# ViTAE-Transformer/SAMRS

Measured on AMD Instinct MI355X. Metric: images/sec (1024^2, vit_h, 32 boxes/img) SAM box->mask, higher is better.
Workload: dtype f16

## Files before the change

### include/samrs_hip_internal.h

```cpp
#ifndef SAMRS_HIP_INTERNAL_H
#define SAMRS_HIP_INTERNAL_H

#include "samrs_hip.h"

#ifdef __cplusplus
extern "C" {
#endif

int samrs_debug_encoder_prefix(samrs_engine_t* e, const uint8_t* images, int n_images, int in_h,
                               int in_w, int n_blocks, float* x_out, void* stream);

int samrs_debug_outlier_columns(samrs_engine_t* e, int block, int gemm, int32_t* out32);

void samrs_debug_set_gemm_variant(int variant);
void samrs_debug_gemm_choice(int prec, int M, int N, int K, int out_f32, int gelu, int accumulate, int has_add2d, int ld, int variant,
                             int32_t* out);
void samrs_debug_set_gemm_skew(int xcd_units, int cu_units);
int samrs_debug_has_experiments(void);

int samrs_debug_copy_buffer(samrs_engine_t* e, const char* name, void* dst, size_t bytes, void* stream);

int samrs_debug_time_dominant_kernel(samrs_engine_t* e, int enable);
int samrs_debug_dominant_kernel_time(samrs_engine_t* e, float* avg_ms, int* launches, int* M, int* N, int* K);

// ... 43 lines not shown
int samrs_k_mask_embed(const float* w0, const float* b0, const float* ln1w, const float* ln1b, const float* w3, const float* b3,
                       const float* ln4w, const float* ln4b, const float* w6, const float* b6, const float* mask_in, float* dense,
                       int n, int grid, void* stream);
int samrs_k_fill_slot_table(const int32_t* start_host, const int32_t* slot_host, int n_runs, int32_t* out, void* stream);
int samrs_k_make_keys(int prec, const float* emb, const float* dense, const float* vec, float* out_f32, void* out_et, int n_batches,
                      int tokens, int C, const int32_t* slot_of, void* stream);
int samrs_k_token_self_attn(const float* q, const float* k, const float* v, float* o, int n, int T, int C, int heads, void* stream);
int64_t samrs_k_t2i_workspace_floats(int n, int T);
int samrs_k_t2i_attention(int prec, const float* qp, const void* kp_et, const void* vp_et, int ld, int64_t bstride, float* out,
                          float* workspace, int n, int T, int tokens, int Ci, int heads, const int32_t* slot_of, void* stream);
int samrs_k_i2t_attention(int prec, const void* qi_et, int ld, int64_t bstride, const float* kt, const float* vt, void* out_et, int n,
                          int T, int tokens, int Ci, int heads, void* stream);
int samrs_k_i2t_fused(int prec, const void* qi_et, int ld, int64_t q_bstride, const float* kt, const float* vt, const void* w_et,
                      const void* w_lo_et, const float* bias, const float* resid, int64_t r_bstride, const float* gamma,
                      const float* beta, float eps, float* outF, void* outE, void* outE_lo, int n, int T, int tokens, int Ci, int C,
                      const int32_t* slot_of, void* stream);
int samrs_k_group_ln_gelu(int prec, const float* in, const float* gamma, const float* beta, float eps, void* out_et, int64_t rows,
                          int groups, int gsize, void* stream);
int samrs_k_mask_product(int prec, const void* up2_et, const float* hyper, float* low, int n, int grid, int n_mask_tokens, int sel0,
                         int n_sel, void* stream);
int samrs_k_attention_mx(int prec, int global, const void* qkv_et, const float* qkv_bias, const float* rel_h, const float* rel_w,
                         void* out_et, void* out_lo_et, int n_images, int grid, int heads, int head_dim, void* q_hi, void* q_lo,
                         void* s_hi, void* s_lo, void* stream);
int64_t samrs_k_mx_scale_bytes(int rows, int Kp, int is_b);
int samrs_k_layernorm_mx(int prec, const float* X, const float* gamma, const float* beta, float eps, void* out_et, int rows, int D,
                         void* q_hi, void* q_lo, void* s_hi, void* s_lo, void* stream);
int samrs_k_mx4_pack(int prec, const float* x, const void* hi_in, const void* lo_in, void* out_hi, void* q_hi, void* q_lo, void* s_hi,
                     void* s_lo, int rows, int K, int G, int GP, int is_b, void* stream);
int samrs_k_gemm_mx(int prec, const void* A, const void* B, void* C, const float* bias, int M, int N, int K, int Kp, const void* a4_lo,
                    const void* a4_hi, const void* sa_lo, const void* sa_hi, const void* b4_hi, const void* b4_lo, const void* sb_hi,
                    const void* sb_lo, int out_f32, int accumulate, int split_from_n, void* stream);
int samrs_k_gemm_mx_gelu_mxout(int prec, const void* A, const void* B, void* C_et, const float* bias, int M, int N, int K, int Kp,
                               const void* a4_lo, const void* a4_hi, const void* sa_lo, const void* sa_hi, const void* b4_hi, const void* b4_lo,
                               const void* sb_hi, const void* sb_lo, int gelu, void* o4_hi, void* o4_lo, void* so_hi, void* so_lo, void* stream);
int samrs_k_convert_split(int prec, const float* in, void* out_hi_et, void* out_lo_et, int64_t n, void* stream);
int samrs_k_range_profile(int prec, const void* x_et, long n, int cols, int ld, int64_t* row48, void* stream);
int samrs_k_column_stats(int prec, const void* x_et, int M, int K, int ld, float* partials, double* sumsq, uint32_t* maxbits, void* stream);
int samrs_k_audit_rows_per_partial(void);
int samrs_k_gemm_ld(int prec, const void* A_et, const void* B_et, void* C_et, const float* bias, int M, int N, int K, int ld, int gelu,
                    int gelu_form, void* stream);
int samrs_k_gemm_ext(int prec, const void* A_et, const void* B_et, const void* Ax_et, const void* Bx_et, float* C, const float* bias, int M,
                     int N, int K, void* stream);
int samrs_k_layernorm_ext(int prec, const float* X, const float* gamma, const float* beta, float eps, void* out_et, int rows, int D,
                          int ld_out, const int32_t* oc_idx, int n_oc, int window_mode, void* stream);
int samrs_k_outlier_weight_ext(int prec, const float* W, int N, int K, const int32_t* idx, int n_oc, void* out_et, int ld, int col0,
                               void* stream);
int samrs_k_outlier_side_weight(int prec, const float* W1, const float* b1, int n_rows1, int D, const int32_t* idx2, int n2,
                                const int32_t* idx1, int n1, void* out_et, int Ks, float* bias_out, void* stream);
int samrs_k_outlier_gather(const void* hi_et, const void* lo_et, int D, const int32_t* idx, int n_oc, void* out_et, int rows, void* stream);
int samrs_k_outlier_side_gemm(int prec, const void* Y_et, int lda, const void* Ws_et, const float* bias, int M, int K, void* out_et,
                              void* stream);
int samrs_k_weight_norms(const float* W, int N, int K, float* col_sq, float* row_sq, void* stream);
int samrs_k_range_scan(int prec, const void* x_et, int64_t n, int cols, int ld, uint64_t* counter, void* stream);
int samrs_k_gemm_f32_batch(const float* const* A, const float* const* A2, const float* const* W, const float* const* bias, float* const* C,
                           int count, int lda, int ldc, int M, int N, int K, int relu, int accumulate, void* stream);
int samrs_k_patch_im2col(int prec, const uint8_t* img_u8, void* A_et, void* A_lo_et, int n_images, int in_h, int in_w, int grid, int patch,
                         void* stream);
int samrs_k_transpose_f32(const float* in, float* out, int rows, int cols, void* stream);
int samrs_k_gelu_split(int prec, const float* in, void* hi_et, void* lo_et, int64_t n, void* stream);
int samrs_k_region_labels(const uint8_t* masks, int n, int h, int w, int complement, int32_t* labels_out, void* stream);
int samrs_k_mask_row_extents(const uint8_t* masks, int n, int h, int w, int32_t* ext_out, void* stream);
int samrs_k_mask_hull(const uint8_t* masks, int n, int h, int w, int x0, int y0, int32_t* ext_scratch, int32_t* verts_out, int cap,
                      int32_t* counts_out, void* stream);
int64_t samrs_k_polygon_scratch_bytes(int n, int h, int w, int max_edges);
int64_t samrs_k_polygon_edge_stride(int h, int w, int max_edges);
int samrs_k_polygon_edges(const uint8_t* masks, int n, int h, int w, int max_edges, void* scratch, uint32_t* ids_out, int32_t* succ_out,
                          uint8_t* corner_out, int32_t* counts_out, void* stream);
int samrs_k_polygon_ranks(const uint8_t* masks, int n, int h, int w, int max_edges, void* scratch, int32_t* leader_out,
                          int32_t* rank_out, int32_t* counts_out, void* stream);
int64_t samrs_k_polygon_simplify_scratch_bytes(int n, int64_t vertex_capacity, int64_t ring_capacity);
int samrs_k_polygon_simplify_keep(const int32_t* vertices, const int32_t* rings, const int64_t* table, int n, int eps_q,
                                  int64_t vertex_capacity, int64_t ring_capacity, void* scratch, uint8_t* keep_out, int32_t* kept_out,
                                  void* stream);

#ifdef __cplusplus
}
#endif
#endif
```

### samrs_amd/csrc/encoder_kernels.hip

```cpp
#include "common.h"
#include "kernels.h"

namespace {

__constant__ float c_mean[3] = {123.675f, 116.28f, 103.53f};
__constant__ float c_std[3] = {58.395f, 57.12f, 57.375f};

template <int PREC>
__global__ void patch_im2col_kernel(const uint8_t* __restrict__ img, uint16_t* __restrict__ A, uint16_t* __restrict__ A_lo,
                                    int n_images, int in_h, int in_w, int grid, int patch) {
    const int P2 = patch * patch;
    const int halves = patch / 8;
    const long total = (long)n_images * grid * grid * patch * halves;
    const long t = (long)blockIdx.x * blockDim.x + threadIdx.x;
    if (t >= total) return;
    const int half = t % halves;
    long u = t / halves;
    const int ky = u % patch; u /= patch;
    const int px = u % grid; u /= grid;
    const int py = u % grid;
    const int im = u / grid;
    const int y = py * patch + ky, x0 = px * patch + half * 8;
    float v[3][8];
#pragma unroll
// ... 1459 lines not shown
    }();
    dim3 g(n_items < n_cu ? n_items : n_cu), b(C::THREADS);
    k<<<g, b, C::LDS_BYTES, s>>>((const uint16_t*)qkv, qb, rh, rw, (uint16_t*)out, grid, heads, n_items, (uint16_t*)out_lo, mx, lo_heads,
                                 dense);
    return hipGetLastError();
}

hipError_t launch_window_attention(int prec, const void* qkv, const float* qkv_bias, const float* rel_h, const float* rel_w, void* out,
                                   int n_images, int grid, int window, int heads, int head_dim, hipStream_t s, void* out_lo,
                                   void* mx_q_hi, void* mx_q_lo, void* mx_s_hi, void* mx_s_lo, uint32_t lo_heads) {
    if (window != 14) return hipErrorInvalidValue;
    if (heads > 32) lo_heads = 0xffffffffu;
    MxOut mx;
    if (mx_q_hi) {
        if (!mx_q_lo || !mx_s_hi || !mx_s_lo || (heads * ((head_dim + 31) / 32) * 32) % MXK) return hipErrorInvalidValue;
        mx.q_hi = (unsigned char*)mx_q_hi; mx.q_lo = (unsigned char*)mx_q_lo; mx.s_hi = (unsigned char*)mx_s_hi; mx.s_lo = (unsigned char*)mx_s_lo;
    }
#define WIN_CALL(P, H)                                                                                                          \
    return mx_q_hi ? launch_win<P, H, 2>(qkv, qkv_bias, rel_h, rel_w, out, n_images, grid, heads, s, nullptr, mx)               \
         : out_lo ? launch_win<P, H, 1>(qkv, qkv_bias, rel_h, rel_w, out, n_images, grid, heads, s, out_lo, MxOut(), lo_heads)  \
                  : launch_win<P, H, 0>(qkv, qkv_bias, rel_h, rel_w, out, n_images, grid, heads, s)
    if (prec == PREC_BF16) {
        if (head_dim == 64) WIN_CALL(PREC_BF16, 64);
        if (head_dim == 80) WIN_CALL(PREC_BF16, 80);
    } else if (prec == PREC_F16) {
        if (head_dim == 64) WIN_CALL(PREC_F16, 64);
        if (head_dim == 80) WIN_CALL(PREC_F16, 80);
    }
#undef WIN_CALL
    return hipErrorInvalidValue;
}

static int g_glb_waves = [] { const char* v = getenv("SAMRS_GLB_WAVES"); return (v && atoi(v) == 4) ? 4 : 8; }();

template <int PREC, int HD, int NW, int LO = 0>
static hipError_t launch_glb_nw(const void* qkv, const float* rh, const float* rw, void* out, int n_images,
                                int heads, void* vt_ws, hipStream_t s, void* out_lo = nullptr, MxOut mx = MxOut()) {
    using C = GlbCfg<HD, NW>;
    constexpr int NTOK = C::G * C::G;
#ifdef SAMRS_EXPERIMENTS
    static const bool pipe = [] { const char* v = getenv("SAMRS_GLB_PIPE"); return v ? atoi(v) != 0 : false; }();
    auto k = pipe ? global_attention_kernel<PREC, HD, NW, LO, 1> : global_attention_kernel<PREC, HD, NW, LO, 0>;
#else
    auto k = global_attention_kernel<PREC, HD, NW, LO, 0>;
#endif
    HIP_CHECK_RET(set_lds(k, C::LDS_BYTES));
    dim3 g((NTOK / (32 * NW)) * heads * n_images), b(64 * NW);
    k<<<g, b, C::LDS_BYTES, s>>>((const uint16_t*)qkv, (const uint16_t*)vt_ws, rh, rw, (uint16_t*)out, heads, (uint16_t*)out_lo, mx);
    return hipGetLastError();
}

template <int PREC, int HD>
static hipError_t launch_glb(const void* qkv, const float* rh, const float* rw, void* out, int n_images,
                             int heads, void* vt_ws, hipStream_t s, void* out_lo, MxOut mx) {
    constexpr int NTOK = GlbCfg<HD>::G * GlbCfg<HD>::G;
    vt_pack_kernel<HD><<<n_images * heads * (NTOK / 64), 256, 0, s>>>((const uint16_t*)qkv, (uint16_t*)vt_ws, heads, NTOK);
    HIP_CHECK_RET(hipGetLastError());
    if (mx.q_hi) return launch_glb_nw<PREC, HD, 8, 2>(qkv, rh, rw, out, n_images, heads, vt_ws, s, nullptr, mx);
    if (out_lo) return launch_glb_nw<PREC, HD, 8, 1>(qkv, rh, rw, out, n_images, heads, vt_ws, s, out_lo);
    if (g_glb_waves == 4) return launch_glb_nw<PREC, HD, 4>(qkv, rh, rw, out, n_images, heads, vt_ws, s);
    return launch_glb_nw<PREC, HD, 8>(qkv, rh, rw, out, n_images, heads, vt_ws, s);
}

hipError_t launch_global_attention(int prec, const void* qkv, const float* rel_h, const float* rel_w, void* out,
                                   int n_images, int grid, int heads, int head_dim, void* vt_ws, hipStream_t s, void* out_lo,
                                   void* mx_q_hi, void* mx_q_lo, void* mx_s_hi, void* mx_s_lo) {
    if (grid != 64 || !vt_ws) return hipErrorInvalidValue;
    MxOut mx;
    if (mx_q_hi) {
        if (!mx_q_lo || !mx_s_hi || !mx_s_lo || (heads * ((head_dim + 31) / 32) * 32) % MXK) return hipErrorInvalidValue;
        mx.q_hi = (unsigned char*)mx_q_hi; mx.q_lo = (unsigned char*)mx_q_lo; mx.s_hi = (unsigned char*)mx_s_hi; mx.s_lo = (unsigned char*)mx_s_lo;
    }
    if (prec == PREC_BF16) {
        if (head_dim == 64) return launch_glb<PREC_BF16, 64>(qkv, rel_h, rel_w, out, n_images, heads, vt_ws, s, out_lo, mx);
        if (head_dim == 80) return launch_glb<PREC_BF16, 80>(qkv, rel_h, rel_w, out, n_images, heads, vt_ws, s, out_lo, mx);
    } else if (prec == PREC_F16) {
        if (head_dim == 64) return launch_glb<PREC_F16, 64>(qkv, rel_h, rel_w, out, n_images, heads, vt_ws, s, out_lo, mx);
        if (head_dim == 80) return launch_glb<PREC_F16, 80>(qkv, rel_h, rel_w, out, n_images, heads, vt_ws, s, out_lo, mx);
    }
    return hipErrorInvalidValue;
}

template <int PREC>
__global__ void gelu_split_kernel(const float* __restrict__ in, uint16_t* __restrict__ hi, uint16_t* __restrict__ lo, long n4) {
    const long i = (long)blockIdx.x * blockDim.x + threadIdx.x;
    if (i >= n4) return;
    const float4 v = reinterpret_cast<const float4*>(in)[i];
    const float2_t a = gelu_erf2(float2_t{v.x, v.y}), b = gelu_erf2(float2_t{v.z, v.w});
    uint2 h, l;
    split2_pack<PREC>(a.x, a.y, h.x, l.x);
    split2_pack<PREC>(b.x, b.y, h.y, l.y);
    reinterpret_cast<uint2*>(hi)[i] = h;
    reinterpret_cast<uint2*>(lo)[i] = l;
}
hipError_t launch_gelu_split(int prec, const float* in, void* hi, void* lo, long n, hipStream_t s) {
    if (n % 4 || !hi || !lo) return hipErrorInvalidValue;
    const long n4 = n / 4;
    const int blocks = (int)((n4 + 255) / 256);
    if (prec == PREC_BF16) gelu_split_kernel<PREC_BF16><<<blocks, 256, 0, s>>>(in, (uint16_t*)hi, (uint16_t*)lo, n4);
    else gelu_split_kernel<PREC_F16><<<blocks, 256, 0, s>>>(in, (uint16_t*)hi, (uint16_t*)lo, n4);
    return hipGetLastError();
}

hipError_t launch_neck_im2col(const void* in, void* A, int n_images, int grid, int C, hipStream_t s) {
    if (C % 8) return hipErrorInvalidValue;
    const long total = (long)n_images * grid * grid * (9 * C / 8);
    neck_im2col_kernel<<<(int)((total + 255) / 256), 256, 0, s>>>((const uint16_t*)in, (uint16_t*)A, n_images, grid, C);
    return hipGetLastError();
}

hipError_t launch_transpose_f32(const float* in, float* out, int rows, int cols, hipStream_t s) {
    dim3 g((cols + 31) / 32, (rows + 31) / 32), b(32, 8);
    transpose_f32_kernel<<<g, b, 0, s>>>(in, out, rows, cols);
    return hipGetLastError();
}
```

### samrs_amd/csrc/engine.hip

```cpp
#include <algorithm>
#include <cmath>
#include <cstdlib>

#include "engine_state.h"

static int env_int(const char* name, int dflt) { const char* v = getenv(name); return v ? atoi(v) : dflt; }

namespace {

bool is_global(const samrs_config& c, int i) {
    for (int k = 0; k < c.n_global; ++k)
        if (c.global_attn_indexes[k] == i) return true;
    return false;
}

void required_tensors(const samrs_engine* e, std::vector<std::pair<std::string, std::vector<int64_t>>>& out) {
    const samrs_config& c = e->cfg;
    const int64_t D = c.embed_dim, g = e->grid, hd = e->hd, C = c.out_chans, P = c.patch_size;
    auto add = [&](const std::string& n, std::vector<int64_t> s) { out.emplace_back(n, std::move(s)); };
    add("image_encoder.pos_embed", {1, g, g, D});
    add("image_encoder.patch_embed.proj.weight", {D, 3, P, P});
    add("image_encoder.patch_embed.proj.bias", {D});
    for (int i = 0; i < c.depth; ++i) {
        const std::string p = "image_encoder.blocks." + std::to_string(i);
// ... 201 lines not shown
extern "C" {

int samrs_abi_version(void) { return SAMRS_ABI_VERSION; }

const char* samrs_last_error(const samrs_engine_t* e) { return e ? e->err.c_str() : "null engine"; }

samrs_engine_t* samrs_create(const samrs_config* cfg, int device, char* err, int err_len) {
    auto bad = [&](const char* m) -> samrs_engine_t* {
        if (err && err_len > 0) snprintf(err, err_len, "%s", m);
        return nullptr;
    };
    if (!cfg) return bad("null config");
    if (cfg->img_size != 1024 || cfg->patch_size != 16 || cfg->window_size != 14 || cfg->out_chans != 256)
        return bad("only img_size 1024 / patch 16 / window 14 / out_chans 256 are supported (build_sam.py:62-80)");
    if (cfg->embed_dim % 128 || cfg->embed_dim % cfg->num_heads) return bad("embed_dim must be a multiple of 128 and of num_heads");
    const int hd = cfg->embed_dim / cfg->num_heads;
    if (hd != 64 && hd != 80) return bad("head_dim must be 64 or 80");
    if (cfg->precision != SAMRS_PREC_BF16 && cfg->precision != SAMRS_PREC_F16) return bad("bad precision");
    if (cfg->max_images < 1 || cfg->max_prompts < 1 || cfg->max_points < 0 || cfg->n_global < 0 || cfg->n_global > 8)
        return bad("bad capacity / n_global");
    if (5 + cfg->max_points + 1 + 2 > 16) return bad("max_points too large (token count must stay <= 16)");
    {
        DeviceGuard dg(device);
        if (dg.status != hipSuccess) return bad("hipSetDevice failed (no HIP device? this library has no CPU fallback)");
    }
    samrs_engine* e = new samrs_engine();
    e->cfg = *cfg;
    e->device = device;
    e->prec = cfg->precision;
    e->grid = cfg->img_size / cfg->patch_size;
    e->tokens = e->grid * e->grid;
    e->D = cfg->embed_dim;
    e->C = cfg->out_chans;
    e->hd = hd;
    e->nwin = (e->grid + cfg->window_size - 1) / cfg->window_size;
    e->T_max = 5 + cfg->max_points + 1 + 2;
    e->decode_prompts = cfg->max_prompts;
    e->slot_set.assign(cfg->max_images, 0);
    e->slot_split.assign(cfg->max_images, 0);
    e->slot_depth.assign(cfg->max_images, 0);
    e->decoder_fusion = env_int("SAMRS_DECODER_FUSION", 1) != 0;
    e->ln_fold = env_int("SAMRS_LN_FOLD", 0) != 0 && gemm_has_experiments();
    const bool h_like = gemm_split3_ok(e->tokens, 3 * e->D, e->D) && gemm_split3_ok(e->tokens, e->D, e->D) && (2 * e->D) % 320 == 0;
    e->split = env_int("SAMRS_SPLIT", SPLIT_DEFAULT | (h_like ? SPLIT_ATTN_V : 0)) & SPLIT_ALL;
    e->grade_multimask = h_like ? SPLIT_ATTN_ANY : 0;
    e->allow_reduced = env_int("SAMRS_ALLOW_REDUCED", getenv("SAMRS_SPLIT") ? 1 : 0) != 0;
    e->upscaler_fused = env_int("SAMRS_UPSCALER_FUSED", 1) != 0;
    e->split_passes = env_int("SAMRS_SPLIT_PASSES", 0) != 0;
    e->split_depth = env_int("SAMRS_SPLIT_DEPTH", 0);
    e->lo_format = (h_like && env_int("SAMRS_LO_FORMAT", 4) == 4) ? 4 : 0;
    e->gelu_fast = env_int("SAMRS_GELU_FAST", -1);
    e->ln_tail = env_int("SAMRS_LN_TAIL", 0) != 0;
    e->operand_pad_on = env_int("SAMRS_OPERAND_PAD", 1) != 0;
    e->outlier_on = env_int("SAMRS_OUTLIER_COLS", 7) & 7;
    e->outlier_ratio_pct = env_int("SAMRS_OUTLIER_RATIO_PCT", 400);
    if (e->outlier_ratio_pct < 101) e->outlier_ratio_pct = 101;
    if (e->gelu_fast > 1) e->gelu_fast = 1;
    e->range_profile = env_int("SAMRS_RANGE_PROFILE", 0);
    if (e->range_profile < 0 || e->range_profile > 2) e->range_profile = 0;
    e->audit_passes = env_int("SAMRS_AUDIT_PASSES", 0);
    if (e->audit_passes > 0) e->range_profile = 2; else e->audit_passes = 0;
    if (const int rc0 = env_int("SAMRS_RANGE_CHECK", 0)) {
        if (samrs_set_option(e, "range_check", rc0) != SAMRS_OK) {
            if (err && err_len > 0) snprintf(err, err_len, "SAMRS_RANGE_CHECK=%d: %s", rc0, e->err.c_str());
            samrs_destroy(e);
            return nullptr;
        }
    }
    return e;
}

void samrs_destroy(samrs_engine_t* e) {
    if (!e) return;
    DeviceGuard dg(e->device);
    for (void* p : e->owned) (void)hipFree(p);
    for (DeviceScratch* sc : {&e->rle_scratch, &e->rle_decode_scratch, &e->region_scratch, &e->box_scratch, &e->poly_scratch, &e->png_scratch, &e->png_rgb_scratch, &e->overlap_scratch, &e->ap_scratch, &e->boundary_scratch}) scratch_release(*sc);
    delete e;
}

int samrs_load_weight(samrs_engine_t* e, const char* name, const float* host, const int64_t* shape, int ndim) {
    if (!e || !name || !host || !shape || ndim < 1 || ndim > 4) return fail(e, SAMRS_ERR_BAD_ARG, "samrs_load_weight: bad argument");
    if (e->finalized) return fail(e, SAMRS_ERR_BAD_WEIGHTS, "weights already finalized");
    ON_DEVICE(e);
    DevTensor t;
    t.shape.assign(shape, shape + ndim);
    t.numel = 1;
    for (int i = 0; i < ndim; ++i) t.numel *= (size_t)shape[i];
    const std::string n(name);
    std::vector<float> tmp;
    const float* src = host;
    if (n == "image_encoder.neck.2.weight" && ndim == 4) {
        const int64_t Co = shape[0], Ci = shape[1], KH = shape[2], KW = shape[3];
        tmp.resize(t.numel);
        for (int64_t co = 0; co < Co; ++co)
            for (int64_t ci = 0; ci < Ci; ++ci)
                for (int64_t ky = 0; ky < KH; ++ky)
                    for (int64_t kx = 0; kx < KW; ++kx)
                        tmp[(co * KH * KW + ky * KW + kx) * Ci + ci] = host[((co * Ci + ci) * KH + ky) * KW + kx];
        src = tmp.data();
    } else if ((n == "mask_decoder.output_upscaling.0.weight" || n == "mask_decoder.output_upscaling.3.weight") && ndim == 4) {
        const int64_t Ci = shape[0], Co = shape[1];
        tmp.resize(t.numel);
        for (int64_t ci = 0; ci < Ci; ++ci)
            for (int64_t co = 0; co < Co; ++co)
                for (int64_t s = 0; s < 4; ++s) tmp[(s * Co + co) * Ci + ci] = host[(ci * Co + co) * 4 + s];
        src = tmp.data();
// ... 324 lines not shown

int samrs_get_slot_info(const samrs_engine_t* e, int slot, int32_t* is_set, int32_t* split, int32_t* split_depth) {
    if (!e) return SAMRS_ERR_BAD_ARG;
    if (slot < 0 || slot >= e->cfg.max_images) return SAMRS_ERR_CAPACITY;
    if (is_set) *is_set = e->slot_set[slot];
    if (split) *split = e->slot_set[slot] ? e->slot_split[slot] : 0;
    if (split_depth) *split_depth = e->slot_set[slot] ? e->slot_depth[slot] : 0;
    return SAMRS_OK;
}

int samrs_reset_image(samrs_engine_t* e, int slot) {
    if (!e) return SAMRS_ERR_BAD_ARG;
    if (slot < 0 || slot >= e->cfg.max_images) return fail(e, SAMRS_ERR_CAPACITY, "slot out of range");
    e->slot_set[slot] = 0;
    return SAMRS_OK;
}

int samrs_set_option(samrs_engine_t* e, const char* name, int value) {
    if (!e || !name) return SAMRS_ERR_BAD_ARG;
    const std::string n(name);
    if (n == "decoder_fusion") e->decoder_fusion = value != 0;
    else if (n == "ln_fold") {
        if (value && !gemm_has_experiments())
            return fail(e, SAMRS_ERR_BAD_ARG, "ln_fold: the folded LayerNorm (measured slower: DESIGN.md 6) is built with make EXPERIMENTS=1 only");
        e->ln_fold = value != 0;
    }
    else if (n == "split") {
        if (e->finalized && (value & (SPLIT_ATTN_ANY | SPLIT_MLP | SPLIT_LIN2) & ~e->split_ready))
            return fail(e, SAMRS_ERR_BAD_ARG, "split bits 16 / 32 / 64 / 128 (block GEMMs) need their lo weights: set them before the weights are "
                                              "finalized (SAMRS_SPLIT or options={'split': ...})");
        e->split = value & SPLIT_ALL;
    }
    else if (n == "gemm_variant") e->gemm_variant = value;
    else if (n == "decode_prompts") {
        const long long prod = (long long)e->cfg.max_images * e->cfg.max_prompts;
        const int lo = e->cfg.max_prompts, lim = prod < DECODE_PROMPTS_LIMIT ? (int)prod : DECODE_PROMPTS_LIMIT, hi = lim > lo ? lim : lo;
        if (value < lo || value > hi)
            return fail(e, SAMRS_ERR_BAD_ARG, "decode_prompts=%d is outside [%d, %d]: from max_prompts to max_images x max_prompts = %lld, "
                                              "at most %d (the index range of the decoder kernels)", value, lo, hi, prod, DECODE_PROMPTS_LIMIT);
        if (e->finalized) {
            ON_DEVICE(e);
            const int rc = grow_decode_workspaces(e, value);
            if (rc != SAMRS_OK) return rc;
        }
        e->decode_prompts = value;
    }
    else if (n == "upscaler_fused") e->upscaler_fused = value != 0;
    else if (n == "split_passes") e->split_passes = value != 0;
    else if (n == "split_depth") e->split_depth = value > 0 ? value : 0;
    else if (n == "allow_reduced") e->allow_reduced = value != 0;
    else if (n == "gelu_fast") e->gelu_fast = value < 0 ? -1 : (value != 0);
    else if (n == "ln_tail") e->ln_tail = value > 0;
    else if (n == "operand_pad") e->operand_pad_on = value != 0;
    else if (n == "outlier_cols") e->outlier_on = value & 7;
    else if (n == "outlier_ratio_pct") {
        if (e->finalized) return fail(e, SAMRS_ERR_BAD_ARG, "outlier_ratio_pct: the columns are picked when the weights are finalized; set it before");
        if (value < 101) return fail(e, SAMRS_ERR_BAD_ARG, "outlier_ratio_pct must exceed 100 (a column's score as a percentage of the median score)");
        e->outlier_ratio_pct = value;
    }
    else if (n == "range_check") {
        if (value < 0 || value > 2) return fail(e, SAMRS_ERR_BAD_ARG, "range_check is 0 (off), 1 (count) or 2 (count, and samrs_set_images fails)");
        if (value && !e->range_counter) {
            ON_DEVICE(e);
            CK(e, dalloc(e, &e->range_counter, 1));
            CK(e, hipMemset(e->range_counter, 0, sizeof(unsigned long long)));
        }
        if (value == 2 && e->range_check != 2 && e->range_counter) {
            ON_DEVICE(e);
            CK(e, hipDeviceSynchronize());
            CK(e, hipMemcpy(&e->range_seen, e->range_counter, sizeof(unsigned long long), hipMemcpyDeviceToHost));
        }
        e->range_check = value;
    }
    else if (n == "saturated") {
        if (e->range_counter) {
            ON_DEVICE(e);
            CK(e, hipDeviceSynchronize());
            CK(e, hipMemset(e->range_counter, 0, sizeof(unsigned long long)));
        }
        e->range_seen = 0;
    }
    else if (n == "range_profile") {
        if (value < 0 || value > 2) return fail(e, SAMRS_ERR_BAD_ARG, "range_profile is 0 (off), 1 (range profile per site) or 2 (and column statistics)");
        e->range_profile = value;
        if (!value) e->audit_passes = 0;
    }
    else if (n == "audit_passes") {
        if (value < 0) return fail(e, SAMRS_ERR_BAD_ARG, "audit_passes is the number of encoder passes to profile (0 stops a running audit)");
        if (value > 0) {
            ON_DEVICE(e);
            const int rc = audit_reset(e);
            if (rc != SAMRS_OK) return rc;
            e->range_profile = 2;
        } else if (e->audit_passes > 0) e->range_profile = 0;
        e->audit_passes = value;
    }
    else if (n == "lo_format") {
        if (value != 0 && value != 4) return fail(e, SAMRS_ERR_BAD_ARG, "lo_format is 0 (f16 lo terms) or 4 (MXFP4 lo terms)");
        if (value == 4 && e->finalized && !e->mx_ready && !e->mx_mlp_ready)
            return fail(e, SAMRS_ERR_BAD_ARG, "lo_format 4 needs the fp4 weight copies: set it (and a block-GEMM split bit) before the weights are "
                                              "finalized; it covers the attention-side split of models whose block GEMMs fit the 256 x 320 tile (ViT-H)");
        e->lo_format = value;
    }
    else return fail(e, SAMRS_ERR_BAD_ARG, "unknown option %s", name);
    return SAMRS_OK;
}
int samrs_get_option(const samrs_engine_t* e, const char* name, int* value) {
    if (!e || !name || !value) return SAMRS_ERR_BAD_ARG;
    const std::string n(name);
    if (n == "decoder_fusion") *value = e->decoder_fusion;
    else if (n == "ln_fold") *value = e->ln_fold;
    else if (n == "split") *value = e->split;
    else if (n == "gemm_variant") *value = e->gemm_variant;
    else if (n == "decode_prompts") *value = e->decode_prompts;
    else if (n == "decode_kbytes") *value = (int)((e->decode_bytes + 1023) / 1024);
    else if (n == "upscaler_fused") *value = e->upscaler_fused;
    else if (n == "split_passes") *value = e->split_passes;
    else if (n == "split_depth") *value = e->split_depth;
    else if (n == "allow_reduced") *value = e->allow_reduced;
    else if (n == "gelu_fast") *value = e->gelu_fast;
    else if (n == "ln_tail") *value = e->ln_tail;
    else if (n == "operand_pad") *value = e->operand_pad_on;
    else if (n == "outlier_cols") *value = e->outlier_on;
    else if (n == "outlier_ratio_pct") *value = e->outlier_ratio_pct;
    else if (n == "outlier_blocks") *value = e->outlier_blocks;
    else if (n == "outlier_columns") *value = e->outlier_columns;
    else if (n == "outlier_dominant_blocks") *value = e->outlier_dominant_blocks;
    else if (n == "range_check") *value = e->range_check;
    else if (n == "saturated") {
        unsigned long long c = 0;
        if (e->range_counter) {
            DeviceGuard dg(e->device);
            if (dg.status != hipSuccess || hipDeviceSynchronize() != hipSuccess ||
                hipMemcpy(&c, e->range_counter, sizeof(c), hipMemcpyDeviceToHost) != hipSuccess) return SAMRS_ERR_HIP;
        }
        *value = c > 0x7fffffffull ? 0x7fffffff : (int)c;
    }
    else if (n == "range_profile") *value = e->range_profile;
    else if (n == "audit_passes") *value = e->audit_passes;
    else if (n == "lo_format") *value = (e->finalized && !e->mx_ready && !e->mx_mlp_ready) ? 0 : e->lo_format;
    else if (n == "grade_multimask") *value = e->grade_multimask;
    else return SAMRS_ERR_BAD_ARG;
    return SAMRS_OK;
}

}
```

### samrs_amd/csrc/engine_decode.hip

```cpp
#include "engine_state.h"

namespace {

struct PredictImage {
    int slot, p0, p1, in_h, in_w, orig_h, orig_w;
    void* masks;
};


enum class I2T { FUSED, PER_SEGMENT, SHARED_RESIDUAL, ACCUMULATE };
enum class Upscaler { ONE_KERNEL, GLN_SPLIT, GLN, UNFUSED };

struct DecodeLayerRoute {
    bool shared = false;
    long bstride = 0;
    bool tab = false;
    I2T i2t = I2T::FUSED;
    bool write_kf = false;
    bool write_ke_lo = false;
    bool ow_lo = false;
};

struct DecodeRoute {
    int T = 0, BT = 0, Mi = 0;
// ... 149 lines not shown
    const size_t hs = (size_t)e->decode_alloc * C;
    F32Batch l0{}, l1{}, l2{};
    for (int i = 0; i < 5; ++i) {
        l0.A[i] = i < 4 ? e->Q + (size_t)(1 + i) * C : e->Q;
        l0.W[i] = w.head_w[i][0]; l0.bias[i] = w.head_b[i][0]; l0.C[i] = e->HY1 + i * hs;
        l1.A[i] = e->HY1 + i * hs;
        l1.W[i] = w.head_w[i][1]; l1.bias[i] = w.head_b[i][1]; l1.C[i] = e->HY2 + i * hs;
        if (i < 4) {
            l2.A[i] = e->HY2 + i * hs;
            l2.W[i] = w.head_w[i][2]; l2.bias[i] = w.head_b[i][2]; l2.C[i] = e->HYPER + i * (C / 8);
        }
    }
    CK(e, launch_gemm_f32_batch(l0, 5, r.T * C, C, n, C, C, true, false, s));
    CK(e, launch_gemm_f32_batch(l1, 5, C, C, n, C, C, true, false, s));
    CK(e, launch_gemm_f32_batch(l2, 4, C, 4 * (C / 8), n, C / 8, C, false, false, s));
    if (r.iou)
        CK(e, launch_gemm_f32(e->HY2 + 4 * hs, C, w.head_w[4][2] + (size_t)r.sel0 * C, w.head_b[4][2] + r.sel0, iou_out, r.nsel, n, r.nsel, C,
                              false, false, s));
    return SAMRS_OK;
}

static int run_upscaler(samrs_engine_t* e, const DecodeRoute& r, int n, float* low, hipStream_t s) {
    const int C = e->C, prec = e->prec, g = e->grid, Mi = r.Mi;
    for (const char* name : {"U1raw", "U1", "U2"}) {
        const bool used = !strcmp(name, "U1raw") ? (r.up == Upscaler::GLN_SPLIT || r.up == Upscaler::UNFUSED)
                        : !strcmp(name, "U1")    ? (r.up == Upscaler::GLN || r.up == Upscaler::UNFUSED) : r.up == Upscaler::UNFUSED;
        if (used) { const int rc = need_decode_buffer(e, name); if (rc != SAMRS_OK) return rc; }
    }
    switch (r.up) {
    case Upscaler::ONE_KERNEL:
        CK(e, launch_upscaler_fused(prec, e->KE, r.sp_up ? e->KE_lo : nullptr, e->up1_w, r.sp_up ? e->up1_w_lo : nullptr, e->up1_b, e->up_ln,
                                    e->up2_w, r.sp_up ? e->up2_w_lo : nullptr, e->up2_b, e->HYPER, low, n, g, 4, r.sel0, r.nsel, s));
        break;
    case Upscaler::GLN_SPLIT:
        CK(e, launch_gemm_et_gln(prec, e->KE, e->up1_w, e->U1raw, e->up1_b, e->up_ln, Mi, C, C, s, e->KE_lo, e->up1_w_lo));
        CK(e, launch_upscale2_masks(prec, e->U1raw, e->up2_w, e->up2_w_lo, e->up2_b, e->HYPER, low, n, g, 4, r.sel0, r.nsel, s));
        break;
    case Upscaler::GLN:
        CK(e, launch_gemm_et_gln(prec, e->KE, e->up1_w, e->U1, e->up1_b, e->up_ln, Mi, C, C, s));
        CK(e, launch_upscale2_masks(prec, e->U1, e->up2_w, nullptr, e->up2_b, e->HYPER, low, n, g, 4, r.sel0, r.nsel, s));
        break;
    case Upscaler::UNFUSED:
        CK(e, launch_gemm_et(prec, e->KE, e->up1_w, e->U1raw, e->up1_b, nullptr, 0, Mi, C, C, true, false, false, s));
        CK(e, launch_group_ln_gelu(prec, e->U1raw, e->dec.up_ln_w, e->dec.up_ln_b, 1e-6f, e->U1, (long)Mi, 4, C / 4, s));
        CK(e, launch_gemm_et(prec, e->U1, e->up2_w, e->U2, e->up2_b, nullptr, 0, Mi * 4, C / 2, C / 4, false, true, false, s));
        CK(e, launch_mask_product(prec, e->U2, e->HYPER, low, n, g, 4, r.sel0, r.nsel, s));
        break;
    }
    return SAMRS_OK;
}

static int run_postprocess(samrs_engine_t* e, const DecodeRoute& r, const PredictImage* seg, int n_seg, const float* low, int return_logits,
                           hipStream_t s) {
    for (int k = 0; k < n_seg; ++k)
        if (seg[k].masks)
            CK(e, launch_postprocess(low + (size_t)seg[k].p0 * r.nsel * 256 * 256, (seg[k].p1 - seg[k].p0) * r.nsel, seg[k].in_h, seg[k].in_w,
                                     seg[k].orig_h, seg[k].orig_w, e->cfg.img_size, return_logits, seg[k].masks, s));
    return SAMRS_OK;
}

static int predict_chunk(samrs_engine_t* e, const PredictImage* seg, int n_seg, int n, const float* boxes, const float* point_coords,
                         const int32_t* point_labels, int n_points, const float* mask_input, int multimask,
                         int return_logits, float* iou_out, float* lowres_out, void* stream) {
    if (n < 1 || n > e->decode_prompts || n > e->decode_alloc)
        return fail(e, SAMRS_ERR_CAPACITY, "a decoder chain of %d prompts exceeds decode_prompts=%d", n, e->decode_prompts);
    hipStream_t s = (hipStream_t)stream;
    ON_DEVICE(e);
    const DecodeRoute r = decode_route(e, n, n_seg, seg[0].slot, boxes != nullptr, point_coords ? n_points : 0, mask_input != nullptr,
                                       multimask != 0, iou_out != nullptr, lowres_out != nullptr);
    float* low = r.low_own ? e->LOW : lowres_out;
    int rc;
    if ((rc = run_prompt_side(e, r, seg, n_seg, n, boxes, point_coords, point_labels, n_points, mask_input, s))) return rc;
    for (int li = 0; li < 2; ++li)
        if ((rc = run_dec_layer(e, r, li, seg, n_seg, n, s))) return rc;
    if ((rc = run_final_attn(e, r, n, s))) return rc;
    if ((rc = run_heads(e, r, n, iou_out, s))) return rc;
    if ((rc = run_upscaler(e, r, n, low, s))) return rc;
    return run_postprocess(e, r, seg, n_seg, low, return_logits, s);
}

static std::string slot_note(int slot) { return " (slot " + std::to_string(slot) + ")"; }

static int check_multimask_grade(samrs_engine_t* e, int slot, bool multi) {
    if (e->allow_reduced || !e->grade_multimask || slot < 0 || slot >= e->cfg.max_images || !e->slot_set[slot]) return SAMRS_OK;
    const int sm = e->slot_split[slot];
    const int need_depth = sm < 0 ? 0 : (sm & (SPLIT_ATTN | SPLIT_MLP | SPLIT_LIN2)) ? e->cfg.depth : (3 * e->cfg.depth + 3) / 4;
    if (sm >= 0 && (!(sm & e->grade_multimask) || e->slot_depth[slot] < need_depth ||
                    (e->split & (SPLIT_OI | SPLIT_UP)) != (SPLIT_OI | SPLIT_UP)))
        return fail(e, SAMRS_ERR_PRECISION, "multimask_output=True on an embedding encoded with split=%d over %d of %d blocks (decoder split=%d): "
                    "this model's multimask outputs need a block-GEMM split bit (64 or 16) at its automatic depth and the decoder "
                    "bits 4 | 8 to hold IoU >= 0.999; re-encode the image in the engine's default mode, or set option "
                    "\"allow_reduced\" = 1%s", sm, e->slot_depth[slot], need_depth, e->split, multi ? slot_note(slot).c_str() : "");
    return SAMRS_OK;
}

static int check_predict(samrs_engine_t* e, const PredictImage* im, int n_img, bool multi, const float* boxes, const float* point_coords,
                         const int32_t* point_labels, int n_points, const float* mask_input) {
    if (!e->finalized) return fail(e, SAMRS_ERR_BAD_WEIGHTS, "weights not finalized");
    const samrs_config& c = e->cfg;
    for (int i = 0; i < n_img; ++i) {
        const int slot = im[i].slot;
        if (slot < 0 || slot >= c.max_images)
            return multi ? fail(e, SAMRS_ERR_CAPACITY, "image %d: slot %d out of range (max_images=%d)", i, slot, c.max_images)
                         : fail(e, SAMRS_ERR_CAPACITY, "slot out of range");
        if (!e->slot_set[slot])
            return multi ? fail(e, SAMRS_ERR_NOT_SET, "An image must be set with .set_image(...) before mask prediction "
                                "(image %d: slot %d is not set).", i, slot)
                         : fail(e, SAMRS_ERR_NOT_SET, "An image must be set with .set_image(...) before mask prediction.");
    }
    if (!boxes && !point_coords && !mask_input) return fail(e, SAMRS_ERR_BAD_ARG, "at least one prompt (points, boxes or mask_input) is required");
// ... 77 lines not shown
```

### samrs_amd/csrc/engine_encode.hip

```cpp
#include "engine_state.h"

enum { AUDIT_QKV_IN = 0, AUDIT_Q, AUDIT_K, AUDIT_V, AUDIT_PROJ_IN, AUDIT_LIN1_IN, AUDIT_LIN2_IN, AUDIT_PER_BLOCK };
enum { AUDIT_NECK1_IN = 0, AUDIT_NECK2_IN, AUDIT_KEYS0, AUDIT_TAIL };

namespace samrs_detail {
void audit_build_sites(samrs_engine_t* e) {
    static const char* const per_block[AUDIT_PER_BLOCK] = {"qkv_in", "q", "k", "v", "proj_in", "lin1_in", "lin2_in"};
    e->audit_sites.clear();
    e->audit_columns = 0;
    auto add = [&](const std::string& name, int columns) {
        e->audit_sites.push_back({name, columns, e->audit_columns});
        e->audit_columns += (size_t)columns;
    };
    for (int i = 0; i < e->cfg.depth; ++i)
        for (int k = 0; k < AUDIT_PER_BLOCK; ++k)
            add("blocks." + std::to_string(i) + "." + per_block[k],
                (k == AUDIT_QKV_IN || k == AUDIT_PROJ_IN || k == AUDIT_LIN1_IN) ? e->D : k == AUDIT_LIN2_IN ? 4 * e->D : 0);
    add("neck.conv1_in", 0); add("neck.conv2_in", 0); add("decoder.keys0", 0);
    e->audit_col_rows.assign(e->audit_sites.size(), 0);
}

int audit_reset(samrs_engine_t* e) {
    if (e->audit_rows || e->audit_sumsq) CK(e, hipDeviceSynchronize());
    if (e->audit_rows) CK(e, hipMemset(e->audit_rows, 0, e->audit_sites.size() * AUDIT_PROFILE_WORDS * sizeof(long long)));
// ... 62 lines not shown
    if (r == hipSuccess && order == MainPass::LAST) r = launch_gemm_et(prec, A, B, C, bias, add2d, add2d_period, M, N, K, true, false, true, s);
    return r;
}

namespace {
struct PassRoute {
    int M = 0;
    int n_blocks = 0;
    bool sp_patch = false, sp_neck = false;
    bool one3 = false;
    bool fold = false;
    int depth_full = 0, depth_v = 0;
    bool fast_gelu = false;
    bool ln_tail = false;
    bool pad_ok = false;
    bool oc_any = false, oc_ok = false;
};

static PassRoute pass_route(const samrs_engine_t* e, int M, int n_blocks) {
    const samrs_config& c = e->cfg;
    const int D = e->D;
    PassRoute p;
    p.M = M;
    p.n_blocks = n_blocks;
    p.sp_patch = (e->split & SPLIT_PATCH) != 0;
    p.sp_neck = (e->split & SPLIT_NECK) != 0;
    p.fold = e->can_fold && e->ln_fold && !(e->split & SPLIT_ATTN_ANY) && !(e->split & SPLIT_MLP);
    p.depth_full = e->split_depth > 0 ? e->split_depth : c.depth;
    p.depth_v = e->split_depth > 0 ? e->split_depth : (3 * c.depth + 3) / 4;
    p.one3 = !e->split_passes;
    p.fast_gelu = e->gelu_fast >= 0 ? e->gelu_fast != 0 : !(e->split & (SPLIT_ATTN_ANY | SPLIT_MLP | SPLIT_LIN2));
    p.ln_tail = !p.fold && !(e->split & (SPLIT_ATTN_ANY | SPLIT_MLP | SPLIT_LIN2)) && e->ln_tail > 0 &&
                e->ln_counters && gemm_lntail_ok(M, D, D) && gemm_lntail_ok(M, D, 4 * D);
    p.pad_ok = e->ldk && e->operand_pad_on && !p.fold && !p.ln_tail;
    p.oc_any = e->outlier_on && e->outlier_columns > 0 && !p.fold && !p.ln_tail;
    p.oc_ok = p.oc_any && (e->outlier_on & 1);
    return p;
}

enum class Norm { NONE, TAIL, PLAIN, LO, MX };
enum class Gemm { FOLD, MX, SPLIT3, PLAIN, LNTAIL, EXT };
enum class Wcopy { W, WP, WX };

struct BlockRoute {
    Norm norm1 = Norm::PLAIN, norm2 = Norm::PLAIN;
    Gemm qkv = Gemm::PLAIN, proj = Gemm::PLAIN, lin1 = Gemm::PLAIN, lin2 = Gemm::PLAIN;
    bool qkv_one = false, proj_one = false, lin1_one = false, lin2_one = false;
    int v_from = 0;
    int noc = 0;
    Wcopy qkv_wc = Wcopy::W;
    int qkv_K = 0, qkv_ld = 0;
    int norm1_ld = 0;
    int y1_ld = 0, y1_live = 0;
    bool mx_ao = false;
    bool ao_lo = false;
    int nop = 0;
    uint32_t lo_heads = 0xffffffffu;
    int nol = 0;
    Wcopy lin1_wc = Wcopy::W;
    int lin1_K = 0, lin1_ld = 0;
    int norm2_ld = 0;
    int y2_ld = 0, y2_live = 0;
    int lin1_mx_from = 0;
    int nol2 = 0;
    int side_ld = 0;
    bool next_rowstat = false;
};

static BlockRoute block_route(const samrs_engine_t* e, const PassRoute& p, const EncBlock& b, int i) {
    const int D = e->D, M = p.M, depth = e->cfg.depth;
    BlockRoute r;
    const bool attn_full = (e->split & SPLIT_ATTN) && i < p.depth_full;
    const bool oc_dominant = p.oc_any && (e->outlier_on & 5) == 5 && !attn_full && (b.oc_share[0] > 0.5f || b.oc_share[3] > 0.5f);
    const bool sp_attn = attn_full || ((e->split & SPLIT_ATTN_V) && i < p.depth_v && !oc_dominant);
    const bool sp_mlp = (e->split & SPLIT_MLP) && i < p.depth_full;
    const bool mx_mlp = e->lo_format == 4 && e->mx_mlp_ready && !e->split_passes && gemm_mx_ok(M, 4 * D, D, D) && gemm_mx_ok(M, D, 4 * D, e->mx_kp_lin2);
    const bool sp_lin2 = (e->split & SPLIT_LIN2) && !sp_mlp && mx_mlp && i < p.depth_full;
    const bool mx_attn = e->lo_format == 4 && e->mx_ready && !e->split_passes && gemm_mx_ok(M, 3 * D, D, D) && (2 * D) % 320 == 0;

    r.qkv_K = D; r.y1_ld = D; r.y1_live = D;
    if (p.fold) {
        r.norm1 = Norm::NONE; r.qkv = Gemm::FOLD;
    } else if (sp_attn && mx_attn) {
        r.norm1 = Norm::MX; r.qkv = Gemm::MX;
        r.v_from = attn_full ? 0 : 2 * D;
        r.noc = (p.oc_ok && !attn_full && b.oc_n[0] && e->ldk && b.qkv_wp) ? b.oc_n[0] : 0;
        if (r.noc) { r.qkv_wc = Wcopy::WP; r.qkv_ld = r.norm1_ld = r.y1_ld = e->ldk; r.y1_live = D + 64; }
    } else if (sp_attn) {
        r.norm1 = Norm::LO; r.qkv = Gemm::SPLIT3;
        r.qkv_one = p.one3 && gemm_split3_ok(M, 3 * D, D);
        r.v_from = (!attn_full && r.qkv_one && (2 * D) % 320 == 0) ? 2 * D : 0;
    } else {
        r.noc = (p.oc_ok && b.oc_n[0] && b.qkv_wx) ? b.oc_n[0] : 0;
        r.qkv_K = r.noc ? D + 64 : D;
        r.qkv_ld = (p.pad_ok && b.qkv_wp && gemm_ld_ok(M, 3 * D, r.qkv_K, false)) ? e->ldk : 0;
        r.qkv_wc = r.qkv_ld ? Wcopy::WP : (r.noc ? Wcopy::WX : Wcopy::W);
        r.y1_ld = r.qkv_ld ? r.qkv_ld : r.qkv_K;
        r.y1_live = r.qkv_K;
        r.norm1_ld = r.y1_ld == D ? 0 : r.y1_ld;
    }

    r.mx_ao = sp_attn && mx_attn;
    r.nop = (p.oc_any && (e->outlier_on & 4) && !sp_attn && b.oc_n[3] && b.oc_bx[3] && e->AOlo && e->OCX) ? b.oc_n[3] : 0;
    r.ao_lo = (sp_attn && !r.mx_ao) || r.nop;
    r.lo_heads = r.nop ? b.oc_heads : 0xffffffffu;

    if (p.fold) r.proj = Gemm::FOLD;
    else if (sp_attn && mx_attn) r.proj = Gemm::MX;
    else if (sp_attn) { r.proj = Gemm::SPLIT3; r.proj_one = p.one3 && gemm_split3_ok(M, D, D); }
    else if (p.ln_tail) r.proj = Gemm::LNTAIL;
    else if (r.nop) r.proj = Gemm::EXT;

    const bool lin1_plain = !p.fold && !sp_lin2 && !sp_mlp;
    r.nol = (p.oc_ok && lin1_plain && b.oc_n[1] && b.lin1_wx) ? b.oc_n[1] : 0;
    r.lin1_K = r.nol ? D + 64 : D;
    r.lin1_ld = (p.pad_ok && b.lin1_wp && lin1_plain && gemm_ld_ok(M, 4 * D, r.lin1_K, true)) ? e->ldk : 0;
    r.lin1_wc = r.lin1_ld ? Wcopy::WP : (r.nol ? Wcopy::WX : Wcopy::W);
    r.side_ld = r.lin1_ld ? r.lin1_ld : r.lin1_K;
    r.y2_ld = D; r.y2_live = D;
    if (p.fold) r.norm2 = Norm::NONE;
    else if (r.proj == Gemm::LNTAIL) r.norm2 = Norm::TAIL;
    else if (sp_mlp && mx_mlp) r.norm2 = Norm::MX;
    else {
        r.norm2 = sp_mlp ? Norm::LO : Norm::PLAIN;
        r.norm2_ld = (sp_mlp || r.side_ld == D) ? 0 : r.side_ld;
        if (r.norm2_ld) { r.y2_ld = r.norm2_ld; r.y2_live = r.lin1_K; }
    }
    if (p.fold) r.lin1 = Gemm::FOLD;
    else if (sp_lin2) { r.lin1 = Gemm::MX; r.lin1_mx_from = 4 * D; }
    else if (sp_mlp && mx_mlp) r.lin1 = Gemm::MX;
    else if (sp_mlp) { r.lin1 = Gemm::SPLIT3; r.lin1_one = p.one3 && gemm_split3_ok(M, 4 * D, D); }

    r.nol2 = (p.oc_any && (e->outlier_on & 2) && lin1_plain && b.oc_n[2] && b.oc_bx[2] && e->OCX && b.lin2_ws &&
              (b.oc_n[1] == 0 || r.nol > 0)) ? b.oc_n[2] : 0;
    if (p.fold) { r.lin2 = Gemm::FOLD; r.next_rowstat = i + 1 < depth; }
    else if ((sp_mlp && mx_mlp) || sp_lin2) r.lin2 = Gemm::MX;
    else if (sp_mlp) { r.lin2 = Gemm::SPLIT3; r.lin2_one = p.one3 && gemm_split3_ok(M, D, 4 * D); }
    else if (p.ln_tail && i + 1 < depth && i + 1 < p.n_blocks) r.lin2 = Gemm::LNTAIL;
    else if (r.nol2) r.lin2 = Gemm::EXT;
    return r;
}

static const uint16_t* weight_copy(Wcopy c, const uint16_t* w, const uint16_t* wp, const uint16_t* wx) {
    return c == Wcopy::WP ? wp : c == Wcopy::WX ? wx : w;
}

static hipError_t run_norm(samrs_engine_t* e, Norm form, const float* gamma, const float* beta, int M, int ld, const int* oc_idx, int n_oc,
                           hipStream_t s) {
    if (form == Norm::NONE || form == Norm::TAIL) return hipSuccess;
    const bool mx = form == Norm::MX;
    return launch_layernorm(e->prec, e->X, gamma, beta, 1e-6f, e->Y, nullptr, M, e->D, 0, e->grid, 0, s, form == Norm::LO ? e->Ylo : nullptr,
                            mx ? e->Y4[0] : nullptr, mx ? e->Y4[1] : nullptr, mx ? e->SY4[0] : nullptr, mx ? e->SY4[1] : nullptr, ld,
                            n_oc ? oc_idx : nullptr, n_oc);
}
}

static int run_patch_embed(samrs_engine_t* e, const PassRoute& p, const uint8_t* const* images, const int* in_h, const int* in_w, int n,
                           hipStream_t s) {
    const samrs_config& c = e->cfg;
    const int D = e->D, tokens = e->tokens, prec = e->prec, M = p.M;
    const size_t KP = (size_t)3 * c.patch_size * c.patch_size;
    uint16_t* Hlo = e->H + (size_t)M * KP;
    for (int i = 0; i < n;) {
        int j = i + 1;
        while (j < n && in_h[j] == in_h[i] && in_w[j] == in_w[i] &&
               images[j] == images[i] + (size_t)(j - i) * in_h[i] * in_w[i] * 3) ++j;
        CK(e, launch_patch_im2col(prec, images[i], e->H + (size_t)i * tokens * KP, j - i, in_h[i], in_w[i], e->grid, c.patch_size, s,
                                  p.sp_patch ? Hlo + (size_t)i * tokens * KP : nullptr));
        i = j;
    }
    const float *bias = W(e, "image_encoder.patch_embed.proj.bias"), *pos = W(e, "image_encoder.pos_embed");
    if (p.sp_patch)
        CK(e, gemm_hilo(prec, p.one3 && gemm_split3_ok(M, D, (int)KP, true), MainPass::FIRST, e->H, Hlo, e->patch_w, e->patch_w_lo, e->X,
                        bias, pos, tokens, M, D, (int)KP, false, s));
    else
        CK(e, launch_gemm_et(prec, e->H, e->patch_w, e->X, bias, pos, tokens, M, D, (int)KP, true, false, false, s));
    if (p.fold && p.n_blocks > 0) {
        CK(e, launch_rowstats_convert(prec, e->X, e->Y, e->STATS, M, D, s));
        CK(e, launch_ln_rowstat(e->STATS, e->ROWSTAT, M, 1e-6f, s));
    }
    return SAMRS_OK;
}

static int run_block_attn(samrs_engine_t* e, const PassRoute& p, const BlockRoute& r, const EncBlock& b, int i, int n, bool y_ready,
                          hipStream_t s) {
    const samrs_config& c = e->cfg;
    const int D = e->D, g = e->grid, prec = e->prec, M = p.M;
    int rc;
    if (!y_ready) CK(e, run_norm(e, r.norm1, b.ln1w, b.ln1b, M, r.norm1_ld, b.oc_idx[0], r.noc, s));
    const uint16_t* qkv_w = weight_copy(r.qkv_wc, b.qkv_w, b.qkv_wp, b.qkv_wx);
    if (r.qkv == Gemm::FOLD) {
        CK(e, launch_gemm_et_fold(prec, e->Y, b.qkv_wf, e->QKV, b.qkv_bf, b.qkv_c, e->ROWSTAT, M, 3 * D, D, false, s));
    } else if (r.qkv == Gemm::MX) {
        CK(e, launch_gemm_et_mx(prec, e->Y, qkv_w, e->QKV, b.qkv_b, M, 3 * D, D, D, e->Y4[1], e->Y4[0], e->SY4[1], e->SY4[0],
                                b.qkv_w4[0], b.qkv_w4[1], b.qkv_s4[0], b.qkv_s4[1], false, false, r.v_from, s,
                                false, nullptr, nullptr, nullptr, nullptr, r.qkv_ld, r.noc != 0));
    } else if (r.qkv == Gemm::SPLIT3 && r.qkv_one) {
        CK(e, launch_gemm_et_split3(prec, e->Y, e->Ylo, b.qkv_w, b.qkv_w_lo, e->QKV, b.qkv_b, M, 3 * D, D, false, false, s, r.v_from));
    } else if (r.qkv == Gemm::SPLIT3) {
        if (!e->F32T) CK(e, dalloc(e, &e->F32T, (size_t)c.max_images * e->tokens * 4 * D));
        CK(e, gemm_hilo(prec, false, MainPass::LAST, e->Y, e->Ylo, b.qkv_w, b.qkv_w_lo, e->F32T, b.qkv_b, nullptr, 0, M, 3 * D, D, false, s));
        CK(e, launch_convert(prec, e->F32T, e->QKV, (long)M * 3 * D, s));
    } else {
        CK(e, launch_gemm_et(prec, e->Y, qkv_w, e->QKV, b.qkv_b, nullptr, 0, M, 3 * D, r.qkv_K, false, false, false, s, GemmOpts{r.qkv_ld, 1}));
    }
    if (!b.global)
        CK(e, launch_window_attention(prec, e->QKV, b.qkv_b, b.rel_h, b.rel_w, e->AO, n, g, c.window_size, c.num_heads, e->hd, s,
                                      r.ao_lo ? e->AOlo : nullptr, r.mx_ao ? e->AO4[0] : nullptr, r.mx_ao ? e->AO4[1] : nullptr,
                                      r.mx_ao ? e->SAO4[0] : nullptr, r.mx_ao ? e->SAO4[1] : nullptr, r.lo_heads));
    else
        CK(e, launch_global_attention(prec, e->QKV, b.rel_h, b.rel_w, e->AO, n, g, c.num_heads, e->hd, e->VTG, s,
                                      r.ao_lo ? e->AOlo : nullptr, r.mx_ao ? e->AO4[0] : nullptr, r.mx_ao ? e->AO4[1] : nullptr,
                                      r.mx_ao ? e->SAO4[0] : nullptr, r.mx_ao ? e->SAO4[1] : nullptr));
    if ((rc = range_scan(e, e->Y, (size_t)M * r.y1_live, s, r.y1_live, r.y1_ld))) return rc;
    if ((rc = range_scan(e, e->QKV, (size_t)M * 3 * D, s))) return rc;
    if ((rc = range_scan(e, e->AO, (size_t)M * D, s))) return rc;
    if ((rc = audit_site(e, AUDIT_PER_BLOCK * i + AUDIT_QKV_IN, e->Y, M, D, r.y1_ld, s))) return rc;
    for (int t = 0; t < 3; ++t)
        if ((rc = audit_site(e, AUDIT_PER_BLOCK * i + AUDIT_Q + t, e->QKV + (size_t)t * D, M, D, 3 * D, s))) return rc;
    if ((rc = audit_site(e, AUDIT_PER_BLOCK * i + AUDIT_PROJ_IN, e->AO, M, D, D, s))) return rc;

    if (r.proj == Gemm::FOLD) {
        CK(e, launch_gemm_et_stats(prec, e->AO, b.proj_w, e->X, b.proj_b, e->Y, e->STATS, M, D, D, s));
        CK(e, launch_ln_rowstat(e->STATS, e->ROWSTAT, M, 1e-6f, s));
    } else if (r.proj == Gemm::MX) {
        CK(e, launch_gemm_et_mx(prec, e->AO, b.proj_w, e->X, b.proj_b, M, D, D, e->mx_kp_proj, e->AO4[1], e->AO4[0], e->SAO4[1],
                                e->SAO4[0], b.proj_w4[0], b.proj_w4[1], b.proj_s4[0], b.proj_s4[1], true, true, 0, s));
    } else if (r.proj == Gemm::SPLIT3) {
        CK(e, gemm_hilo(prec, r.proj_one, MainPass::LAST, e->AO, e->AOlo, b.proj_w, b.proj_w_lo, e->X, b.proj_b, nullptr, 0, M, D, D, true, s));
    } else if (r.proj == Gemm::LNTAIL) {
        CK(e, launch_gemm_et_lntail(prec, e->AO, b.proj_w, e->X, b.proj_b, M, D, D, b.ln2w, b.ln2b, 1e-6f, e->Y, e->ln_counters, s));
    } else if (r.proj == Gemm::EXT) {
        CK(e, launch_outlier_gather(e->AO, e->AOlo, D, b.oc_idx[3], r.nop, e->OCX, M, s));
        CK(e, resid_gemm_ext(e, prec, e->AO, b.proj_w, e->OCX, b.oc_bx[3], b.proj_b, M, D, D, s));
    } else {
        CK(e, launch_gemm_et(prec, e->AO, b.proj_w, e->X, b.proj_b, nullptr, 0, M, D, D, true, false, true, s));
    }
    CK(e, run_norm(e, r.norm2, b.ln2w, b.ln2b, M, r.norm2_ld, b.oc_idx[1], r.nol, s));
    return SAMRS_OK;
}

static int run_block_mlp(samrs_engine_t* e, const PassRoute& p, const BlockRoute& r, const EncBlock& b, int i, bool* y_ready, hipStream_t s) {
    const int D = e->D, prec = e->prec, M = p.M;
    int rc;
    hipEvent_t t0 = nullptr, t1 = nullptr;
    if (e->timing) {
        auto get = [&](hipEvent_t* ev) -> hipError_t {
            if (!e->tpool.empty()) { *ev = e->tpool.back(); e->tpool.pop_back(); return hipSuccess; }
            return hipEventCreate(ev);
        };
        CK(e, get(&t0)); CK(e, get(&t1));
        CK(e, hipEventRecord(t0, s));
    }
    if (r.lin1 == Gemm::FOLD) {
        CK(e, launch_gemm_et_fold(prec, e->Y, b.lin1_wf, e->H, b.lin1_bf, b.lin1_c, e->ROWSTAT, M, 4 * D, D, true, s));
    } else if (r.lin1 == Gemm::MX) {
        CK(e, launch_gemm_et_mx(prec, e->Y, b.lin1_w, e->H, b.lin1_b, M, 4 * D, D, D, e->Y4[1], e->Y4[0], e->SY4[1], e->SY4[0], b.lin1_w4[0],
                                b.lin1_w4[1], b.lin1_s4[0], b.lin1_s4[1], false, false, r.lin1_mx_from, s, true, e->H4[0], e->H4[1], e->SH4[0], e->SH4[1]));
    } else if (r.lin1 == Gemm::SPLIT3) {
        CK(e, gemm_hilo(prec, r.lin1_one, MainPass::LAST, e->Y, e->Ylo, b.lin1_w, b.lin1_w_lo, e->F32T, b.lin1_b, nullptr, 0, M, 4 * D, D, false, s));
        CK(e, launch_gelu_split(prec, e->F32T, e->H, e->Hlo, (long)M * 4 * D, s));
    } else {
        CK(e, launch_gemm_et(prec, e->Y, weight_copy(r.lin1_wc, b.lin1_w, b.lin1_wp, b.lin1_wx), e->H, b.lin1_b, nullptr, 0, M, 4 * D, r.lin1_K,
                             false, true, false, s, GemmOpts{r.lin1_ld, p.fast_gelu ? 2 : 1}));
    }
    if (e->timing) {
        CK(e, hipEventRecord(t1, s));
        e->tev.emplace_back(t0, t1);
    }
    if ((rc = range_scan(e, e->Y, (size_t)M * r.y2_live, s, r.y2_live, r.y2_ld))) return rc;
    if ((rc = range_scan(e, e->H, (size_t)M * 4 * D, s))) return rc;
    if ((rc = audit_site(e, AUDIT_PER_BLOCK * i + AUDIT_LIN1_IN, e->Y, M, D, r.y2_ld, s))) return rc;
    if ((rc = audit_site(e, AUDIT_PER_BLOCK * i + AUDIT_LIN2_IN, e->H, M, 4 * D, 4 * D, s))) return rc;

    *y_ready = false;
    if (r.lin2 == Gemm::FOLD) {
        CK(e, launch_gemm_et_stats(prec, e->H, b.lin2_w, e->X, b.lin2_b, e->Y, e->STATS, M, D, 4 * D, s));
        if (r.next_rowstat) CK(e, launch_ln_rowstat(e->STATS, e->ROWSTAT, M, 1e-6f, s));
    } else if (r.lin2 == Gemm::MX) {
        CK(e, launch_gemm_et_mx(prec, e->H, b.lin2_w, e->X, b.lin2_b, M, D, 4 * D, e->mx_kp_lin2, e->H4[1], e->H4[0], e->SH4[1], e->SH4[0],
                                b.lin2_w4[0], b.lin2_w4[1], b.lin2_s4[0], b.lin2_s4[1], true, true, 0, s));
    } else if (r.lin2 == Gemm::SPLIT3) {
        CK(e, gemm_hilo(prec, r.lin2_one, MainPass::LAST, e->H, e->Hlo, b.lin2_w, b.lin2_w_lo, e->X, b.lin2_b, nullptr, 0, M, D, 4 * D, true, s));
    } else if (r.lin2 == Gemm::LNTAIL) {
        const EncBlock& nb = e->blocks[i + 1];
        CK(e, launch_gemm_et_lntail(prec, e->H, b.lin2_w, e->X, b.lin2_b, M, D, 4 * D, nb.ln1w, nb.ln1b, 1e-6f, e->Y, e->ln_counters, s));
        *y_ready = true;
    } else if (r.lin2 == Gemm::EXT) {
        CK(e, launch_outlier_side_gemm(prec, e->Y, r.side_ld, b.lin2_ws, b.lin2_sb, M, r.lin1_K, e->OCX, s));
        CK(e, resid_gemm_ext(e, prec, e->H, b.lin2_w, e->OCX, b.oc_bx[2], b.lin2_b, M, D, 4 * D, s));
    } else {
        CK(e, launch_gemm_et(prec, e->H, b.lin2_w, e->X, b.lin2_b, nullptr, 0, M, D, 4 * D, true, false, true, s));
    }
    return SAMRS_OK;
}

static int prepare_slot_keys(samrs_engine_t* e, int slot0, int n, hipStream_t s) {
    const int C = e->C, Ci = C / 2, tokens = e->tokens, prec = e->prec;
    const DecLayer& L = e->layers[0];
    for (int i = 0; i < n; ++i) {
        const size_t o = (size_t)(slot0 + i) * tokens * C;
        CK(e, launch_make_keys(prec, e->EMB + o, nullptr, e->dec.no_mask_embed, e->K0F + o, e->K0E + o, 1, tokens, C, s));
    }
    CK(e, launch_gemm_et(prec, e->K0E + (size_t)slot0 * tokens * C, L.kvq_w, e->KVQ0 + (size_t)slot0 * tokens * 3 * Ci, L.kvq_b, L.kvq_pe,
                         tokens, n * tokens, 3 * Ci, C, false, false, false, s));
    return SAMRS_OK;
}

static int run_neck(samrs_engine_t* e, const PassRoute& p, int n, int slot0, hipStream_t s) {
    const samrs_config& c = e->cfg;
    const int D = e->D, C = e->C, g = e->grid, tokens = e->tokens, prec = e->prec, M = p.M;
    const int audit_tail = AUDIT_PER_BLOCK * c.depth;
    int rc;
    uint16_t* lo_buf = e->QKV;
    if (p.sp_neck) CK(e, launch_convert(prec, e->X, e->Y, (long)M * D, s, lo_buf));
    else if (!(p.fold && c.depth > 0 && p.n_blocks >= c.depth)) CK(e, launch_convert(prec, e->X, e->Y, (long)M * D, s));
    if ((rc = range_scan(e, e->Y, (size_t)M * D, s))) return rc;
    if ((rc = audit_site(e, audit_tail + AUDIT_NECK1_IN, e->Y, M, D, D, s))) return rc;
    if (p.sp_neck)
        CK(e, gemm_hilo(prec, p.one3 && gemm_split3_ok(M, C, D, true), MainPass::FIRST, e->Y, lo_buf, e->neck0_w, e->neck0_w_lo, e->N1,
                        nullptr, nullptr, 0, M, C, D, false, s));
    else
        CK(e, launch_gemm_et(prec, e->Y, e->neck0_w, e->N1, nullptr, nullptr, 0, M, C, D, true, false, false, s));
    CK(e, launch_layernorm(prec, e->N1, W(e, "image_encoder.neck.1.weight"), W(e, "image_encoder.neck.1.bias"), 1e-6f,
                           e->N1e, nullptr, M, C, 0, g, 0, s, p.sp_neck ? lo_buf : nullptr));
    if ((rc = range_scan(e, e->N1e, (size_t)M * C, s))) return rc;
    if ((rc = audit_site(e, audit_tail + AUDIT_NECK2_IN, e->N1e, M, C, C, s))) return rc;
    CK(e, launch_neck_im2col(e->N1e, e->H, n, g, C, s));
    uint16_t* H2lo = e->H + (size_t)M * 9 * C;
    if (p.sp_neck) {
        CK(e, launch_neck_im2col(lo_buf, H2lo, n, g, C, s));
        CK(e, gemm_hilo(prec, p.one3 && gemm_split3_ok(M, C, 9 * C, true), MainPass::FIRST, e->H, H2lo, e->neck2_w, e->neck2_w_lo, e->N1,
                        nullptr, nullptr, 0, M, C, 9 * C, false, s));
    } else
        CK(e, launch_gemm_et(prec, e->H, e->neck2_w, e->N1, nullptr, nullptr, 0, M, C, 9 * C, true, false, false, s));
    CK(e, launch_layernorm(prec, e->N1, W(e, "image_encoder.neck.3.weight"), W(e, "image_encoder.neck.3.bias"), 1e-6f,
                           nullptr, e->EMB + (size_t)slot0 * tokens * C, M, C, 0, g, 0, s));
    return prepare_slot_keys(e, slot0, n, s);
}

static int finish_pass(samrs_engine_t* e, const PassRoute& p, int n, int slot0, hipStream_t s) {
    const int C = e->C, tokens = e->tokens;
    int rc;
    if ((rc = range_scan(e, e->K0E + (size_t)slot0 * tokens * C, (size_t)n * tokens * C, s))) return rc;
    if (e->range_check == 2) {
        unsigned long long now = 0;
        CK(e, hipStreamSynchronize(s));
        CK(e, hipMemcpy(&now, e->range_counter, sizeof(now), hipMemcpyDeviceToHost));
        const unsigned long long before = e->range_seen;
        e->range_seen = now;
        if (now > before)
            return fail(e, SAMRS_ERR_RANGE, "%llu operand values of this encoder pass saturated the %s range (|x| >= %s): the masks of these "
                        "images are not the reference's.  Use precision bf16 (fp32 exponent range, 8 mantissa bits) for this "
                        "checkpoint, or option \"range_check\" = 1 to count without failing", now - before,
                        e->prec == PREC_F16 ? "f16" : "bf16", e->prec == PREC_F16 ? "65504" : "inf");
    }
// ... 16 lines not shown
    for (int i = 0; i < n; ++i) {
        if (!images[i]) return fail(e, SAMRS_ERR_BAD_ARG, "samrs_set_images: null image pointer (tile %d)", i);
        if (in_h[i] < 1 || in_w[i] < 1 || in_h[i] > c.img_size || in_w[i] > c.img_size || (in_h[i] != c.img_size && in_w[i] != c.img_size))
            return fail(e, SAMRS_ERR_BAD_SHAPE, "set_torch_image input must be BCHW with long side %d.", c.img_size);
    }
    hipStream_t s = (hipStream_t)stream;
    ON_DEVICE(e);
    int rc;
    for (int i = 0; i < n; ++i) e->slot_set[slot0 + i] = 0;
    if (e->range_profile && (rc = audit_prepare(e, e->range_profile == 2))) return rc;
    const PassRoute p = pass_route(e, n * e->tokens, n_blocks);
    if ((rc = run_patch_embed(e, p, images, in_h, in_w, n, s))) return rc;
    bool y_ready = false;
    for (int i = 0; i < c.depth && i < n_blocks; ++i) {
        const EncBlock& b = e->blocks[i];
        const BlockRoute r = block_route(e, p, b, i);
        if ((rc = run_block_attn(e, p, r, b, i, n, y_ready, s))) return rc;
        if ((rc = run_block_mlp(e, p, r, b, i, &y_ready, s))) return rc;
    }
    if (!do_neck) return SAMRS_OK;
    if ((rc = run_neck(e, p, n, slot0, s))) return rc;
    return finish_pass(e, p, n, slot0, s);
}

static int encode_stack(samrs_engine_t* e, const uint8_t* images, int n, int in_h, int in_w, int slot0, void* stream,
                        int n_blocks, bool do_neck) {
    if (!e || !images) return fail(e, SAMRS_ERR_BAD_ARG, "samrs_set_images: null argument");
    if (n < 1 || n > e->cfg.max_images) return fail(e, SAMRS_ERR_CAPACITY, "n_images/slot out of range (max_images=%d)", e->cfg.max_images);
    std::vector<const uint8_t*> ptr(n);
    std::vector<int> hs(n, in_h), ws(n, in_w);
    for (int i = 0; i < n; ++i) ptr[i] = images + (size_t)i * (in_h > 0 ? in_h : 0) * (in_w > 0 ? in_w : 0) * 3;
    return encode(e, ptr.data(), hs.data(), ws.data(), n, slot0, stream, n_blocks, do_neck);
}

extern "C" {
int samrs_set_images(samrs_engine_t* e, const uint8_t* images, int n, int in_h, int in_w, int slot0, void* stream) {
    return encode_stack(e, images, n, in_h, in_w, slot0, stream, 1 << 30, true);
}

int samrs_set_images_ragged(samrs_engine_t* e, const uint8_t* const* images, const int* in_h, const int* in_w, int n,
                            int slot0, void* stream) {
    return encode(e, images, in_h, in_w, n, slot0, stream, 1 << 30, true);
}

int samrs_debug_encoder_prefix(samrs_engine_t* e, const uint8_t* images, int n, int in_h, int in_w, int n_blocks,
                               float* x_out, void* stream) {
    if (!x_out) return fail(e, SAMRS_ERR_BAD_ARG, "samrs_debug_encoder_prefix: null output");
    const int rc = encode_stack(e, images, n, in_h, in_w, 0, stream, n_blocks, false);
    if (rc) return rc;
    CK(e, hipMemcpyAsync(x_out, e->X, sizeof(float) * (size_t)n * e->tokens * e->D, hipMemcpyDeviceToDevice, (hipStream_t)stream));
    return SAMRS_OK;
}

int samrs_get_embedding(samrs_engine_t* e, int slot, float* out_chw, void* stream) {
    if (!e || !out_chw) return fail(e, SAMRS_ERR_BAD_ARG, "samrs_get_embedding: null argument");
    if (slot < 0 || slot >= e->cfg.max_images) return fail(e, SAMRS_ERR_CAPACITY, "slot out of range");
    if (!e->slot_set[slot]) return fail(e, SAMRS_ERR_NOT_SET, "An image must be set with .set_image(...) to generate an embedding.");
    ON_DEVICE(e);
    CK(e, launch_transpose_f32(e->EMB + (size_t)slot * e->tokens * e->C, out_chw, e->tokens, e->C, (hipStream_t)stream));
    return SAMRS_OK;
}

int samrs_set_embedding(samrs_engine_t* e, int slot, const float* emb_chw, void* stream) {
    if (!e || !emb_chw) return fail(e, SAMRS_ERR_BAD_ARG, "samrs_set_embedding: null argument");
    if (!e->finalized) return fail(e, SAMRS_ERR_BAD_WEIGHTS, "weights not finalized");
    if (slot < 0 || slot >= e->cfg.max_images) return fail(e, SAMRS_ERR_CAPACITY, "slot out of range");
    ON_DEVICE(e);
    CK(e, launch_transpose_f32(emb_chw, e->EMB + (size_t)slot * e->tokens * e->C, e->C, e->tokens, (hipStream_t)stream));
    { const int rc = prepare_slot_keys(e, slot, 1, (hipStream_t)stream); if (rc != SAMRS_OK) return rc; }
    e->slot_set[slot] = 1;
    e->slot_split[slot] = -1;
    e->slot_depth[slot] = 0;
    return SAMRS_OK;
}

int samrs_audit_site_count(const samrs_engine_t* e, int* n_sites) {
    if (!e || !n_sites) return SAMRS_ERR_BAD_ARG;
    *n_sites = (int)e->audit_sites.size();
    return SAMRS_OK;
}
int samrs_audit_site_name(const samrs_engine_t* e, int site, char* name, int name_len, int* columns) {
    if (!e || !name || name_len < 1 || site < 0 || site >= (int)e->audit_sites.size()) return SAMRS_ERR_BAD_ARG;
    snprintf(name, (size_t)name_len, "%s", e->audit_sites[site].name.c_str());
    if (columns) *columns = e->audit_sites[site].columns;
    return SAMRS_OK;
}
int samrs_audit_read_profile(samrs_engine_t* e, int64_t* rows, int reset) {
    if (!e || !rows) return fail(e, SAMRS_ERR_BAD_ARG, "samrs_audit_read_profile: null argument");
    const size_t n = e->audit_sites.size() * AUDIT_PROFILE_WORDS;
    if (!e->audit_rows) {
        for (size_t i = 0; i < n; ++i) rows[i] = 0;
        return SAMRS_OK;
    }
    ON_DEVICE(e);
    CK(e, hipDeviceSynchronize());
    CK(e, hipMemcpy(rows, e->audit_rows, n * sizeof(int64_t), hipMemcpyDeviceToHost));
    return reset ? audit_reset(e) : SAMRS_OK;
}
int samrs_audit_read_columns(samrs_engine_t* e, int site, double* sumsq, float* max_abs, int64_t* n_rows) {
    if (!e || !sumsq || !max_abs || !n_rows) return fail(e, SAMRS_ERR_BAD_ARG, "samrs_audit_read_columns: null argument");
    if (site < 0 || site >= (int)e->audit_sites.size()) return fail(e, SAMRS_ERR_BAD_ARG, "samrs_audit_read_columns: site %d of %d", site, (int)e->audit_sites.size());
    const samrs_engine::AuditSite& a = e->audit_sites[site];
    if (a.columns == 0)
        return fail(e, SAMRS_ERR_BAD_ARG, "samrs_audit_read_columns: site %s has no column statistics (the block GEMMs' A operands have: qkv_in, proj_in, lin1_in, lin2_in)", a.name.c_str());
    if (!e->audit_sumsq || e->audit_col_rows[site] == 0)
        return fail(e, SAMRS_ERR_BAD_ARG, "samrs_audit_read_columns: no encoder pass has been profiled with option \"range_profile\" = 2 (or \"audit_passes\") since the last reset");
// ... 21 lines not shown
```

### samrs_amd/csrc/engine_hooks.hip

```cpp
#include <mutex>

#include "engine_state.h"

extern "C" {
void samrs_debug_set_gemm_variant(int v) { set_gemm_variant(v); }
void samrs_debug_gemm_choice(int prec, int M, int N, int K, int out_f32, int gelu, int accumulate, int has_add2d, int ld, int variant,
                             int32_t* out) {
    gemm_debug_choice(prec, M, N, K, out_f32 != 0, gelu != 0, accumulate != 0, has_add2d != 0, ld, variant, out);
}
void samrs_debug_set_gemm_skew(int xcd_units, int cu_units) { set_gemm_skew(xcd_units, cu_units); }
int samrs_debug_has_experiments(void) { return gemm_has_experiments() ? 1 : 0; }

int samrs_debug_copy_buffer(samrs_engine_t* e, const char* name, void* dst, size_t bytes, void* stream) {
    if (!e || !name || !dst) return SAMRS_ERR_BAD_ARG;
    const std::string n(name);
    const void* src = nullptr;
    if (n == "Q") src = e->Q; else if (n == "TOK0") src = e->TOK0; else if (n == "KF") src = e->KF; else if (n == "KE") src = e->KE;
    else if (n == "KVQ") src = e->KVQ; else if (n == "OI") src = e->OI; else if (n == "U1raw") src = e->U1raw;
    else if (n == "U1") src = e->U1; else if (n == "U2") src = e->U2; else if (n == "HYPER") src = e->HYPER;
    else if (n == "K0F") src = e->K0F; else if (n == "K0E") src = e->K0E; else if (n == "O128") src = e->O128;
    else if (n == "MH") src = e->MH; else if (n == "KT") src = e->KT; else if (n == "VT") src = e->VT; else if (n == "QP") src = e->QP;
    else if (n == "DENSE") src = e->DENSE;
    else return fail(e, SAMRS_ERR_BAD_ARG, "unknown buffer %s", name);
    if (!src) return fail(e, SAMRS_ERR_BAD_ARG, "buffer %s is not allocated yet", name);
    CK(e, hipMemcpyAsync(dst, src, bytes, hipMemcpyDeviceToDevice, (hipStream_t)stream));
    return SAMRS_OK;
}

int samrs_debug_time_dominant_kernel(samrs_engine_t* e, int enable) {
    if (!e) return SAMRS_ERR_BAD_ARG;
    e->timing = enable != 0;
    return SAMRS_OK;
}

int samrs_debug_dominant_kernel_time(samrs_engine_t* e, float* avg_ms, int* launches, int* M, int* N, int* K) {
    if (!e || !avg_ms || !launches) return SAMRS_ERR_BAD_ARG;
    double tot = 0.0;
    int n = 0;
    for (auto& pr : e->tev) {
        CK(e, hipEventSynchronize(pr.second));
        float ms = 0.f;
        CK(e, hipEventElapsedTime(&ms, pr.first, pr.second));
        tot += ms;
        ++n;
        e->tpool.push_back(pr.first);
        e->tpool.push_back(pr.second);
    }
    e->tev.clear();
    *avg_ms = n ? (float)(tot / n) : 0.f;
    *launches = n;
    if (M) *M = 0;
    if (N) *N = 4 * e->D;
    if (K) *K = e->D;
    return SAMRS_OK;
}

int samrs_k_gemm(int prec, const void* A, const void* B, void* C, const float* bias, const float* add2d, int period,
                 int M, int N, int K, int out_f32, int gelu, int accumulate, void* stream) {
    KRET(launch_gemm_et(prec, A, B, C, bias, add2d, period, M, N, K, out_f32 != 0, gelu != 0, accumulate != 0, (hipStream_t)stream));
}
int samrs_k_gemm_stats(int prec, const void* A, const void* B, float* C, const float* bias, void* xh, float* stats, int M, int N,
                       int K, void* stream) {
    KRET(launch_gemm_et_stats(prec, A, B, C, bias, xh, stats, M, N, K, (hipStream_t)stream));
}
int samrs_k_gemm_fold(int prec, const void* xh, const void* Wf, void* C, const float* bias_f, const float* cvec, const float* rowstat,
                      int M, int N, int K, int gelu, void* stream) {
    KRET(launch_gemm_et_fold(prec, xh, Wf, C, bias_f, cvec, rowstat, M, N, K, gelu != 0, (hipStream_t)stream));
}
int samrs_k_ln_rowstat(const float* stats, float* rowstat, int rows, float eps, void* stream) {
    KRET(launch_ln_rowstat(stats, rowstat, rows, eps, (hipStream_t)stream));
}
int samrs_k_ln_fold_weight(int prec, const float* W, const float* gamma, const float* beta, const float* bias, void* Wf, float* cvec,
                           float* bias_f, int N, int K, void* stream) {
    KRET(launch_ln_fold_weight(prec, W, gamma, beta, bias, Wf, cvec, bias_f, N, K, (hipStream_t)stream));
}
// ... 54 lines not shown
                         void* stream) {
    if (!global)
        KRET(launch_window_attention(prec, qkv, qkv_bias, rel_h, rel_w, out, n_images, grid, 14, heads, head_dim, (hipStream_t)stream, out_lo,
                                     q_hi, q_lo, s_hi, s_lo));
    const size_t need = (size_t)n_images * heads * head_dim * grid * grid * 2;
    void* ws = kernel_hook_workspace(need);
    if (!ws) return SAMRS_ERR_HIP;
    KRET(launch_global_attention(prec, qkv, rel_h, rel_w, out, n_images, grid, heads, head_dim, ws, (hipStream_t)stream, out_lo, q_hi, q_lo, s_hi, s_lo));
}
int samrs_debug_outlier_columns(samrs_engine_t* e, int block, int gemm, int32_t* out32) {
    if (!e || !out32 || gemm < 0 || gemm > 3 || block < 0 || block >= (int)e->blocks.size()) return SAMRS_ERR_BAD_ARG;
    const EncBlock& b = e->blocks[block];
    if (b.oc_n[gemm] > 0) {
        ON_DEVICE(e);
        CK(e, hipMemcpy(out32, b.oc_idx[gemm], sizeof(int32_t) * b.oc_n[gemm], hipMemcpyDeviceToHost));
    }
    return b.oc_n[gemm];
}
int samrs_k_range_profile(int prec, const void* x, long n, int cols, int ld, int64_t* row48, void* stream) {
    if (!x || !row48 || n < 0) return SAMRS_ERR_BAD_ARG;
    KRET(launch_range_profile(prec, x, n, cols, ld, reinterpret_cast<long long*>(row48), (hipStream_t)stream));
}
int samrs_k_column_stats(int prec, const void* x, int M, int K, int ld, float* partials, double* sumsq, uint32_t* maxbits, void* stream) {
    if (!x || !partials || !sumsq || !maxbits) return SAMRS_ERR_BAD_ARG;
    KRET(launch_column_stats(prec, x, M, K, ld, partials, sumsq, maxbits, (hipStream_t)stream));
}
int samrs_k_audit_rows_per_partial(void) { return AUDIT_ROWS_PER_PARTIAL; }
static bool idx_ok(const int32_t* idx, int n, int bound, void* stream) {
    if (n == 0) return true;
    int32_t h[32];
    if (!idx || n < 0 || n > 32 || bound < 1) return false;
    if (hipMemcpyAsync(h, idx, sizeof(int32_t) * n, hipMemcpyDeviceToHost, (hipStream_t)stream) != hipSuccess) return false;
    if (hipStreamSynchronize((hipStream_t)stream) != hipSuccess) return false;
    for (int j = 0; j < n; ++j)
        if (h[j] < 0 || h[j] >= bound || (j && h[j] <= h[j - 1])) return false;
    return true;
}
static bool aligned16(const void* p) { return (reinterpret_cast<uintptr_t>(p) & 15) == 0; }
int samrs_k_gemm_ld(int prec, const void* A, const void* B, void* C, const float* bias, int M, int N, int K, int ld, int gelu, int gelu_form,
                    void* stream) {
    if (!A || !B || !C || !aligned16(A) || !aligned16(B) || !aligned16(C)) return SAMRS_ERR_BAD_ARG;
    if (ld < 0 || (gelu_form != 1 && gelu_form != 2)) return SAMRS_ERR_BAD_ARG;
    GemmOpts opts;
    opts.ld = ld;
    opts.gelu_form = gelu_form;
    KRET(launch_gemm_et(prec, A, B, C, bias, nullptr, 0, M, N, K, false, gelu != 0, false, (hipStream_t)stream, opts));
}
int samrs_k_gemm_ext(int prec, const void* A, const void* B, const void* Ax, const void* Bx, float* C, const float* bias, int M, int N, int K,
                     void* stream) {
    if (!A || !B || !Ax || !Bx || !C || !aligned16(A) || !aligned16(B) || !aligned16(Ax) || !aligned16(Bx) || !aligned16(C)) return SAMRS_ERR_BAD_ARG;
    if (M < 1 || N < 1 || K < 1 || !gemm_ext_ok(M, N, K)) return SAMRS_ERR_BAD_SHAPE;
    KRET(launch_gemm_et_ext(prec, A, B, Ax, Bx, C, bias, M, N, K, (hipStream_t)stream));
}
int samrs_k_layernorm_ext(int prec, const float* X, const float* gamma, const float* beta, float eps, void* out_et, int rows, int D, int ld_out,
                          const int32_t* oc_idx, int n_oc, int window_mode, void* stream) {
    if (!X || !gamma || !beta || !out_et || !aligned16(X) || !aligned16(gamma) || !aligned16(beta) || !aligned16(out_et)) return SAMRS_ERR_BAD_ARG;
    if (rows < 1 || D < 4 || ld_out < 0 || n_oc < 0 || n_oc > 32 || (n_oc && ld_out < D + 64)) return SAMRS_ERR_BAD_SHAPE;
    if (window_mode) return SAMRS_ERR_BAD_SHAPE;
    if (!idx_ok(oc_idx, n_oc, D, stream)) return SAMRS_ERR_BAD_ARG;
    KRET(launch_layernorm(prec, X, gamma, beta, eps, out_et, nullptr, rows, D, 0, 0, 0, (hipStream_t)stream, nullptr, nullptr, nullptr, nullptr,
                          nullptr, ld_out, n_oc ? oc_idx : nullptr, n_oc));
}
int samrs_k_outlier_weight_ext(int prec, const float* W, int N, int K, const int32_t* idx, int n_oc, void* out, int ld, int col0, void* stream) {
    if (!W || !out || N < 1 || K < 1 || n_oc < 0 || n_oc > 32 || col0 < 0 || ld < col0 + 64) return SAMRS_ERR_BAD_SHAPE;
    if (!idx_ok(idx, n_oc, K, stream)) return SAMRS_ERR_BAD_ARG;
    KRET(launch_outlier_weight_ext(prec, W, N, K, idx, n_oc, out, ld, col0, (hipStream_t)stream));
}
int samrs_k_outlier_side_weight(int prec, const float* W1, const float* b1, int n_rows1, int D, const int32_t* idx2, int n2, const int32_t* idx1,
                                int n1, void* out, int Ks, float* bias_out, void* stream) {
    if (!W1 || !b1 || !out || n_rows1 < 1 || D < 1 || n2 < 1 || n2 > 32 || n1 < 0 || n1 > 32 || Ks < D + (n1 ? 64 : 0)) return SAMRS_ERR_BAD_SHAPE;
    if (!idx_ok(idx2, n2, n_rows1, stream) || !idx_ok(idx1, n1, D, stream)) return SAMRS_ERR_BAD_ARG;
    KRET(launch_outlier_side_weight(prec, W1, b1, D, idx2, n2, idx1, n1, out, Ks, bias_out, (hipStream_t)stream));
}
int samrs_k_outlier_gather(const void* hi, const void* lo, int D, const int32_t* idx, int n_oc, void* out, int rows, void* stream) {
    if (!hi || !lo || !out || D < 1 || n_oc < 1 || n_oc > 32 || rows < 1) return SAMRS_ERR_BAD_SHAPE;
    if (!idx_ok(idx, n_oc, D, stream)) return SAMRS_ERR_BAD_ARG;
    KRET(launch_outlier_gather(hi, lo, D, idx, n_oc, out, rows, (hipStream_t)stream));
}
int samrs_k_outlier_side_gemm(int prec, const void* Y, int lda, const void* Ws, const float* bias, int M, int K, void* out, void* stream) {
    if (!Y || !Ws || !bias || !out || !aligned16(Y) || !aligned16(Ws)) return SAMRS_ERR_BAD_ARG;
    if (M < 64 || M % 64 || K < 32 || K % 32 || lda < K || lda % 8) return SAMRS_ERR_BAD_SHAPE;
    KRET(launch_outlier_side_gemm(prec, Y, lda, Ws, bias, M, K, out, (hipStream_t)stream));
}
int samrs_k_weight_norms(const float* W, int N, int K, float* col_sq, float* row_sq, void* stream) {
    if (!W || (!col_sq && !row_sq)) return SAMRS_ERR_BAD_ARG;
    if (N < 1 || K < 1) return SAMRS_ERR_BAD_SHAPE;
    KRET(launch_weight_norms(W, N, K, col_sq, row_sq, (hipStream_t)stream));
}
int samrs_k_range_scan(int prec, const void* x, int64_t n, int cols, int ld, uint64_t* counter, void* stream) {
    if (!x || !counter || !aligned16(x)) return SAMRS_ERR_BAD_ARG;
    if (n < 0 || n % 8 || (cols > 0 && (cols % 8 || ld % 8 || ld < cols || n % cols))) return SAMRS_ERR_BAD_SHAPE;
    KRET(launch_range_scan(prec, x, (long)n, reinterpret_cast<unsigned long long*>(counter), (hipStream_t)stream, cols, ld));
}
int samrs_k_neck_im2col(const void* in, void* A, int n_images, int grid, int C, void* stream) {
    if (!in || !A || n_images < 1 || grid < 1 || C < 8 || C % 8) return SAMRS_ERR_BAD_ARG;
    KRET(launch_neck_im2col(in, A, n_images, grid, C, (hipStream_t)stream));
}
int samrs_k_gemm_f32_batch(const float* const* A, const float* const* A2, const float* const* W, const float* const* bias, float* const* C,
                           int count, int lda, int ldc, int M, int N, int K, int relu, int accumulate, void* stream) {
    if (!A || !W || !bias || !C || count < 1 || count > F32_BATCH_MAX) return SAMRS_ERR_BAD_ARG;
    if (M < 1 || N < 1 || K < 16 || K % 16 || lda % 4 || lda < K || ldc < N) return SAMRS_ERR_BAD_ARG;
    F32Batch bt{};
    for (int z = 0; z < count; ++z) {
        const float* a2 = A2 ? A2[z] : nullptr;
        if (!A[z] || !W[z] || !C[z] || !aligned16(A[z]) || !aligned16(a2) || !aligned16(W[z])) return SAMRS_ERR_BAD_ARG;
        bt.A[z] = A[z]; bt.A2[z] = a2; bt.W[z] = W[z]; bt.bias[z] = bias[z]; bt.C[z] = C[z];
// ... 191 lines not shown
```

### samrs_amd/csrc/engine_state.h

```cpp
#pragma once
#include <cstdarg>
#include <cstdio>
#include <cstring>
#include <map>
#include <string>
#include <utility>
#include <vector>

#include "../../include/samrs_hip.h"
#include "../../include/samrs_hip_internal.h"
#include "common.h"
#include "kernels.h"

namespace samrs_detail {
struct DevTensor {
    float* p = nullptr;
    std::vector<int64_t> shape;
    size_t numel = 0;
};

enum { SPLIT_PATCH = 1, SPLIT_NECK = 2, SPLIT_OI = 4, SPLIT_UP = 8, SPLIT_DEFAULT = 15, SPLIT_ATTN = 16, SPLIT_MLP = 32, SPLIT_ATTN_V = 64,
       SPLIT_LIN2 = 128, SPLIT_ATTN_ANY = SPLIT_ATTN | SPLIT_ATTN_V, SPLIT_ALL = 255 };

struct DecAttn {
// ... 48 lines not shown

struct samrs_engine {
    samrs_config cfg{};
    int device = 0;
    int prec = 0;
    bool finalized = false;
    std::string err;
    std::map<std::string, DevTensor> w;
    std::vector<void*> owned;

    int grid = 64, tokens = 4096, D = 0, C = 256, hd = 0, nwin = 5;
    int T_max = 0;
    bool decoder_fusion = true, ln_fold = false;
    int split = SPLIT_DEFAULT;
    int split_ready = SPLIT_DEFAULT;
    int gemm_variant = -1;
    int split_depth = 0;
    bool split_passes = false;
    int lo_format = 0;
    bool mx_ready = false;
    int mx_gp = 0, mx_kp_proj = 0;
    bool mx_mlp_ready = false;
    int mx_kp_lin2 = 0;
    unsigned char *H4[2] = {nullptr, nullptr}, *SH4[2] = {nullptr, nullptr};
    unsigned char *Y4[2] = {nullptr, nullptr}, *SY4[2] = {nullptr, nullptr};
    unsigned char *AO4[2] = {nullptr, nullptr}, *SAO4[2] = {nullptr, nullptr};
    bool upscaler_fused = true;

    std::vector<EncBlock> blocks;
    uint16_t *patch_w = nullptr, *neck0_w = nullptr, *neck2_w = nullptr;
    uint16_t *patch_w_lo = nullptr, *neck0_w_lo = nullptr, *neck2_w_lo = nullptr;
    float* X = nullptr;
    uint16_t* Y = nullptr;
    float* STATS = nullptr;
    float* ROWSTAT = nullptr;
    bool can_fold = false;
    uint16_t* QKV = nullptr;
    uint16_t* AO = nullptr;
    uint16_t *Ylo = nullptr, *AOlo = nullptr, *Hlo = nullptr;
    float* F32T = nullptr;
    uint16_t* VTG = nullptr;
    uint16_t* H = nullptr;
    float* N1 = nullptr;
    uint16_t* N1e = nullptr;
    float* EMB = nullptr;
    std::vector<char> slot_set;
    std::vector<int> slot_split, slot_depth;
    int grade_multimask = 0;
    bool allow_reduced = false;
    int ln_tail = 0;
    unsigned int* ln_counters = nullptr;
    int operand_pad_on = 1;
    int ldk = 0;
    int outlier_on = 7 , outlier_ratio_pct = 400, outlier_blocks = 0, outlier_columns = 0;
    int outlier_dominant_blocks = 0;
    float* oc_scratch = nullptr;
    uint16_t* OCX = nullptr;
    bool oc_resid = false;
    int gelu_fast = -1;
    int range_check = 0;
    unsigned long long* range_counter = nullptr;
    unsigned long long range_seen = 0;
    struct AuditSite { std::string name; int columns; size_t col_off; };
    std::vector<AuditSite> audit_sites;
    size_t audit_columns = 0;
    int range_profile = 0, audit_passes = 0;
    long long* audit_rows = nullptr;
    double* audit_sumsq = nullptr;
    uint32_t* audit_maxbits = nullptr;
    float* audit_partials = nullptr;
    std::vector<long long> audit_col_rows;

    std::vector<DecLayer> layers;
    DecAttn fin{};
    DecWeights dec{};
    uint16_t* fin_kv_w = nullptr;
    float *fin_kv_b = nullptr, *fin_pe = nullptr;
    uint16_t *up1_w = nullptr, *up2_w = nullptr, *up1_w_lo = nullptr, *up2_w_lo = nullptr;
    float *up1_b = nullptr, *up2_b = nullptr, *up_ln = nullptr;
    float* PE = nullptr;

    float *TOK0 = nullptr, *Q = nullptr, *TA = nullptr, *TQ = nullptr, *TK = nullptr, *TV = nullptr, *TO = nullptr;
    float *MH = nullptr, *QP = nullptr, *KT = nullptr, *VT = nullptr, *O128 = nullptr, *T2IW = nullptr;
    float *K0F = nullptr;
    uint16_t* K0E = nullptr;
    uint16_t* KVQ0 = nullptr;
    int decode_prompts = 0;
    int decode_alloc = 0;
    size_t decode_bytes = 0;
    float* KF = nullptr;
    uint16_t* KE = nullptr;
    uint16_t* KE_lo = nullptr;
    float* DENSE = nullptr;
    int* SLOT_OF = nullptr;
    uint16_t* KVQ = nullptr;
    uint16_t* OI = nullptr;
    float* U1raw = nullptr;
    uint16_t* U1 = nullptr;
    uint16_t* U2 = nullptr;
    float *HY1 = nullptr, *HY2 = nullptr, *HYPER = nullptr, *IOU = nullptr, *LOW = nullptr;

    DeviceScratch rle_scratch;
    DeviceScratch rle_decode_scratch;
    DeviceScratch region_scratch;
    DeviceScratch box_scratch;
    DeviceScratch poly_scratch;
// ... 89 lines not shown
```

### samrs_amd/csrc/gemm.hip

```cpp
#include "gemm_device.h"
#include "gemm_families.h"


int gemm_fam::cu_count_now() {
    int dev = 0, n = 256;
    if (hipGetDevice(&dev) == hipSuccess) (void)hipDeviceGetAttribute(&n, hipDeviceAttributeMultiprocessorCount, dev);
    return n > 0 ? n : 256;
}
int gemm_fam::cu_count() {
    static const int n = cu_count_now();
    return n;
}

namespace {


template <int PREC, int GELU, int JC = 4, bool DRAIN = false, bool FOLD = false, bool MXO = false, bool STREAM = false >
__device__ __forceinline__ void epilogue_pair_et(f32x4_t (&acc)[5][8], unsigned char* lds, void* __restrict__ Cv,
                                                 const float* __restrict__ bias, const float* __restrict__ pre2d, int period, int N,
                                                 int m_base , int n_pair ,
                                                 int wm, int wn, int lane, const float2* __restrict__ rowstat = nullptr ,
                                                 const float* __restrict__ cvec = nullptr , MxOut mxo = MxOut()) {
    constexpr int RS = 400;
    constexpr int TS = 16 * RS;
    const int fr = lane & 15, fq = lane >> 4, half = wn & 1;
    unsigned char* scr = lds + (wm * 2 + (wn >> 1)) * (JC * TS);
    float4 bv[5];
#pragma unroll
    for (int i = 0; i < 5; ++i)
        bv[i] = bias ? *reinterpret_cast<const float4*>(bias + n_pair + half * 80 + i * 16 + 4 * fq) : make_float4(0.f, 0.f, 0.f, 0.f);
    float2 rs_cur[JC], rs_nxt[JC];
    if constexpr (FOLD) {
#pragma unroll
        for (int jj = 0; jj < JC; ++jj) rs_cur[jj] = rowstat[m_base + jj * 16 + fr];
    }
#pragma unroll
    for (int j0 = 0; j0 < 8; j0 += JC) {
        if (j0) __syncthreads();
        if constexpr (FOLD) {
            if (j0 + JC < 8) {
#pragma unroll
                for (int jj = 0; jj < JC; ++jj) rs_nxt[jj] = rowstat[m_base + (j0 + JC + jj) * 16 + fr];
            }
        }
#pragma unroll
        for (int jj = 0; jj < JC; ++jj) {
            const int j = j0 + jj;
            float2 rs = make_float2(1.f, 0.f);
            if constexpr (FOLD) rs = rs_cur[jj];
            float mxh[MXO ? 24 : 1], mxl[MXO ? 24 : 1];
#pragma unroll
            for (int i = 0; i < 5; ++i) {
                float v0 = acc[i][j][0] + bv[i].x, v1 = acc[i][j][1] + bv[i].y;
                float v2 = acc[i][j][2] + bv[i].z, v3 = acc[i][j][3] + bv[i].w;
                if constexpr (FOLD) {
                    const float4 cv = *reinterpret_cast<const float4*>(cvec + n_pair + half * 80 + i * 16 + 4 * fq);
                    v0 = fmaf(rs.x, acc[i][j][0], fmaf(rs.y, cv.x, bv[i].x)); v1 = fmaf(rs.x, acc[i][j][1], fmaf(rs.y, cv.y, bv[i].y));
                    v2 = fmaf(rs.x, acc[i][j][2], fmaf(rs.y, cv.z, bv[i].z)); v3 = fmaf(rs.x, acc[i][j][3], fmaf(rs.y, cv.w, bv[i].w));
                }
                if (pre2d) {
                    const float4 e = *reinterpret_cast<const float4*>(pre2d + (size_t)((m_base + j * 16 + fr) % period) * N + n_pair +
                                                                      half * 80 + i * 16 + 4 * fq);
                    v0 += e.x; v1 += e.y; v2 += e.z; v3 += e.w;
                }
                if constexpr (GELU == 2) { const float2_t g01 = gelu_erf2_et(float2_t{v0, v1}), g23 = gelu_erf2_et(float2_t{v2, v3}); v0 = g01.x; v1 = g01.y; v2 = g23.x; v3 = g23.y; }
                else if constexpr (GELU != 0) { const float2_t g01 = gelu_erf2(float2_t{v0, v1}), g23 = gelu_erf2(float2_t{v2, v3}); v0 = g01.x; v1 = g01.y; v2 = g23.x; v3 = g23.y; }
                uint2 o;
                o.x = pack2<PREC>(v0, v1);
                o.y = pack2<PREC>(v2, v3);
                *reinterpret_cast<uint2*>(scr + jj * TS + fr * RS + half * 160 + (i * 16 + 4 * fq) * 2) = o;
                if constexpr (MXO) {
                    const float vv[4] = {v0, v1, v2, v3};
#pragma unroll
                    for (int e = 0; e < 4; ++e) {
                        const float hv = ET<PREC>::to_float((uint16_t)(((e & 2) ? o.y : o.x) >> (16 * (e & 1))));
                        mxh[4 * i + e] = hv;
                        mxl[4 * i + e] = vv[e] - hv;
                    }
                }
            }
            if constexpr (MXO) {
#pragma unroll
                for (int e = 20; e < 24; ++e) { mxh[e] = 0.f; mxl[e] = 0.f; }
                const int row = m_base + j * 16 + fr;
                const int wt = (n_pair + half * 80) / 80, nblk = (N / 80) * 3;
                const size_t rowb = (size_t)row * (size_t)(nblk * 16);
#pragma unroll
                for (int b3 = 0; b3 < 3; ++b3) {
                    float ah = 0.f, al = 0.f;
#pragma unroll
                    for (int e = 0; e < 8; ++e) { ah = fmaxf(ah, fabsf(mxh[8 * b3 + e])); al = fmaxf(al, fabsf(mxl[8 * b3 + e])); }
                    ah = fmaxf(ah, lane_xor16(ah)); al = fmaxf(al, lane_xor16(al));
                    ah = fmaxf(ah, lane_xor32(ah)); al = fmaxf(al, lane_xor32(al));
                    const int bh = mx_scale_byte(ah), bl = mx_scale_byte(al);
                    const size_t at = rowb + (size_t)(wt * 3 + b3) * 16 + 4 * fq;
                    *reinterpret_cast<uint32_t*>(mxo.q_hi + at) = fp4_pack8(mxh + 8 * b3, bh);
                    *reinterpret_cast<uint32_t*>(mxo.q_lo + at) = fp4_pack8(mxl + 8 * b3, bl);
                    if (fq == 0) {
                        const size_t si = mx_scale_index(false, row, wt * 3 + b3, nblk * 32 / MXK);
                        mxo.s_hi[si] = (unsigned char)bh;
                        mxo.s_lo[si] = (unsigned char)bl;
                    }
                }
            }
        }
        if (DRAIN && j0 == 0) asm volatile("s_waitcnt vmcnt(0)" ::: "memory");
        __syncthreads();
#pragma unroll
        for (int h = 0; h < JC * 160 / 64; ++h) {
            const int idx = lane + 64 * h;
            const int jj = idx / 160, rem = idx % 160;
            const int row = 8 * half + rem / 20, ch = rem % 20;
            const uint4 v = *reinterpret_cast<const uint4*>(scr + jj * TS + row * RS + ch * 16);
            uint16_t* C = reinterpret_cast<uint16_t*>(Cv) + (size_t)(m_base + (j0 + jj) * 16 + row) * N + n_pair + ch * 8;
            store16_stream<STREAM>(C, v);
        }
        if constexpr (FOLD) {
#pragma unroll
            for (int jj = 0; jj < JC; ++jj) rs_cur[jj] = rs_nxt[jj];
        }
    }
}



template <int PREC, bool OUT_F32, bool GELU, int ABL = 0, int NI = 4>
__global__ __launch_bounds__(QTHREADS) void gemm_et_big_kernel(
    const uint16_t* __restrict__ A, const uint16_t* __restrict__ B, void* __restrict__ Cv,
    const float* __restrict__ bias, const float* __restrict__ add2d, int add2d_period,
    int M, int N, int K, int accumulate) {
    constexpr int QBN = 64 * NI;
    constexpr int QSTAGE_ELEMS = (QBM + QBN) * QBK;
    __shared__ __attribute__((aligned(16))) uint16_t lds[QSTAGES * QSTAGE_ELEMS];

    const int tid = threadIdx.x;
    const int lane = tid & 63;
    const int wave = __builtin_amdgcn_readfirstlane(tid >> 6);
    const int grp = wave >> 2;
    const int wm = wave >> 2, wn = wave & 3;

    constexpr int GROUP = 8;
    const int tiles_n = N / QBN, tiles_m = M / QBM;
    const int bid = xcd_remap(blockIdx.x, gridDim.x);
    const int per_group = GROUP * tiles_n;
    const int group = bid / per_group, first_m = group * GROUP;
    const int gsz = (tiles_m - first_m) < GROUP ? (tiles_m - first_m) : GROUP;
    const int in_g = bid - group * per_group;
    const int tile_m = first_m + in_g % gsz, tile_n = in_g / gsz;
    const int m0 = tile_m * QBM, n0 = tile_n * QBN;

    const int g_row = 16 * wave + (lane >> 2);
    const int g_chunk = qswz(g_row, lane & 3);
    const uint16_t* gAg = A + (size_t)(m0 + g_row) * K + g_chunk * 8;
    const uint16_t* gBg = B + (size_t)(n0 + g_row) * K + g_chunk * 8;
    const uint32_t wave_lds_base = __builtin_amdgcn_readfirstlane(
        (uint32_t)(uintptr_t)(__attribute__((address_space(3))) void*)lds + (uint32_t)wave * (16 * QBK * 2));
    const size_t rs128 = (size_t)128 * K;
#define BIG_ISSUE(kt_, stage_)                                                                  \
    do {                                                                                         \
        const size_t koff_ = (size_t)(kt_) * QBK;                                                \
// ... 368 lines not shown
        for (int sl = 0; sl < LNP; ++sl) LNT_LOAD(sl, row0 + sl)
        for (int g = 0; g < 32 / LNP; ++g) {
#pragma unroll
            for (int sl = 0; sl < LNP; ++sl) {
                const int row = row0 + g * LNP + sl;
                float sm = 0.f;
#pragma unroll
                for (int i = 0; i < LNV; ++i) {
                    const int idx = lane_t + 64 * i;
                    if (idx < nv) sm += (ring[sl][i].x + ring[sl][i].y) + (ring[sl][i].z + ring[sl][i].w);
                }
                const float mean = wave_sum(sm) / (float)N;
                float q = 0.f;
#pragma unroll
                for (int i = 0; i < LNV; ++i) {
                    const int idx = lane_t + 64 * i;
                    if (idx < nv) {
                        const float a = ring[sl][i].x - mean, b = ring[sl][i].y - mean, c = ring[sl][i].z - mean, d = ring[sl][i].w - mean;
                        q += (a * a + b * b) + (c * c + d * d);
                    }
                }
                const float rstd = 1.0f / sqrtf(wave_sum(q) / (float)N + ln.eps);
#pragma unroll
                for (int i = 0; i < LNV; ++i) {
                    const int idx = lane_t + 64 * i;
                    if (idx < nv) {
                        const float4 g4 = reinterpret_cast<const float4*>(ln.gamma)[idx];
                        const float4 bt = reinterpret_cast<const float4*>(ln.beta)[idx];
                        const float o0 = (ring[sl][i].x - mean) * rstd * g4.x + bt.x;
                        const float o1 = (ring[sl][i].y - mean) * rstd * g4.y + bt.y;
                        const float o2 = (ring[sl][i].z - mean) * rstd * g4.z + bt.z;
                        const float o3 = (ring[sl][i].w - mean) * rstd * g4.w + bt.w;
                        uint2 o;
                        o.x = pack2<PREC>(o0, o1);
                        o.y = pack2<PREC>(o2, o3);
                        reinterpret_cast<uint2*>(ln.out + (size_t)row * N)[idx] = o;
                    }
                }
                if (g + 1 < 32 / LNP) LNT_LOAD(sl, row + LNP)
            }
        }
#undef LNT_LOAD
    }
#undef X64_PIECE
#undef X64_SEL
#undef X64_ISSUE
#undef X64_READ
#undef X64_MFMA
#undef X64_MIDBAR
}


template <int PREC, bool OUT_F32, int GELU , bool FOLD = false,
          bool SPLIT3 = false, bool MXO = false, bool STREAM = false >
__global__ __launch_bounds__(QTHREADS) void gemm_et_x64p_kernel(
    const uint16_t* __restrict__ A, const uint16_t* __restrict__ B, void* __restrict__ Cv,
    const float* __restrict__ bias, int M, int N, int K, int accumulate,
    const float2* __restrict__ rowstat = nullptr, const float* __restrict__ cvec = nullptr,
    const uint16_t* __restrict__ A_lo = nullptr, const uint16_t* __restrict__ B_lo = nullptr, int split_from_n = 0,
    MxOut mxo = MxOut(), int ld = 0 ) {
    static_assert(!(FOLD && OUT_F32), "the folded LayerNorm feeds ET outputs only (qkv, lin1)");
    static_assert(!(FOLD && SPLIT3), "the split operands come from an explicit LayerNorm");
    static_assert(!(MXO && (FOLD || SPLIT3 || OUT_F32)), "MX rows go with the plain ET-output flavour");
    constexpr int NI = 5;
    constexpr int XBN = 64 * NI;
    constexpr int XROWS = QBM + XBN;
    constexpr int XSTAGE_ELEMS = XROWS * XBK;
    constexpr uint32_t XSB = XSTAGE_ELEMS * 2;
    constexpr int NPIECE = 4 + NI;
    __shared__ __attribute__((aligned(16))) uint16_t lds[2 * XSTAGE_ELEMS];

    const int tid = threadIdx.x;
    const int lane = tid & 63;
    const int wave = __builtin_amdgcn_readfirstlane(tid >> 6);
    const int grp = wave >> 2;
    const int wm = wave >> 2, wn = wave & 3;

    constexpr int GROUP = 8;
    const int tiles_n = N / XBN, tiles_m = M / QBM, ntiles = tiles_n * tiles_m;
    const int per_group = GROUP * tiles_n;
#define X64P_TILE(L_, m_, n_)                                                                    \
    do {                                                                                         \
        const int bid_ = xcd_remap((L_), ntiles);                                                \
        const int group_ = bid_ / per_group, first_m_ = group_ * GROUP;                           \
        const int gsz_ = (tiles_m - first_m_) < GROUP ? (tiles_m - first_m_) : GROUP;            \
        const int in_g_ = bid_ - group_ * per_group;                                             \
        (m_) = (first_m_ + in_g_ % gsz_) * QBM;                                                  \
        (n_) = (in_g_ / gsz_) * XBN;                                                             \
    } while (0)

    const int LD = ld > 0 ? ld : K;
    const int prow = 8 * wave + ((lane >> 2) & 7);
    const uint32_t voff = ((uint32_t)prow * (uint32_t)LD + (uint32_t)(lane >> 5) * 32u + (uint32_t)qswz(prow, lane & 3) * 8u) * 2u;
    const size_t rs64 = (size_t)64 * LD;
    const uint32_t lds0 = __builtin_amdgcn_readfirstlane(
        (uint32_t)(uintptr_t)(__attribute__((address_space(3))) void*)lds + (uint32_t)wave * 1024u);
    const uint16_t* sA;
    const uint16_t* sB;
    const uint16_t* sAl = nullptr;
    const uint16_t* sBl = nullptr;
    const int nst1 = K / XBK;
    int sb = 0;
#define X64P_PIECE(st_, wr_, q_)                                                                           \
    glds16_s(voff, ((q_) < 4 ? seg_src_a<SPLIT3>(sA, sAl, (st_) + sb, nst1) + (size_t)(q_) * rs64          \
                             : seg_src_b<SPLIT3>(sB, sBl, (st_) + sb, nst1) + (size_t)((q_) - 4) * rs64),  \
             lds0 + (wr_) + ((q_) < 4 ? (q_) * 8192u : (uint32_t)(QBM * XBK * 2) + ((q_) - 4) * 8192u))
#define X64P_ISSUE(st_, wr_)                                                                               \
    do {                                                                                                   \
        X64P_PIECE(st_, wr_, 0); X64P_PIECE(st_, wr_, 1); X64P_PIECE(st_, wr_, 2); X64P_PIECE(st_, wr_, 3); \
        X64P_PIECE(st_, wr_, 4); X64P_PIECE(st_, wr_, 5); X64P_PIECE(st_, wr_, 6); X64P_PIECE(st_, wr_, 7); \
        X64P_PIECE(st_, wr_, 8);                                                                           \
    } while (0)

    const int fr = lane & 15, fq = lane >> 4;
// ... 37 lines not shown
        const int nst = SPLIT3 ? 3 * nst1 - sb : nst1;
#pragma unroll
        for (int i = 0; i < NI; ++i)
#pragma unroll
            for (int j = 0; j < 8; ++j) acc[i][j] = f32x4_t{0.f, 0.f, 0.f, 0.f};
        if (grp == 1) {
            if (nst > 1) X64P_ISSUE(1, XSB);
            __builtin_amdgcn_s_barrier();
        }
        uint32_t rd = 0;
        for (int t = 0; t < nst; ++t) {
            uint4 fa[8], fb[NI];
            const uint32_t wr = XSB - rd;
            const bool dma0 = (grp == 0) && (t + 1 < nst);
            const bool dma1 = (grp == 1) && (t + 2 < nst);
            if (grp == 0) __builtin_amdgcn_s_barrier();
            X64P_READ(rd, 0)
            asm volatile("s_waitcnt lgkmcnt(0)" ::: "memory");
            __builtin_amdgcn_sched_barrier(0);
            __builtin_amdgcn_s_setprio(1);
            X64P_MFMA(dma0, t + 1, wr)
            __builtin_amdgcn_s_setprio(0);
            __builtin_amdgcn_sched_barrier(0);
            X64P_READ(rd, 1)
            asm volatile("s_waitcnt lgkmcnt(0)" ::: "memory");
            if (grp == 1) asm volatile("s_waitcnt vmcnt(0)" ::: "memory");
            __builtin_amdgcn_sched_barrier(0);
            if (grp == 1) __builtin_amdgcn_s_barrier();
            __builtin_amdgcn_s_setprio(1);
            X64P_MFMA(dma1, t + 2, rd)
            __builtin_amdgcn_s_setprio(0);
            if (grp == 0) asm volatile("s_waitcnt vmcnt(0)" ::: "memory");
            __builtin_amdgcn_sched_barrier(0);
            rd = wr;
        }
        if (grp == 0) __builtin_amdgcn_s_barrier();

        const int Ln = L + (int)gridDim.x;
        const bool more = Ln < ntiles;
        int m1 = m0, n1 = n0;
        if (more) {
            X64P_TILE(Ln, m1, n1);
            sA = A + (size_t)m1 * LD;
            sB = B + (size_t)n1 * LD;
            if constexpr (SPLIT3) { sAl = A_lo + (size_t)m1 * LD; sBl = B_lo + (size_t)n1 * LD; sb = n1 >= split_from_n ? 0 : 2 * nst1; }
            X64P_ISSUE(0, 0u);
        }
        {
            unsigned char* upper = reinterpret_cast<unsigned char*>(lds) + XSB;
            if constexpr (MXO) {
                epilogue_pair_et<PREC, GELU, 2, true, false, true>(acc, upper, Cv, bias, nullptr, 1, N, m0 + wm * 128, n0 + (wn >> 1) * 160, wm, wn,
                                                                   lane, nullptr, nullptr, mxo);
            } else if constexpr (!OUT_F32) {
                epilogue_pair_et<PREC, GELU, 2, true, FOLD, false, STREAM>(acc, upper, Cv, bias, nullptr, 1, N, m0 + wm * 128, n0 + (wn >> 1) * 160, wm, wn,
                                                                           lane, rowstat, cvec);
            } else {
                epilogue_coalesced<PREC, true, GELU != 0, 8, 1, NI, false, true>(acc, upper + wave * (XSB / 8), Cv, bias, nullptr, 1, N,
                                                                           m0 + wm * 128, n0 + wn * (16 * NI), accumulate, lane);
            }
        }
        if (!more) break;
        __builtin_amdgcn_s_barrier();
        L = Ln; m0 = m1; n0 = n1;
    }
#undef X64P_TILE
#undef X64P_PIECE
#undef X64P_ISSUE
#undef X64P_READ
#undef X64P_MFMA
}

static bool stream_hidden(long M, long N) {
    static const int mode = [] { const char* v = getenv("SAMRS_NT_HIDDEN"); return v ? atoi(v) : -1; }();
    if (mode >= 0) return mode != 0;
    return M * N * 2 >= (256L << 20);
}
template <int PREC>
hipError_t launch_gemm_x64p(const void* A, const void* B, void* C, const float* bias, int M, int N, int K, bool out_f32, bool gelu,
                            bool accumulate, int ld, int gelu_form, hipStream_t s) {
    const int ntiles = (M / QBM) * (N / WBN);
    const int n_cu = cu_count();
    dim3 grid(ntiles < n_cu ? ntiles : n_cu), block(QTHREADS);
    const uint16_t* a = reinterpret_cast<const uint16_t*>(A);
    const uint16_t* b = reinterpret_cast<const uint16_t*>(B);
    const int acc = accumulate ? 1 : 0;
    if (out_f32) {
        if (gelu) gemm_et_x64p_kernel<PREC, true, true><<<grid, block, 0, s>>>(a, b, C, bias, M, N, K, acc);
        else gemm_et_x64p_kernel<PREC, true, false><<<grid, block, 0, s>>>(a, b, C, bias, M, N, K, acc);
    } else {
        const bool so = gelu && stream_hidden(M, N);
#define X64P_ARGS a, b, C, bias, M, N, K, acc, nullptr, nullptr, nullptr, nullptr, 0, MxOut(), ld
        if (gelu && gelu_form == 2 && so) gemm_et_x64p_kernel<PREC, false, 2, false, false, false, true><<<grid, block, 0, s>>>(X64P_ARGS);
        else if (gelu && gelu_form == 2) gemm_et_x64p_kernel<PREC, false, 2><<<grid, block, 0, s>>>(X64P_ARGS);
        else if (gelu && so) gemm_et_x64p_kernel<PREC, false, true, false, false, false, true><<<grid, block, 0, s>>>(X64P_ARGS);
        else if (gelu) gemm_et_x64p_kernel<PREC, false, true><<<grid, block, 0, s>>>(X64P_ARGS);
        else gemm_et_x64p_kernel<PREC, false, false><<<grid, block, 0, s>>>(X64P_ARGS);
#undef X64P_ARGS
    }
    return hipGetLastError();
}

template <int PREC>
hipError_t launch_gemm_x64p_mxo(const void* A, const void* B, void* C, const float* bias, int M, int N, int K, bool gelu,
                                void* o4_hi, void* o4_lo, void* so_hi, void* so_lo, hipStream_t s) {
    const int ntiles = (M / QBM) * (N / WBN);
    const int n_cu = cu_count();
    dim3 grid(ntiles < n_cu ? ntiles : n_cu), block(QTHREADS);
    const uint16_t* a = reinterpret_cast<const uint16_t*>(A);
    const uint16_t* b = reinterpret_cast<const uint16_t*>(B);
    MxOut mxo;
    mxo.q_hi = reinterpret_cast<unsigned char*>(o4_hi);
    mxo.q_lo = reinterpret_cast<unsigned char*>(o4_lo);
    mxo.s_hi = reinterpret_cast<unsigned char*>(so_hi);
    mxo.s_lo = reinterpret_cast<unsigned char*>(so_lo);
    if (gelu) gemm_et_x64p_kernel<PREC, false, true, false, false, true><<<grid, block, 0, s>>>(a, b, C, bias, M, N, K, 0, nullptr, nullptr, nullptr, nullptr, 0, mxo);
    else gemm_et_x64p_kernel<PREC, false, false, false, false, true><<<grid, block, 0, s>>>(a, b, C, bias, M, N, K, 0, nullptr, nullptr, nullptr, nullptr, 0, mxo);
    return hipGetLastError();
}

template <int PREC, bool ZERO>
__device__ __forceinline__ void mfma16_asm(f32x4_t& c, const uint4& a, const uint4& b) {
    const u32x4_t av = __builtin_bit_cast(u32x4_t, a), bv = __builtin_bit_cast(u32x4_t, b);
    if constexpr (PREC == PREC_F16) {
        if constexpr (ZERO) asm volatile("v_mfma_f32_16x16x32_f16 %0, %1, %2, 0" : "=a"(c) : "v"(av), "v"(bv));
        else asm volatile("v_mfma_f32_16x16x32_f16 %0, %1, %2, %0" : "+a"(c) : "v"(av), "v"(bv));
    } else {
        if constexpr (ZERO) asm volatile("v_mfma_f32_16x16x32_bf16 %0, %1, %2, 0" : "=a"(c) : "v"(av), "v"(bv));
        else asm volatile("v_mfma_f32_16x16x32_bf16 %0, %1, %2, %0" : "+a"(c) : "v"(av), "v"(bv));
    }
}

constexpr int W4X_ROWS = QBM + W4X_BN;
constexpr int W4X_STAGE_ELEMS = W4X_ROWS * XBK;
constexpr int W4X_SCR_BYTES = 4 * 16 * 272;

template <int PREC, bool OUT_F32, int GELU, bool STREAM = false >
__global__ __attribute__((amdgpu_flat_work_group_size(W4THREADS, W4THREADS), amdgpu_waves_per_eu(1, 1))) void gemm_et_w4x_kernel(
    const uint16_t* __restrict__ A, const uint16_t* __restrict__ B, void* __restrict__ Cv,
    const float* __restrict__ bias, int M, int N, int K, int accumulate, int ld = 0 ) {
    static_assert(!OUT_F32, "ET outputs only (epilogue scratch: 16 rows x 272 B per wave)");
    constexpr int NI = 8, NJ = 8;
    constexpr uint32_t XSB = W4X_STAGE_ELEMS * 2;
    __shared__ __attribute__((aligned(16))) uint16_t lds[2 * W4X_STAGE_ELEMS + W4X_SCR_BYTES / 2];

    const int tid = threadIdx.x;
    const int lane = tid & 63;
    const int wave = __builtin_amdgcn_readfirstlane(tid >> 6);
    const int wm = wave >> 1, wn = wave & 1;

    constexpr int GROUP = 8;
    const int tiles_n = N / W4X_BN, tiles_m = M / QBM, ntiles = tiles_n * tiles_m;
// ... 587 lines not shown
#undef ABL_CASE
#undef XABL_CASE
    return hipGetLastError();
}
#endif

hipError_t launch_gemm_et(int prec, const void* A, const void* B, void* C, const float* bias,
                          const float* add2d, int add2d_period, int M, int N, int K, bool out_f32,
                          bool gelu, bool accumulate, hipStream_t s, GemmOpts opts) {
    if (add2d && add2d_period <= 0) return hipErrorInvalidValue;
    const GemmChoice ch = gemm_select(GemmCall{M, N, K, out_f32, gelu, accumulate, add2d != nullptr, opts.ld, prec == PREC_F16}, gemm_env());
    if (ch.reject) return hipErrorInvalidValue;
    return with_prec(prec, [&](auto P) -> hipError_t {
        constexpr int PR = P.value;
        auto x64 = [&](auto NI, auto MODE) {
            return launch_gemm_x64<PR, NI.value, MODE.value>(A, B, C, bias, add2d, add2d_period, M, N, K, out_f32, gelu, accumulate, s);
        };
        switch (ch.kernel) {
            case GemmKernel::BASE: return gemm_fam::base(prec, ch.glds, ch.group_m, A, B, C, bias, add2d, add2d_period, M, N, K, out_f32, gelu, accumulate, s);
            case GemmKernel::STAG: return gemm_fam::stag(prec, A, B, C, bias, add2d, add2d_period, M, N, K, out_f32, gelu, accumulate, s);
            case GemmKernel::DUAL: return gemm_fam::dual(prec, true, A, B, C, bias, add2d, add2d_period, M, N, K, out_f32, gelu, accumulate, s);
            case GemmKernel::DUAL_LOCKSTEP: return gemm_fam::dual(prec, false, A, B, C, bias, add2d, add2d_period, M, N, K, out_f32, gelu, accumulate, s);
            case GemmKernel::STAG_256x256: return launch_gemm_big<PR>(A, B, C, bias, add2d, add2d_period, M, N, K, out_f32, gelu, accumulate, s);
            case GemmKernel::STAG_256x320: return launch_gemm_big<PR, 5>(A, B, C, bias, add2d, add2d_period, M, N, K, out_f32, gelu, accumulate, s);
            case GemmKernel::X64:
                switch (ch.ni * 8 + ch.mode) {
                    case 4 * 8 + 0: return x64(Int<4>{}, Int<0>{});
                    case 5 * 8 + 0: return x64(Int<5>{}, Int<0>{});
                    case 4 * 8 + 1: return x64(Int<4>{}, Int<1>{});
                    case 5 * 8 + 1: return x64(Int<5>{}, Int<1>{});
                    case 4 * 8 + 2: return x64(Int<4>{}, Int<2>{});
                    case 5 * 8 + 2: return x64(Int<5>{}, Int<2>{});
                    case 4 * 8 + 3: return x64(Int<4>{}, Int<3>{});
                    case 5 * 8 + 7: return x64(Int<5>{}, Int<7>{});
                    case 5 * 8 + 3: return x64(Int<5>{}, Int<3>{});
                }
                return hipErrorInvalidValue;
            case GemmKernel::X64P: return launch_gemm_x64p<PR>(A, B, C, bias, M, N, K, out_f32, gelu, accumulate, opts.ld, opts.gelu_form, s);
            case GemmKernel::W4X: return launch_gemm_w4x<PR>(A, B, C, bias, M, N, K, out_f32, gelu, accumulate, opts.ld, opts.gelu_form, s);
            case GemmKernel::K256: return gemm_fam::k256(prec, A, B, C, bias, add2d, add2d_period, M, N, s);
#ifdef SAMRS_EXPERIMENTS
            case GemmKernel::M32: return gemm_fam::m32(prec, ch.mode ? 1 : 0, A, B, C, bias, M, N, K, out_f32, gelu, accumulate, ch.persistent, s);
            case GemmKernel::W4: return gemm_fam::w4(prec, A, B, C, bias, M, N, K, out_f32, gelu, accumulate, ch.persistent, s);
            case GemmKernel::ABL_BIG:
            case GemmKernel::ABL_X64: return launch_gemm_abl(ch, A, B, C, bias, add2d, add2d_period, M, N, K, s);
#else
            default: break;
#endif
        }
        return hipErrorInvalidValue;
    });
}

bool gemm_has_experiments() {
#ifdef SAMRS_EXPERIMENTS
    return true;
#else
    return false;
#endif
}
#ifdef SAMRS_EXPERIMENTS
hipError_t gemm_fam::x64p_fold(int prec, const void* A, const void* B, void* C, const float* bias, const float* cvec, const float* rowstat,
                               int M, int N, int K, bool gelu, hipStream_t s) {
    return with_prec(prec, [&](auto P) { return launch_gemm_x64p_fold<P.value>(A, B, C, bias, cvec, rowstat, M, N, K, gelu, s); });
}
#endif

template <int PREC>
static hipError_t launch_gemm_split3_prec(const uint16_t* a, const uint16_t* al, const uint16_t* b, const uint16_t* bl, void* C,
                                          const float* bias, int M, int N, int K, bool out_f32, bool accumulate, int split_from_n,
                                          const float* add2d, int add2d_period, hipStream_t s) {
    if (out_f32) {
        if (N % WBN == 0)
            gemm_et_x64_kernel<PREC, true, false, 5, 3, 0, true><<<dim3((M / QBM) * (N / WBN)), dim3(QTHREADS), 0, s>>>(
                a, b, C, bias, add2d, add2d_period, M, N, K, accumulate ? 1 : 0, 0, al, bl);
        else
            gemm_et_x64_kernel<PREC, true, false, 4, 3, 0, true><<<dim3((M / QBM) * (N / QBN)), dim3(QTHREADS), 0, s>>>(
                a, b, C, bias, add2d, add2d_period, M, N, K, accumulate ? 1 : 0, 0, al, bl);
    } else {
        const int ntiles = (M / QBM) * (N / WBN);
        const int n_cu = cu_count_now();
        gemm_et_x64p_kernel<PREC, false, false, false, true><<<dim3(ntiles < n_cu ? ntiles : n_cu), dim3(QTHREADS), 0, s>>>(
            a, b, C, bias, M, N, K, 0, nullptr, nullptr, al, bl, split_from_n);
    }
    return hipGetLastError();
}

bool gemm_split3_ok(int M, int N, int K, bool out_f32) {
    return M > 0 && N > 0 && K > 0 && M % QBM == 0 && K % XBK == 0 && (N % WBN == 0 || (out_f32 && N % QBN == 0));
}

hipError_t launch_gemm_et_split3(int prec, const void* A, const void* A_lo, const void* B, const void* B_lo, void* C, const float* bias,
                                 int M, int N, int K, bool out_f32, bool accumulate, hipStream_t s, int split_from_n,
                                 const float* add2d, int add2d_period) {
    if (!gemm_split3_ok(M, N, K, out_f32) || !A || !A_lo || !B || !B_lo || (accumulate && !out_f32)) return hipErrorInvalidValue;
    if (split_from_n < 0 || split_from_n % WBN || (split_from_n && out_f32)) return hipErrorInvalidValue;
    if (add2d && (!out_f32 || add2d_period <= 0)) return hipErrorInvalidValue;
    const uint16_t* a = reinterpret_cast<const uint16_t*>(A);
    const uint16_t* al = reinterpret_cast<const uint16_t*>(A_lo);
    const uint16_t* b = reinterpret_cast<const uint16_t*>(B);
    const uint16_t* bl = reinterpret_cast<const uint16_t*>(B_lo);
    return with_prec(prec, [&](auto P) {
        return launch_gemm_split3_prec<P.value>(a, al, b, bl, C, bias, M, N, K, out_f32, accumulate, split_from_n, add2d, add2d_period, s);
    });
}

// ... 84 lines not shown
```

### samrs_amd/csrc/gemm_select.h

```cpp
#pragma once

namespace gemm_sel {

constexpr int BM = 128, BN = 128, BK = 64;
constexpr int PBM = 256;
constexpr int DBM = 256, DBN = 128, DBK = 32;
constexpr int QBM = 256, QBN = 256, QBK = 32;
constexpr int WBN = 320;
constexpr int XBK = 64;
constexpr int W4X_BN = 256;
constexpr int K2_ROWS = 128, K2_K = 256;

enum class GemmKernel {
    BASE,
    STAG,
    DUAL,
    DUAL_LOCKSTEP,
    STAG_256x256,
    STAG_256x320,
    X64,
    X64P,
    W4X,
    K256,
    M32,
// ... 98 lines not shown
        ch.persistent = v == 34;
        return ch;
    }
    if (v == 38 && !w4x_ok(M, N, K, c.has_add2d, c.out_f32)) v = pair;
    if (v == 38) return pick(GK::W4X);
    if (v == 28 && x64p_fits) return pick(GK::X64P);
    if ((v == 28 || v == 27) && x64_ok(M, N, K, 5)) {
        GemmChoice ch = pick(GK::X64);
        ch.ni = 5;
        ch.mode = 3;
        return ch;
    }
    const bool dual_fits = M % DBM == 0 && K % DBK == 0;
    if (v == 9 && dual_fits) return pick(GK::DUAL_LOCKSTEP);
    if (v == 7 && dual_fits) return pick(GK::DUAL);
    if ((v == 10 || v == 11) && M % QBM == 0 && N % WBN == 0 && K % QBK == 0) return pick(GK::STAG_256x320);
    if (v == 10 || v == 11) v = 5;
    if (v == 6 && M % QBM == 0 && N % QBN == 0 && K % QBK == 0) return pick(GK::STAG_256x256);
    if ((v == 5 || v == 6 || v == 7 || v == 9) && M % PBM == 0) return pick(GK::STAG);
    GemmChoice ch = pick(GK::BASE);
    ch.glds = !(gv == 0 || gv == 3);
    ch.group_m = (gv == 0 || gv == 1) ? 1 : 8;
    return ch;
}

inline bool gemm_takes_ld(GemmKernel k) { return k == GemmKernel::X64P || k == GemmKernel::W4X; }

inline GemmChoice gemm_select(const GemmCall& c, const GemmEnv& e) {
    GemmChoice no;
    no.reject = true;
    if (c.M <= 0 || c.N <= 0 || c.K <= 0 || c.M % BM || c.N % BN || c.K % BK) return no;
    if (c.has_add2d && c.gelu) return no;
    const GemmChoice ch = gemm_rule(c, e);
    if (c.ld != 0 && (c.ld < c.K || c.ld % 8 || e.variant != 8 || c.out_f32 || c.has_add2d || !gemm_takes_ld(ch.kernel))) return no;
    return ch;
}

inline bool gemm_is_x64_wide(const GemmChoice& ch) { return !ch.reject && ch.kernel == GemmKernel::X64 && ch.ni == 5 && ch.mode == 3; }
inline GemmChoice gemm_plan_choice(int M, int N, int K, bool out_f32, bool gelu, bool accumulate, GemmEnv e) {
    e.m32_mask = 0;
    return gemm_rule(GemmCall{M, N, K, out_f32, gelu, accumulate, false, 0, true}, e);
}
inline bool gemm_plan_ld_ok(int M, int N, int K, bool gelu, const GemmEnv& e) {
    const GemmChoice ch = gemm_plan_choice(M, N, K, false, gelu, false, e);
    return e.variant == 8 && !ch.reject && gemm_takes_ld(ch.kernel);
}
inline bool gemm_plan_ext_ok(int M, int N, int K, const GemmEnv& e) {
    return e.variant == 8 && K >= 2 * XBK && gemm_is_x64_wide(gemm_plan_choice(M, N, K, true, false, true, e));
}
inline bool gemm_plan_lntail_ok(int M, int N, int K, GemmEnv e) {
    e.variant = 8;
    return N <= 1280 && K >= 2 * XBK && gemm_is_x64_wide(gemm_plan_choice(M, N, K, true, false, true, e));
}

}
```

### samrs_amd/csrc/kernels.h

```cpp
#pragma once
#include <hip/hip_runtime.h>
#include <stdint.h>

struct GemmOpts {
    int ld = 0;
    int gelu_form = 1;
};
hipError_t launch_gemm_et(int prec, const void* A, const void* B, void* C, const float* bias,
                          const float* add2d, int add2d_period, int M, int N, int K, bool out_f32,
                          bool gelu, bool accumulate, hipStream_t s, GemmOpts opts = {});
void gemm_debug_choice(int prec, int M, int N, int K, bool out_f32, bool gelu, bool accumulate, bool has_add2d, int ld, int variant,
                       int32_t* out8);
hipError_t launch_gemm_et_gln(int prec, const void* A, const void* B, void* C, const float* bias, const float* gamma_beta,
                              int M, int N, int K, hipStream_t s, const void* A_lo = nullptr, const void* B_lo = nullptr);
hipError_t launch_gemm_et_stats(int prec, const void* A, const void* B, float* C, const float* bias, void* Xh, float* stats,
                                int M, int N, int K, hipStream_t s);
hipError_t launch_gemm_et_fold(int prec, const void* Xh, const void* Wf, void* C, const float* bias_f, const float* cvec,
                               const float* rowstat, int M, int N, int K, bool gelu, hipStream_t s);
bool gemm_split3_ok(int M, int N, int K, bool out_f32 = false);
hipError_t launch_gemm_et_split3(int prec, const void* A, const void* A_lo, const void* B, const void* B_lo, void* C, const float* bias,
                                 int M, int N, int K, bool out_f32, bool accumulate, hipStream_t s, int split_from_n = 0,
                                 const float* add2d = nullptr, int add2d_period = 0);
void set_gemm_variant(int v);
bool gemm_has_experiments();
bool gemm_lntail_ok(int M, int N, int K);
hipError_t launch_gemm_et_lntail(int prec, const void* A, const void* B, float* C, const float* bias, int M, int N, int K,
                                 const float* gamma, const float* beta, float eps, void* out_et, unsigned int* counters, hipStream_t s);
bool gemm_ld_ok(int M, int N, int K, bool gelu);
bool gemm_ext_ok(int M, int N, int K);
hipError_t launch_gemm_et_ext(int prec, const void* A, const void* B, const void* Ax, const void* Bx, float* C, const float* bias,
                              int M, int N, int K, hipStream_t s);
int swap_gemm_variant_override(int v);
void set_gemm_skew(int xcd_units, int cu_units);
hipError_t launch_gemm_f32(const float* A, int lda, const float* W, const float* bias, float* C,
                           int ldc, int M, int N, int K, bool relu, bool accumulate, hipStream_t s);
constexpr int F32_BATCH_MAX = 5;
struct F32Batch {
    const float* A[F32_BATCH_MAX];
    const float* A2[F32_BATCH_MAX];
    const float* W[F32_BATCH_MAX];
    const float* bias[F32_BATCH_MAX];
    float* C[F32_BATCH_MAX];
};
hipError_t launch_gemm_f32_batch(const F32Batch& bt, int count, int lda, int ldc, int M, int N, int K, bool relu,
                                 bool accumulate, hipStream_t s);

hipError_t launch_patch_im2col(int prec, const uint8_t* img, void* A, int n_images, int in_h, int in_w,
                               int grid, int patch, hipStream_t s, void* A_lo = nullptr);
hipError_t launch_convert(int prec, const float* in, void* out, long n, hipStream_t s, void* out_lo = nullptr);
hipError_t launch_ln_fold_weight(int prec, const float* W, const float* gamma, const float* beta, const float* bias, void* Wf,
                                 float* cvec, float* bias_f, int N, int K, hipStream_t s);
hipError_t launch_rowstats_convert(int prec, const float* X, void* Xh, float* stats, int rows, int D, hipStream_t s);
hipError_t launch_ln_rowstat(const float* stats, float* rowstat, int rows, float eps, hipStream_t s);
hipError_t launch_layernorm(int prec, const float* X, const float* gamma, const float* beta, float eps,
                            void* out_et, float* out_f32, int rows_out, int D, int window_mode, int grid,
                            int window, hipStream_t s, void* out_lo = nullptr,
                            void* mx_q_hi = nullptr, void* mx_q_lo = nullptr, void* mx_s_hi = nullptr, void* mx_s_lo = nullptr,
                            int ld_out = 0 ,
                            const int* oc_idx = nullptr, int n_oc = 0);
hipError_t launch_outlier_weight_ext(int prec, const float* W, int N, int K, const int* idx, int n_oc, void* out, int ld, int col0, hipStream_t s);
hipError_t launch_outlier_side_weight(int prec, const float* W1, const float* b1, int D, const int* idx2, int n2, const int* idx1, int n1,
                                      void* out, int Ks, float* bias_out, hipStream_t s);
hipError_t launch_outlier_gather(const void* hi, const void* lo, int D, const int* idx, int n_oc, void* out, int rows, hipStream_t s);
hipError_t launch_outlier_side_gemm(int prec, const void* Y, int lda, const void* Ws, const float* bias, int M, int K, void* out, hipStream_t s);
hipError_t launch_weight_norms(const float* W, int N, int K, float* col_sq, float* row_sq, hipStream_t s);
hipError_t launch_window_attention(int prec, const void* qkv, const float* qkv_bias, const float* rel_h, const float* rel_w, void* out,
                                   int n_images, int grid, int window, int heads, int head_dim, hipStream_t s, void* out_lo = nullptr,
                                   void* mx_q_hi = nullptr, void* mx_q_lo = nullptr, void* mx_s_hi = nullptr, void* mx_s_lo = nullptr,
                                   uint32_t lo_heads = 0xffffffffu);
hipError_t launch_gelu_split(int prec, const float* in, void* hi, void* lo, long n, hipStream_t s);
hipError_t launch_range_scan(int prec, const void* x, long n, unsigned long long* counter, hipStream_t s,
                             int cols = 0, int ld = 0 );
hipError_t launch_global_attention(int prec, const void* qkv, const float* rel_h, const float* rel_w, void* out,
                                   int n_images, int grid, int heads, int head_dim, void* vt_ws, hipStream_t s, void* out_lo = nullptr,
                                   void* mx_q_hi = nullptr, void* mx_q_lo = nullptr, void* mx_s_hi = nullptr, void* mx_s_lo = nullptr);
hipError_t launch_neck_im2col(const void* in, void* A, int n_images, int grid, int C, hipStream_t s);
hipError_t launch_transpose_f32(const float* in, float* out, int rows, int cols, hipStream_t s);

constexpr int AUDIT_PROFILE_WORDS = 48;
constexpr int AUDIT_ROWS_PER_PARTIAL = 256;
hipError_t launch_range_profile(int prec, const void* x, long n, int cols, int ld, long long* row48, hipStream_t s);
size_t column_stats_partial_floats(int M, int K);
hipError_t launch_column_stats(int prec, const void* x, int M, int K, int ld, float* partials, double* sumsq, uint32_t* maxbits, hipStream_t s);

struct PromptParams {
    const float* boxes;
    const float* point_coords;
    const int32_t* point_labels;
    int n_prompts, n_points;
    float img_size;
    const float* gauss;
    const float* point_emb[4];
    const float* not_a_point;
    const float* iou_token;
    const float* mask_tokens;
};
hipError_t launch_prompt_tokens(const PromptParams& p, float* tokens, float* tokens2 , int T, hipStream_t s);
hipError_t launch_dense_pe(const float* gauss, float* pe , int grid, hipStream_t s);
struct MaskEmbedParams {
    const float *w0, *b0, *ln1w, *ln1b, *w3, *b3, *ln4w, *ln4b, *w6, *b6;
};
hipError_t launch_mask_embed(const MaskEmbedParams& p, const float* mask_in, float* dense, int n, int grid, hipStream_t s);
hipError_t launch_fill_slot_table(const int* start, const int* slot, int n_runs, int* out, hipStream_t s);
hipError_t launch_make_keys(int prec, const float* emb, const float* dense, const float* vec, float* out_f32,
                            void* out_et, int n_batches, int tokens, int C, hipStream_t s, const int* slot_of = nullptr);
hipError_t launch_add_f32(const float* a, const float* b, float* out, long n, hipStream_t s);
hipError_t launch_token_self_attn(const float* q, const float* k, const float* v, float* o, int n, int T, int C,
                                  int heads, hipStream_t s);
constexpr int T2I_MAX_SPLITS = 16;
size_t t2i_workspace_floats(int n_prompts, int T);
hipError_t launch_t2i_attention(int prec, const float* qp, const void* kp, const void* vp, int ld, long batch_stride_rows,
                                float* out, float* workspace, int n, int T, int tokens, int Ci, int heads, hipStream_t s,
                                const int* slot_of = nullptr);
hipError_t launch_i2t_attention(int prec, const void* qi, int ld, long batch_stride_rows, const float* kt,
                                const float* vt, void* out, int n, int T, int tokens, int Ci, int heads, hipStream_t s);
hipError_t launch_group_ln_gelu(int prec, const float* in, const float* gamma, const float* beta, float eps,
                                void* out, long rows, int groups, int gsize, hipStream_t s);
hipError_t launch_upscale2_masks(int prec, const void* u1, const void* w, const void* w_lo, const float* bias, const float* hyper,
                                 float* low, int n, int grid, int n_mask_tokens, int sel0, int n_sel, hipStream_t s);
hipError_t launch_mask_product(int prec, const void* up2, const float* hyper, float* low, int n, int grid,
                               int n_mask_tokens, int sel0, int n_sel, hipStream_t s);
hipError_t launch_postprocess(const float* low, int n_masks, int in_h, int in_w, int orig_h, int orig_w,
                              int img_size, int return_logits, void* out, hipStream_t s);
hipError_t launch_paint(const uint8_t* masks, const int32_t* labels, int n, int h, int w, uint8_t* seg,
                        unsigned long long* areas, unsigned long long* class_pixels,
                        unsigned long long* class_instances, int n_classes, hipStream_t s);
hipError_t launch_select_best(const uint8_t* masks, const float* iou, int n, int nsel, int h, int w, uint8_t* out, float* quality,
                              unsigned long long* areas, hipStream_t s);
// ... 126 lines not shown
```

### samrs_amd/engine.py

```python
from __future__ import annotations

import contextlib
import ctypes as C
import os
from typing import Dict, List, Optional, Sequence, Tuple

import numpy as np
import torch

from .synth import SamConfig

_HERE = os.path.dirname(os.path.abspath(__file__))
LIB_PATH = os.path.join(_HERE, "csrc", "libsamrs_hip.so")

PREC_BF16, PREC_F16 = 0, 1
PRECISIONS = {"bf16": PREC_BF16, "f16": PREC_F16, "fp16": PREC_F16}

ABI_VERSION = 5
POLYGON_EPS_Q_MAX = 16384
REGION_MODES = {"holes": 1, "islands": 2, "both": 3}
OVERLAP_RULES = {"logit": 1, "smallest": 2, "priority": 3}
SPLIT_PATCH, SPLIT_NECK, SPLIT_OI, SPLIT_UP, SPLIT_DEFAULT = 1, 2, 4, 8, 15
SPLIT_ATTN, SPLIT_MLP, SPLIT_ATTN_V, SPLIT_LIN2, SPLIT_ALL = 16, 32, 64, 128, 255

# ... 145 lines not shown
    lib.samrs_k_prompt_tokens.argtypes = [vp, vp, vp, ip, ip, fp, vp, vp, vp, vp, vp, vp, vp, ip, vp]
    lib.samrs_k_dense_pe.argtypes = [vp, vp, ip, vp]
    lib.samrs_k_mask_embed.argtypes = [vp] * 12 + [ip, ip, vp]
    lib.samrs_k_fill_slot_table.argtypes = [C.POINTER(C.c_int32), C.POINTER(C.c_int32), ip, vp, vp]
    lib.samrs_k_make_keys.argtypes = [ip, vp, vp, vp, vp, vp, ip, ip, ip, vp, vp]
    lib.samrs_k_token_self_attn.argtypes = [vp, vp, vp, vp, ip, ip, ip, ip, vp]
    lib.samrs_k_t2i_workspace_floats.argtypes = [ip, ip]
    lib.samrs_k_t2i_workspace_floats.restype = i64
    lib.samrs_k_t2i_attention.argtypes = [ip, vp, vp, vp, ip, i64, vp, vp, ip, ip, ip, ip, ip, vp, vp]
    lib.samrs_k_i2t_attention.argtypes = [ip, vp, ip, i64, vp, vp, vp, ip, ip, ip, ip, ip, vp]
    lib.samrs_k_i2t_fused.argtypes = [ip, vp, ip, i64, vp, vp, vp, vp, vp, vp, i64, vp, vp, fp, vp, vp, vp, ip, ip, ip, ip, ip, vp, vp]
    lib.samrs_k_group_ln_gelu.argtypes = [ip, vp, vp, vp, fp, vp, i64, ip, ip, vp]
    lib.samrs_k_mask_product.argtypes = [ip, vp, vp, vp, ip, ip, ip, ip, ip, vp]
    for name in ("samrs_k_prompt_tokens", "samrs_k_dense_pe", "samrs_k_mask_embed", "samrs_k_fill_slot_table", "samrs_k_make_keys",
                 "samrs_k_token_self_attn", "samrs_k_t2i_attention", "samrs_k_i2t_attention", "samrs_k_i2t_fused",
                 "samrs_k_group_ln_gelu", "samrs_k_mask_product", "samrs_debug_copy_buffer", "samrs_debug_outlier_columns"):
        getattr(lib, name).restype = ip
    lib.samrs_debug_copy_buffer.argtypes = [vp, C.c_char_p, vp, C.c_size_t, vp]
    lib.samrs_debug_outlier_columns.argtypes = [vp, ip, ip, C.POINTER(C.c_int32)]
    if hasattr(lib, "samrs_debug_gemm_choice"):
        lib.samrs_debug_gemm_choice.argtypes = [ip] * 10 + [C.POINTER(C.c_int32)]
        lib.samrs_debug_gemm_choice.restype = None
    lib.samrs_get_slot_info.argtypes = [vp, ip, C.POINTER(C.c_int32), C.POINTER(C.c_int32), C.POINTER(C.c_int32)]
    lib.samrs_audit_site_count.argtypes = [vp, C.POINTER(ip)]
    lib.samrs_audit_site_name.argtypes = [vp, ip, C.c_char_p, ip, C.POINTER(ip)]
    lib.samrs_audit_read_profile.argtypes = [vp, vp, ip]
    lib.samrs_audit_read_columns.argtypes = [vp, ip, vp, vp, C.POINTER(C.c_int64)]
    lib.samrs_k_range_profile.argtypes = [ip, vp, C.c_long, ip, ip, vp, vp]
    lib.samrs_k_column_stats.argtypes = [ip, vp, ip, ip, ip, vp, vp, vp, vp]
    lib.samrs_k_audit_rows_per_partial.argtypes = []
    for name in ("samrs_audit_site_count", "samrs_audit_site_name", "samrs_audit_read_profile", "samrs_audit_read_columns",
                 "samrs_k_range_profile", "samrs_k_column_stats", "samrs_k_audit_rows_per_partial"):
        getattr(lib, name).restype = ip
    if hasattr(lib, "samrs_k_gemm_ext"):
        lib.samrs_k_gemm_ld.argtypes = [ip, vp, vp, vp, vp, ip, ip, ip, ip, ip, ip, vp]
        lib.samrs_k_gemm_ext.argtypes = [ip, vp, vp, vp, vp, vp, vp, ip, ip, ip, vp]
        lib.samrs_k_layernorm_ext.argtypes = [ip, vp, vp, vp, fp, vp, ip, ip, ip, vp, ip, ip, vp]
        lib.samrs_k_outlier_weight_ext.argtypes = [ip, vp, ip, ip, vp, ip, vp, ip, ip, vp]
        lib.samrs_k_outlier_side_weight.argtypes = [ip, vp, vp, ip, ip, vp, ip, vp, ip, vp, ip, vp, vp]
        lib.samrs_k_outlier_gather.argtypes = [vp, vp, ip, vp, ip, vp, ip, vp]
        lib.samrs_k_outlier_side_gemm.argtypes = [ip, vp, ip, vp, vp, ip, ip, vp, vp]
        lib.samrs_k_weight_norms.argtypes = [vp, ip, ip, vp, vp, vp]
        lib.samrs_k_range_scan.argtypes = [ip, vp, i64, ip, ip, vp, vp]
        for name in ("samrs_k_gemm_ld", "samrs_k_gemm_ext", "samrs_k_layernorm_ext", "samrs_k_outlier_weight_ext", "samrs_k_outlier_side_weight",
                     "samrs_k_outlier_gather", "samrs_k_outlier_side_gemm", "samrs_k_weight_norms", "samrs_k_range_scan"):
            getattr(lib, name).restype = ip
    if hasattr(lib, "samrs_k_gemm_f32_batch"):
        lib.samrs_k_gemm_f32_batch.argtypes = [vp, vp, vp, vp, vp, ip, ip, ip, ip, ip, ip, ip, ip, vp]
        lib.samrs_k_patch_im2col.argtypes = [ip, vp, vp, vp, ip, ip, ip, ip, ip, vp]
        lib.samrs_k_transpose_f32.argtypes = [vp, vp, ip, ip, vp]
        lib.samrs_k_gelu_split.argtypes = [ip, vp, vp, vp, i64, vp]
        for name in ("samrs_k_gemm_f32_batch", "samrs_k_patch_im2col", "samrs_k_transpose_f32", "samrs_k_gelu_split"):
            getattr(lib, name).restype = ip
    for name in ("samrs_load_weight", "samrs_finalize_weights", "samrs_set_images", "samrs_set_images_ragged", "samrs_get_embedding",
                 "samrs_set_embedding", "samrs_reset_image", "samrs_predict", "samrs_predict_multi", "samrs_paint", "samrs_k_gemm",
                 "samrs_k_gemm_f32", "samrs_k_convert", "samrs_k_layernorm", "samrs_k_window_attention",
                 "samrs_k_window_attention_lo", "samrs_k_global_attention", "samrs_k_postprocess", "samrs_k_gemm_gln", "samrs_k_upscale2_masks",
                 "samrs_k_gemm_stats", "samrs_k_gemm_fold", "samrs_k_ln_fold_weight", "samrs_k_rowstats_convert", "samrs_k_ln_rowstat",
                 "samrs_set_option", "samrs_get_option", "samrs_rle_encode", "samrs_k_convert_split", "samrs_select_best", "samrs_gt_match",
                 "samrs_png_encode_labels", "samrs_k_upscaler_fused", "samrs_k_gemm_split3", "samrs_get_slot_info"):
        getattr(lib, name).restype = ip
    if lib.samrs_abi_version() != ABI_VERSION:
        raise ImportError("libsamrs_hip.so ABI version mismatch; rebuild it")
    _lib = lib
    return lib


RLE_STATUS = ("OK", "ABSENT", "RANGE", "BAD_CHAR", "TRUNCATED", "BAD_COUNT", "BAD_SUM")


PNG_RGB_BLOCK_BYTES = 1 << 20


def png_rgb_bound(h: int, w: int) -> int:
    n = (3 * int(w) + 1) * int(h)
    blocks = -(-n // PNG_RGB_BLOCK_BYTES)
    return (63 + -(-(9 * n + blocks * (4498 + 9)) // 8) + 15) & ~15


def _ptr(t: Optional[torch.Tensor]) -> Optional[int]:
    return None if t is None else t.data_ptr()


def _stream() -> int:
    return torch.cuda.current_stream().cuda_stream


class EngineError(RuntimeError):
    pass


def multi_call_args(slots: Sequence[int], counts: Sequence[int], input_sizes: Sequence[Sequence[int]],
                    original_sizes: Sequence[Sequence[int]], n_rows: int) -> Tuple[List[int], List[int], List[int], List[int]]:
    n_img = len(slots)
    if n_img < 1:
        raise ValueError("predict_multi needs at least one image")
    if not (len(counts) == len(input_sizes) == len(original_sizes) == n_img):
        raise ValueError(f"predict_multi: {n_img} slots but {len(counts)} prompt counts, {len(input_sizes)} input sizes and "
                         f"{len(original_sizes)} original sizes")
    offsets = [0]
    for c in counts:
        if int(c) < 0:
            raise ValueError(f"predict_multi: negative prompt count {c}")
        offsets.append(offsets[-1] + int(c))
    if offsets[-1] != n_rows:
        raise ValueError(f"predict_multi: the prompt counts sum to {offsets[-1]} but the prompt tensors have {n_rows} rows")
# ... 93 lines not shown

    def get_slot_info(self, slot: int = 0) -> Dict[str, int]:
        a, b, c = C.c_int32(), C.c_int32(), C.c_int32()
        self._check(self.lib.samrs_get_slot_info(self.handle, slot, C.byref(a), C.byref(b), C.byref(c)))
        return {"is_set": int(a.value), "split": int(b.value), "split_depth": int(c.value)}

    def close(self) -> None:
        if getattr(self, "handle", None):
            self.lib.samrs_destroy(self.handle)
            self.handle = None

    def __del__(self):
        try:
            self.close()
        except Exception:
            pass

    def load_state_dict(self, sd: Dict[str, torch.Tensor]) -> None:
        for name, t in sd.items():
            a = np.ascontiguousarray(t.detach().to(torch.float32).cpu().numpy())
            shape = (C.c_int64 * a.ndim)(*a.shape)
            self._check(self.lib.samrs_load_weight(self.handle, name.encode(), a.ctypes.data, shape, a.ndim))
        with torch.cuda.device(self.device):
            self._check(self.lib.samrs_finalize_weights(self.handle, _stream()))

    def set_images(self, images_u8: torch.Tensor, slot0: int = 0) -> None:
        assert images_u8.dtype == torch.uint8 and images_u8.dim() == 4 and images_u8.shape[-1] == 3
        assert images_u8.is_cuda and images_u8.is_contiguous()
        n, h, w, _ = images_u8.shape
        with torch.cuda.device(self.device):
            self._check(self.lib.samrs_set_images(self.handle, images_u8.data_ptr(), n, h, w, slot0, _stream()))
        if self._audit_done is not None:
            self._audit_poll()

    def set_images_ragged(self, images_u8, slot0: int = 0) -> None:
        n = len(images_u8)
        for t in images_u8:
            assert t.dtype == torch.uint8 and t.dim() == 3 and t.shape[-1] == 3 and t.is_cuda and t.is_contiguous()
        ptrs = (C.c_void_p * n)(*[t.data_ptr() for t in images_u8])
        hs = (C.c_int * n)(*[int(t.shape[0]) for t in images_u8])
        ws = (C.c_int * n)(*[int(t.shape[1]) for t in images_u8])
        with torch.cuda.device(self.device):
            self._check(self.lib.samrs_set_images_ragged(self.handle, ptrs, hs, ws, n, slot0, _stream()))
        if self._audit_done is not None:
            self._audit_poll()

    def debug_encoder_prefix(self, images_u8: torch.Tensor, n_blocks: int) -> torch.Tensor:
        n, h, w, _ = images_u8.shape
        out = torch.empty(n, self.cfg.grid, self.cfg.grid, self.cfg.embed_dim, dtype=torch.float32, device=self.device)
        with torch.cuda.device(self.device):
            self._check(self.lib.samrs_debug_encoder_prefix(self.handle, images_u8.data_ptr(), n, h, w, n_blocks,
                                                            out.data_ptr(), _stream()))
        return out

    def outlier_columns(self, block: int, gemm: int):
        buf = (C.c_int32 * 32)()
        n = self.lib.samrs_debug_outlier_columns(self.handle, block, gemm, buf)
        if n < 0:
            self._check(n)
        return [int(buf[i]) for i in range(n)]

    PROFILE_WORDS = 48

    def audit_sites(self) -> List[Tuple[str, int]]:
        n, k = C.c_int(), C.c_int()
        self._check(self.lib.samrs_audit_site_count(self.handle, C.byref(n)))
        buf = C.create_string_buffer(64)
        out = []
        for i in range(n.value):
            self._check(self.lib.samrs_audit_site_name(self.handle, i, buf, 64, C.byref(k)))
            out.append((buf.value.decode(), int(k.value)))
        return out

    def range_profile(self, reset: bool = False) -> np.ndarray:
        rows = np.zeros((len(self.audit_sites()), self.PROFILE_WORDS), dtype=np.int64)
        self._check(self.lib.samrs_audit_read_profile(self.handle, rows.ctypes.data, int(bool(reset))))
        return rows

    def column_stats(self, site) -> Dict[str, object]:
        sites = self.audit_sites()
        if isinstance(site, str):
            names = [s[0] for s in sites]
            if site not in names:
                raise KeyError(f"no audit site {site!r}")
            site = names.index(site)
        k = sites[site][1] if 0 <= site < len(sites) else 0
        sumsq, max_abs, n_rows = np.zeros(max(k, 1), np.float64), np.zeros(max(k, 1), np.float32), C.c_int64()
        self._check(self.lib.samrs_audit_read_columns(self.handle, int(site), sumsq.ctypes.data, max_abs.ctypes.data, C.byref(n_rows)))
        return {"sumsq": sumsq, "max_abs": max_abs, "n_rows": int(n_rows.value)}

    def start_audit(self, passes: int, done=None) -> None:
        self.set_option("audit_passes", int(passes))
        self._audit_done = done if passes > 0 else None

    def _audit_poll(self) -> None:
        if self.get_option("audit_passes") == 0:
            done, self._audit_done = self._audit_done, None
            done(self)

    def debug_copy_buffer(self, name: str, dst: torch.Tensor) -> torch.Tensor:
        if not dst.is_contiguous() or dst.device != torch.device(self.device):
            raise ValueError("debug_copy_buffer: dst must be a contiguous tensor on the engine's device")
        with torch.cuda.device(self.device):
            self._check(self.lib.samrs_debug_copy_buffer(self.handle, name.encode(), dst.data_ptr(), dst.numel() * dst.element_size(),
                                                         _stream()))
        return dst
# ... 48 lines not shown
            n = int(boxes.shape[0])
        if mask_input is not None:
            side = 4 * self.cfg.grid
            if mask_input.dim() != 4 or tuple(mask_input.shape[1:]) != (1, side, side):
                raise ValueError(f"mask_input must be Bx1x{side}x{side}, got {tuple(mask_input.shape)}")
            if n is not None and mask_input.shape[0] != n:
                raise ValueError(f"mask_input has batch {mask_input.shape[0]} but the other prompts have {n}")
            mask_input = mask_input.to(**f32).contiguous()
            n = int(mask_input.shape[0])
        if n is None:
            raise AssertionError("at least one prompt (points, boxes or mask_input) is required")
        return boxes, point_coords, point_labels, mask_input, n

    def predict(self, slot: int, boxes: Optional[torch.Tensor], point_coords: Optional[torch.Tensor],
                point_labels: Optional[torch.Tensor], mask_input: Optional[torch.Tensor], multimask_output: bool,
                return_logits: bool, input_size: Tuple[int, int], original_size: Tuple[int, int],
                want_masks: bool = True) -> Tuple[Optional[torch.Tensor], torch.Tensor, torch.Tensor]:
        dev = self.device
        f32 = dict(dtype=torch.float32, device=dev)
        boxes, point_coords, point_labels, mask_input, n = self._prompt_arrays(boxes, point_coords, point_labels, mask_input)
        if n < 1:
            raise ValueError("empty prompt batch")
        npts = 0 if point_coords is None else point_coords.shape[1]
        c = 3 if multimask_output else 1
        oh, ow = int(original_size[0]), int(original_size[1])
        masks = None
        if want_masks:
            masks = torch.empty(n, c, oh, ow, dtype=torch.float32 if return_logits else torch.uint8, device=dev)
        iou = torch.empty(n, c, **f32)
        low = torch.empty(n, c, 256, 256, **f32)
        with torch.cuda.device(dev):
            self._check(self.lib.samrs_predict(
                self.handle, slot, n, _ptr(boxes), _ptr(point_coords), _ptr(point_labels), npts, _ptr(mask_input),
                int(bool(multimask_output)), int(bool(return_logits)), int(input_size[0]), int(input_size[1]), oh, ow,
                _ptr(masks), iou.data_ptr(), low.data_ptr(), _stream()))
        if masks is not None and not return_logits:
            masks = masks.view(torch.bool)
        return masks, iou, low

    def predict_multi(self, slots: Sequence[int], counts: Sequence[int], boxes: Optional[torch.Tensor],
                      point_coords: Optional[torch.Tensor], point_labels: Optional[torch.Tensor], mask_input: Optional[torch.Tensor],
                      multimask_output: bool, return_logits: bool, input_sizes: Sequence[Tuple[int, int]],
                      original_sizes: Sequence[Tuple[int, int]], want_masks: bool = True):
        rows = _prompt_rows(boxes, point_coords, mask_input)
        slots, offsets, in_hw, orig_hw = multi_call_args(slots, counts, input_sizes, original_sizes, rows if rows is not None else 0)
        n_img, counts = len(slots), [offsets[i + 1] - offsets[i] for i in range(len(slots))]
        boxes, point_coords, point_labels, mask_input, n = self._prompt_arrays(boxes, point_coords, point_labels, mask_input)
        dev = self.device
        f32 = dict(dtype=torch.float32, device=dev)
        npts = 0 if point_coords is None else point_coords.shape[1]
        c = 3 if multimask_output else 1
        masks = [None] * n_img
        if want_masks:
            masks = [torch.empty(counts[i], c, orig_hw[2 * i], orig_hw[2 * i + 1],
                                 dtype=torch.float32 if return_logits else torch.uint8, device=dev) for i in range(n_img)]
        iou = torch.empty(n, c, **f32)
        low = torch.empty(n, c, 256, 256, **f32)
        if n > 0:
            ia = C.c_int * n_img
            mptr = (C.c_void_p * n_img)(*[m.data_ptr() if m is not None and m.numel() else None for m in masks])
            with torch.cuda.device(dev):
                self._check(self.lib.samrs_predict_multi(
                    self.handle, n_img, ia(*slots), (C.c_int * (n_img + 1))(*offsets), _ptr(boxes), _ptr(point_coords),
                    _ptr(point_labels), npts, _ptr(mask_input), int(bool(multimask_output)), int(bool(return_logits)),
                    (C.c_int * (2 * n_img))(*in_hw), (C.c_int * (2 * n_img))(*orig_hw), mptr, iou.data_ptr(), low.data_ptr(),
                    _stream()))
        if want_masks and not return_logits:
            masks = [m.view(torch.bool) for m in masks]
        return masks, list(torch.split(iou, counts)), list(torch.split(low, counts))

    def rle_encode(self, masks: torch.Tensor, out: torch.Tensor, cursor: torch.Tensor, table: torch.Tensor) -> None:
        m = masks.view(torch.uint8) if masks.dtype == torch.bool else masks
        m = m.reshape(-1, m.shape[-2], m.shape[-1]).contiguous()
        n, h, w = m.shape
        assert out.dtype == torch.uint8 and out.is_cuda and out.is_contiguous() and out.data_ptr() % 16 == 0
        assert cursor.dtype == torch.int64 and cursor.is_cuda and table.dtype == torch.int64 and table.is_cuda
        assert table.is_contiguous() and table.numel() >= 3 * n
        with torch.cuda.device(self.device):
            self._check(self.lib.samrs_rle_encode(self.handle, m.data_ptr(), n, h, w, out.data_ptr(), out.numel(),
                                                  cursor.data_ptr(), table.data_ptr(), _stream()))

    def rle_decode(self, strings: torch.Tensor, table: torch.Tensor, size: Sequence[int], out: Optional[torch.Tensor] = None,
                   areas_out: Optional[torch.Tensor] = None, status_out: Optional[torch.Tensor] = None):
        h, w = int(size[0]), int(size[1])
        if not (isinstance(strings, torch.Tensor) and strings.dtype == torch.uint8 and strings.is_cuda and strings.is_contiguous() and strings.dim() == 1):
            raise ValueError("strings must be a contiguous uint8 [bytes] tensor on the engine's device")
        if not (isinstance(table, torch.Tensor) and table.dtype == torch.int64 and table.is_cuda and table.is_contiguous()
                and table.dim() == 2 and table.shape[1] == 3):
            raise ValueError("table must be a contiguous int64 [n, 3] tensor on the engine's device")
        n = int(table.shape[0])
        outs = []
        for name, t, shape, dt in (("out", out, (n, h, w), torch.uint8), ("areas_out", areas_out, (n,), torch.int64),
                                   ("status_out", status_out, (n,), torch.int32)):
            if t is None:
                t = torch.empty(shape, dtype=dt, device=self.device)
            elif not (isinstance(t, torch.Tensor) and t.dtype == dt and t.is_cuda and t.is_contiguous() and tuple(t.shape) == shape):
                raise ValueError(f"{name} must be a contiguous {dt} {list(shape)} tensor on the engine's device, or None")
            outs.append(t)
        with torch.cuda.device(self.device):
            self._check(self.lib.samrs_rle_decode(self.handle, _ptr(strings) if n else None, strings.numel(), _ptr(table) if n else None,
                                                  n, h, w, _ptr(outs[0]) if n else None, _ptr(outs[1]) if n else None,
                                                  _ptr(outs[2]) if n else None, _stream()))
        return outs[0], outs[1], outs[2]

    def png_encode(self, maps: torch.Tensor, lut: torch.Tensor, out: torch.Tensor, cursor: torch.Tensor, table: torch.Tensor) -> None:
        m = maps.reshape(-1, maps.shape[-2], maps.shape[-1]).contiguous()
        n, h, w = m.shape
        assert m.dtype == torch.uint8 and m.is_cuda
# ... 512 lines not shown
```

Measured before the change: 148.7.

## Emit V^T from QKV GEMM epilogue and batch postprocess/key launches

For global-attention blocks, the QKV GEMM epilogue now also writes the transposed V tile into the VTG workspace, so the separate vt_pack kernel is skipped. Postprocess launches for contiguous same-size image segments are merged into one launch, and per-image key preparation becomes a single launch. Python allocates one contiguous mask buffer that is split per image, which is what lets postprocess launches merge. This removes an extra read and write of V plus several kernel launches, at the cost of a more complex GEMM epilogue and extra stores in that kernel.

```diff
diff --git a/include/samrs_hip_internal.h b/include/samrs_hip_internal.h
--- a/include/samrs_hip_internal.h
+++ b/include/samrs_hip_internal.h
@@ -119,6 +119,11 @@
                               void* stream);
 int samrs_k_weight_norms(const float* W, int N, int K, float* col_sq, float* row_sq, void* stream);
 int samrs_k_range_scan(int prec, const void* x_et, int64_t n, int cols, int ld, uint64_t* counter, void* stream);
+int samrs_debug_gemm_vt_ok(int prec, int M, int N, int K, int ld, int tokens, int variant);
+int samrs_k_gemm_qkv_vt(int prec, const void* A_et, const void* B_et, void* C_et, const float* bias, int M, int N, int K, int ld, void* vt_et,
+                        int tokens, void* stream);
+int samrs_k_vt_pack(const void* qkv_et, void* vt_et, int n_images, int grid, int heads, int head_dim, void* stream);
+int samrs_debug_block_route(samrs_engine_t* e, int n_images, int block, int32_t* out4);
 int samrs_k_gemm_f32_batch(const float* const* A, const float* const* A2, const float* const* W, const float* const* bias, float* const* C,
                            int count, int lda, int ldc, int M, int N, int K, int relu, int accumulate, void* stream);
 int samrs_k_patch_im2col(int prec, const uint8_t* img_u8, void* A_et, void* A_lo_et, int n_images, int in_h, int in_w, int grid, int patch,
diff --git a/samrs_amd/csrc/encoder_kernels.hip b/samrs_amd/csrc/encoder_kernels.hip
--- a/samrs_amd/csrc/encoder_kernels.hip
+++ b/samrs_amd/csrc/encoder_kernels.hip
@@ -1535,10 +1535,12 @@
 
 template <int PREC, int HD>
 static hipError_t launch_glb(const void* qkv, const float* rh, const float* rw, void* out, int n_images,
-                             int heads, void* vt_ws, hipStream_t s, void* out_lo, MxOut mx) {
+                             int heads, void* vt_ws, hipStream_t s, void* out_lo, MxOut mx, bool vt_ready) {
     constexpr int NTOK = GlbCfg<HD>::G * GlbCfg<HD>::G;
-    vt_pack_kernel<HD><<<n_images * heads * (NTOK / 64), 256, 0, s>>>((const uint16_t*)qkv, (uint16_t*)vt_ws, heads, NTOK);
-    HIP_CHECK_RET(hipGetLastError());
+    if (!vt_ready) {
+        vt_pack_kernel<HD><<<n_images * heads * (NTOK / 64), 256, 0, s>>>((const uint16_t*)qkv, (uint16_t*)vt_ws, heads, NTOK);
+        HIP_CHECK_RET(hipGetLastError());
+    }
     if (mx.q_hi) return launch_glb_nw<PREC, HD, 8, 2>(qkv, rh, rw, out, n_images, heads, vt_ws, s, nullptr, mx);
     if (out_lo) return launch_glb_nw<PREC, HD, 8, 1>(qkv, rh, rw, out, n_images, heads, vt_ws, s, out_lo);
     if (g_glb_waves == 4) return launch_glb_nw<PREC, HD, 4>(qkv, rh, rw, out, n_images, heads, vt_ws, s);
@@ -1547,7 +1549,7 @@
 
 hipError_t launch_global_attention(int prec, const void* qkv, const float* rel_h, const float* rel_w, void* out,
                                    int n_images, int grid, int heads, int head_dim, void* vt_ws, hipStream_t s, void* out_lo,
-                                   void* mx_q_hi, void* mx_q_lo, void* mx_s_hi, void* mx_s_lo) {
+                                   void* mx_q_hi, void* mx_q_lo, void* mx_s_hi, void* mx_s_lo, bool vt_ready) {
     if (grid != 64 || !vt_ws) return hipErrorInvalidValue;
     MxOut mx;
     if (mx_q_hi) {
@@ -1555,13 +1557,22 @@
         mx.q_hi = (unsigned char*)mx_q_hi; mx.q_lo = (unsigned char*)mx_q_lo; mx.s_hi = (unsigned char*)mx_s_hi; mx.s_lo = (unsigned char*)mx_s_lo;
     }
     if (prec == PREC_BF16) {
-        if (head_dim == 64) return launch_glb<PREC_BF16, 64>(qkv, rel_h, rel_w, out, n_images, heads, vt_ws, s, out_lo, mx);
-        if (head_dim == 80) return launch_glb<PREC_BF16, 80>(qkv, rel_h, rel_w, out, n_images, heads, vt_ws, s, out_lo, mx);
+        if (head_dim == 64) return launch_glb<PREC_BF16, 64>(qkv, rel_h, rel_w, out, n_images, heads, vt_ws, s, out_lo, mx, vt_ready);
+        if (head_dim == 80) return launch_glb<PREC_BF16, 80>(qkv, rel_h, rel_w, out, n_images, heads, vt_ws, s, out_lo, mx, vt_ready);
     } else if (prec == PREC_F16) {
-        if (head_dim == 64) return launch_glb<PREC_F16, 64>(qkv, rel_h, rel_w, out, n_images, heads, vt_ws, s, out_lo, mx);
-        if (head_dim == 80) return launch_glb<PREC_F16, 80>(qkv, rel_h, rel_w, out, n_images, heads, vt_ws, s, out_lo, mx);
+        if (head_dim == 64) return launch_glb<PREC_F16, 64>(qkv, rel_h, rel_w, out, n_images, heads, vt_ws, s, out_lo, mx, vt_ready);
+        if (head_dim == 80) return launch_glb<PREC_F16, 80>(qkv, rel_h, rel_w, out, n_images, heads, vt_ws, s, out_lo, mx, vt_ready);
     }
     return hipErrorInvalidValue;
+}
+
+hipError_t launch_vt_pack(const void* qkv, void* vt_ws, int n_images, int grid, int heads, int head_dim, hipStream_t s) {
+    if (grid != 64 || !qkv || !vt_ws || n_images < 1 || heads < 1) return hipErrorInvalidValue;
+    const int ntok = grid * grid;
+    if (head_dim == 64) vt_pack_kernel<64><<<n_images * heads * (ntok / 64), 256, 0, s>>>((const uint16_t*)qkv, (uint16_t*)vt_ws, heads, ntok);
+    else if (head_dim == 80) vt_pack_kernel<80><<<n_images * heads * (ntok / 64), 256, 0, s>>>((const uint16_t*)qkv, (uint16_t*)vt_ws, heads, ntok);
+    else return hipErrorInvalidValue;
+    return hipGetLastError();
 }
 
 template <int PREC>
diff --git a/samrs_amd/csrc/engine.hip b/samrs_amd/csrc/engine.hip
--- a/samrs_amd/csrc/engine.hip
+++ b/samrs_amd/csrc/engine.hip
@@ -277,6 +277,7 @@
     e->gelu_fast = env_int("SAMRS_GELU_FAST", -1);
     e->ln_tail = env_int("SAMRS_LN_TAIL", 0) != 0;
     e->operand_pad_on = env_int("SAMRS_OPERAND_PAD", 1) != 0;
+    e->vt_from_qkv = env_int("SAMRS_VT_FROM_QKV", 1) != 0;
     e->outlier_on = env_int("SAMRS_OUTLIER_COLS", 7) & 7;
     e->outlier_ratio_pct = env_int("SAMRS_OUTLIER_RATIO_PCT", 400);
     if (e->outlier_ratio_pct < 101) e->outlier_ratio_pct = 101;
@@ -707,6 +708,7 @@
     else if (n == "gelu_fast") e->gelu_fast = value < 0 ? -1 : (value != 0);
     else if (n == "ln_tail") e->ln_tail = value > 0;
     else if (n == "operand_pad") e->operand_pad_on = value != 0;
+    else if (n == "vt_from_qkv") e->vt_from_qkv = value != 0;
     else if (n == "outlier_cols") e->outlier_on = value & 7;
     else if (n == "outlier_ratio_pct") {
         if (e->finalized) return fail(e, SAMRS_ERR_BAD_ARG, "outlier_ratio_pct: the columns are picked when the weights are finalized; set it before");
@@ -776,6 +778,7 @@
     else if (n == "gelu_fast") *value = e->gelu_fast;
     else if (n == "ln_tail") *value = e->ln_tail;
     else if (n == "operand_pad") *value = e->operand_pad_on;
+    else if (n == "vt_from_qkv") *value = e->vt_from_qkv;
     else if (n == "outlier_cols") *value = e->outlier_on;
     else if (n == "outlier_ratio_pct") *value = e->outlier_ratio_pct;
     else if (n == "outlier_blocks") *value = e->outlier_blocks;
diff --git a/samrs_amd/csrc/engine_decode.hip b/samrs_amd/csrc/engine_decode.hip
--- a/samrs_amd/csrc/engine_decode.hip
+++ b/samrs_amd/csrc/engine_decode.hip
@@ -225,10 +225,18 @@
 
 static int run_postprocess(samrs_engine_t* e, const DecodeRoute& r, const PredictImage* seg, int n_seg, const float* low, int return_logits,
                            hipStream_t s) {
-    for (int k = 0; k < n_seg; ++k)
-        if (seg[k].masks)
-            CK(e, launch_postprocess(low + (size_t)seg[k].p0 * r.nsel * 256 * 256, (seg[k].p1 - seg[k].p0) * r.nsel, seg[k].in_h, seg[k].in_w,
-                                     seg[k].orig_h, seg[k].orig_w, e->cfg.img_size, return_logits, seg[k].masks, s));
+    constexpr int MAX_MASKS = 65535;
+    for (int k = 0; k < n_seg;) {
+        if (!seg[k].masks) { ++k; continue; }
+        const size_t mask_bytes = (size_t)r.nsel * (size_t)seg[k].orig_h * (size_t)seg[k].orig_w * (return_logits ? 4 : 1);
+        int j = k + 1;
+        while (j < n_seg && seg[j].masks && seg[j].in_h == seg[k].in_h && seg[j].in_w == seg[k].in_w && seg[j].orig_h == seg[k].orig_h &&
+               seg[j].orig_w == seg[k].orig_w && seg[j].p0 == seg[j - 1].p1 && (seg[j].p1 - seg[k].p0) * r.nsel <= MAX_MASKS &&
+               seg[j].masks == (unsigned char*)seg[k].masks + (size_t)(seg[j].p0 - seg[k].p0) * mask_bytes) ++j;
+        CK(e, launch_postprocess(low + (size_t)seg[k].p0 * r.nsel * 256 * 256, (seg[j - 1].p1 - seg[k].p0) * r.nsel, seg[k].in_h, seg[k].in_w,
+                                 seg[k].orig_h, seg[k].orig_w, e->cfg.img_size, return_logits, seg[k].masks, s));
+        k = j;
+    }
     return SAMRS_OK;
 }
 
diff --git a/samrs_amd/csrc/engine_encode.hip b/samrs_amd/csrc/engine_encode.hip
--- a/samrs_amd/csrc/engine_encode.hip
+++ b/samrs_amd/csrc/engine_encode.hip
@@ -138,6 +138,7 @@
     int qkv_K = 0, qkv_ld = 0;
     int norm1_ld = 0;
     int y1_ld = 0, y1_live = 0;
+    bool vt_from_qkv = false;
     bool mx_ao = false;
     bool ao_lo = false;
     int nop = 0;
@@ -184,6 +185,8 @@
         r.y1_ld = r.qkv_ld ? r.qkv_ld : r.qkv_K;
         r.y1_live = r.qkv_K;
         r.norm1_ld = r.y1_ld == D ? 0 : r.y1_ld;
+        r.vt_from_qkv = b.global && e->vt_from_qkv && !e->range_check && !e->range_profile &&
+                        gemm_qkv_vt_ok(e->prec, M, 3 * D, r.qkv_K, r.qkv_ld, e->tokens);
     }
 
     r.mx_ao = sp_attn && mx_attn;
@@ -287,6 +290,8 @@
         if (!e->F32T) CK(e, dalloc(e, &e->F32T, (size_t)c.max_images * e->tokens * 4 * D));
         CK(e, gemm_hilo(prec, false, MainPass::LAST, e->Y, e->Ylo, b.qkv_w, b.qkv_w_lo, e->F32T, b.qkv_b, nullptr, 0, M, 3 * D, D, false, s));
         CK(e, launch_convert(prec, e->F32T, e->QKV, (long)M * 3 * D, s));
+    } else if (r.vt_from_qkv) {
+        CK(e, launch_gemm_et_qkv_vt(prec, e->Y, qkv_w, e->QKV, b.qkv_b, M, 3 * D, r.qkv_K, r.qkv_ld, e->VTG, e->tokens, s));
     } else {
         CK(e, launch_gemm_et(prec, e->Y, qkv_w, e->QKV, b.qkv_b, nullptr, 0, M, 3 * D, r.qkv_K, false, false, false, s, GemmOpts{r.qkv_ld, 1}));
     }
@@ -297,7 +302,7 @@
     else
         CK(e, launch_global_attention(prec, e->QKV, b.rel_h, b.rel_w, e->AO, n, g, c.num_heads, e->hd, e->VTG, s,
                                       r.ao_lo ? e->AOlo : nullptr, r.mx_ao ? e->AO4[0] : nullptr, r.mx_ao ? e->AO4[1] : nullptr,
-                                      r.mx_ao ? e->SAO4[0] : nullptr, r.mx_ao ? e->SAO4[1] : nullptr));
+                                      r.mx_ao ? e->SAO4[0] : nullptr, r.mx_ao ? e->SAO4[1] : nullptr, r.vt_from_qkv));
     if ((rc = range_scan(e, e->Y, (size_t)M * r.y1_live, s, r.y1_live, r.y1_ld))) return rc;
     if ((rc = range_scan(e, e->QKV, (size_t)M * 3 * D, s))) return rc;
     if ((rc = range_scan(e, e->AO, (size_t)M * D, s))) return rc;
@@ -384,10 +389,8 @@
 static int prepare_slot_keys(samrs_engine_t* e, int slot0, int n, hipStream_t s) {
     const int C = e->C, Ci = C / 2, tokens = e->tokens, prec = e->prec;
     const DecLayer& L = e->layers[0];
-    for (int i = 0; i < n; ++i) {
-        const size_t o = (size_t)(slot0 + i) * tokens * C;
-        CK(e, launch_make_keys(prec, e->EMB + o, nullptr, e->dec.no_mask_embed, e->K0F + o, e->K0E + o, 1, tokens, C, s));
-    }
+    const size_t o = (size_t)slot0 * tokens * C;
+    CK(e, launch_make_keys(prec, e->EMB + o, nullptr, e->dec.no_mask_embed, e->K0F + o, e->K0E + o, 1, n * tokens, C, s));
     CK(e, launch_gemm_et(prec, e->K0E + (size_t)slot0 * tokens * C, L.kvq_w, e->KVQ0 + (size_t)slot0 * tokens * 3 * Ci, L.kvq_b, L.kvq_pe,
                          tokens, n * tokens, 3 * Ci, C, false, false, false, s));
     return SAMRS_OK;
@@ -510,6 +513,18 @@
     return SAMRS_OK;
 }
 
+int samrs_debug_block_route(samrs_engine_t* e, int n_images, int block, int32_t* out4) {
+    if (!e || !out4) return SAMRS_ERR_BAD_ARG;
+    if (!e->finalized) return fail(e, SAMRS_ERR_BAD_WEIGHTS, "weights not finalized");
+    if (n_images < 1 || n_images > e->cfg.max_images || block < 0 || block >= (int)e->blocks.size())
+        return fail(e, SAMRS_ERR_BAD_ARG, "samrs_debug_block_route: n_images / block out of range");
+    ON_DEVICE(e);
+    const PassRoute p = pass_route(e, n_images * e->tokens, e->cfg.depth);
+    const BlockRoute r = block_route(e, p, e->blocks[block], block);
+    out4[0] = e->blocks[block].global ? 1 : 0; out4[1] = (int32_t)r.qkv; out4[2] = r.qkv_ld; out4[3] = r.vt_from_qkv ? 1 : 0;
+    return SAMRS_OK;
+}
+
 int samrs_get_embedding(samrs_engine_t* e, int slot, float* out_chw, void* stream) {
     if (!e || !out_chw) return fail(e, SAMRS_ERR_BAD_ARG, "samrs_get_embedding: null argument");
     if (slot < 0 || slot >= e->cfg.max_images) return fail(e, SAMRS_ERR_CAPACITY, "slot out of range");
diff --git a/samrs_amd/csrc/engine_hooks.hip b/samrs_amd/csrc/engine_hooks.hip
--- a/samrs_amd/csrc/engine_hooks.hip
+++ b/samrs_amd/csrc/engine_hooks.hip
@@ -21,6 +21,7 @@
     else if (n == "K0F") src = e->K0F; else if (n == "K0E") src = e->K0E; else if (n == "O128") src = e->O128;
     else if (n == "MH") src = e->MH; else if (n == "KT") src = e->KT; else if (n == "VT") src = e->VT; else if (n == "QP") src = e->QP;
     else if (n == "DENSE") src = e->DENSE;
+    else if (n == "AO") src = e->AO; else if (n == "VTG") src = e->VTG;
     else return fail(e, SAMRS_ERR_BAD_ARG, "unknown buffer %s", name);
     if (!src) return fail(e, SAMRS_ERR_BAD_ARG, "buffer %s is not allocated yet", name);
     CK(e, hipMemcpyAsync(dst, src, bytes, hipMemcpyDeviceToDevice, (hipStream_t)stream));
@@ -181,6 +182,17 @@
     if (M < 1 || N < 1 || K < 1 || !gemm_ext_ok(M, N, K)) return SAMRS_ERR_BAD_SHAPE;
     KRET(launch_gemm_et_ext(prec, A, B, Ax, Bx, C, bias, M, N, K, (hipStream_t)stream));
 }
+int samrs_debug_gemm_vt_ok(int prec, int M, int N, int K, int ld, int tokens, int variant) { return gemm_debug_vt_ok(prec, M, N, K, ld, tokens, variant); }
+int samrs_k_gemm_qkv_vt(int prec, const void* A, const void* B, void* C, const float* bias, int M, int N, int K, int ld, void* vt, int tokens,
+                        void* stream) {
+    if (!A || !B || !C || !vt || !aligned16(A) || !aligned16(B) || !aligned16(C) || !aligned16(vt) || ld < 0) return SAMRS_ERR_BAD_ARG;
+    if (!gemm_qkv_vt_ok(prec, M, N, K, ld, tokens)) return SAMRS_ERR_BAD_SHAPE;
+    KRET(launch_gemm_et_qkv_vt(prec, A, B, C, bias, M, N, K, ld, vt, tokens, (hipStream_t)stream));
+}
+int samrs_k_vt_pack(const void* qkv, void* vt, int n_images, int grid, int heads, int head_dim, void* stream) {
+    if (!qkv || !vt || !aligned16(qkv) || !aligned16(vt) || n_images < 1 || heads < 1) return SAMRS_ERR_BAD_ARG;
+    KRET(launch_vt_pack(qkv, vt, n_images, grid, heads, head_dim, (hipStream_t)stream));
+}
 int samrs_k_layernorm_ext(int prec, const float* X, const float* gamma, const float* beta, float eps, void* out_et, int rows, int D, int ld_out,
                           const int32_t* oc_idx, int n_oc, int window_mode, void* stream) {
     if (!X || !gamma || !beta || !out_et || !aligned16(X) || !aligned16(gamma) || !aligned16(beta) || !aligned16(out_et)) return SAMRS_ERR_BAD_ARG;
diff --git a/samrs_amd/csrc/engine_state.h b/samrs_amd/csrc/engine_state.h
--- a/samrs_amd/csrc/engine_state.h
+++ b/samrs_amd/csrc/engine_state.h
@@ -124,6 +124,7 @@
     unsigned int* ln_counters = nullptr;
     int operand_pad_on = 1;
     int ldk = 0;
+    int vt_from_qkv = 1;
     int outlier_on = 7 , outlier_ratio_pct = 400, outlier_blocks = 0, outlier_columns = 0;
     int outlier_dominant_blocks = 0;
     float* oc_scratch = nullptr;
diff --git a/samrs_amd/csrc/gemm.hip b/samrs_amd/csrc/gemm.hip
--- a/samrs_amd/csrc/gemm.hip
+++ b/samrs_amd/csrc/gemm.hip
@@ -15,12 +15,20 @@
 namespace {
 
 
-template <int PREC, int GELU, int JC = 4, bool DRAIN = false, bool FOLD = false, bool MXO = false, bool STREAM = false >
+struct VtOut {
+    uint16_t* vt = nullptr;
+    int tokens = 0;
+    int from = 0;
+};
+template <int PREC, int GELU, int JC = 4, bool DRAIN = false, bool FOLD = false, bool MXO = false, bool STREAM = false ,
+          bool VT = false>
 __device__ __forceinline__ void epilogue_pair_et(f32x4_t (&acc)[5][8], unsigned char* lds, void* __restrict__ Cv,
                                                  const float* __restrict__ bias, const float* __restrict__ pre2d, int period, int N,
                                                  int m_base , int n_pair ,
                                                  int wm, int wn, int lane, const float2* __restrict__ rowstat = nullptr ,
-                                                 const float* __restrict__ cvec = nullptr , MxOut mxo = MxOut()) {
+                                                 const float* __restrict__ cvec = nullptr , MxOut mxo = MxOut(), VtOut vt = VtOut()) {
+    static_assert(!VT || JC == 2, "a V^T pass is 32 tokens: four 8-key chunks of one half of a 64-key tile");
+    static_assert(!(VT && (FOLD || MXO)), "V^T goes with the plain ET-output flavour");
     constexpr int RS = 400;
     constexpr int TS = 16 * RS;
     const int fr = lane & 15, fq = lane >> 4, half = wn & 1;
@@ -106,6 +114,27 @@
         }
         if (DRAIN && j0 == 0) asm volatile("s_waitcnt vmcnt(0)" ::: "memory");
         __syncthreads();
+        if constexpr (VT) {
+            if (n_pair >= vt.from) {
+                const int tok = m_base % vt.tokens + j0 * 16;
+                const int c4 = lane & 3;
+                const unsigned char* col = scr + half * 160 + (lane >> 2) * 2 + (c4 >> 1) * TS + (c4 & 1) * (4 * RS);
+                uint16_t* dst = vt.vt + (size_t)(m_base + j0 * 16 - tok) * (size_t)(vt.from >> 1) +
+                                (size_t)(n_pair - vt.from + half * 80 + (lane >> 2)) * (size_t)vt.tokens + tok + c4 * 8;
+                const size_t step = (size_t)16 * (size_t)vt.tokens;
+#pragma nounroll
+                for (int h = 0; h < 5; ++h, col += 32, dst += step) {
+                    auto key = [&](int k) -> uint32_t { return *reinterpret_cast<const uint16_t*>(col + k * RS); };
+                    uint4 o;
+                    o.x = key(0) | (key(1) << 16);
+                    o.y = key(2) | (key(3) << 16);
+                    o.z = key(8) | (key(9) << 16);
+                    o.w = key(10) | (key(11) << 16);
+                    *reinterpret_cast<uint4*>(dst) = o;
+                }
+                continue;
+            }
+        }
 #pragma unroll
         for (int h = 0; h < JC * 160 / 64; ++h) {
             const int idx = lane + 64 * h;
@@ -580,14 +609,17 @@
 
 
 template <int PREC, bool OUT_F32, int GELU , bool FOLD = false,
-          bool SPLIT3 = false, bool MXO = false, bool STREAM = false >
+          bool SPLIT3 = false, bool MXO = false, bool STREAM = false ,
+          bool VT = false >
 __global__ __launch_bounds__(QTHREADS) void gemm_et_x64p_kernel(
     const uint16_t* __restrict__ A, const uint16_t* __restrict__ B, void* __restrict__ Cv,
     const float* __restrict__ bias, int M, int N, int K, int accumulate,
     const float2* __restrict__ rowstat = nullptr, const float* __restrict__ cvec = nullptr,
     const uint16_t* __restrict__ A_lo = nullptr, const uint16_t* __restrict__ B_lo = nullptr, int split_from_n = 0,
-    MxOut mxo = MxOut(), int ld = 0 ) {
+    MxOut mxo = MxOut(), int ld = 0 ,
+    VtOut vt = VtOut() ) {
     static_assert(!(FOLD && OUT_F32), "the folded LayerNorm feeds ET outputs only (qkv, lin1)");
+    static_assert(!(VT && (OUT_F32 || GELU != 0 || FOLD || SPLIT3 || MXO || STREAM)), "V^T goes with the plain ET-output flavour (qkv)");
     static_assert(!(FOLD && SPLIT3), "the split operands come from an explicit LayerNorm");
     static_assert(!(MXO && (FOLD || SPLIT3 || OUT_F32)), "MX rows go with the plain ET-output flavour");
     constexpr int NI = 5;
@@ -731,8 +763,8 @@
                 epilogue_pair_et<PREC, GELU, 2, true, false, true>(acc, upper, Cv, bias, nullptr, 1, N, m0 + wm * 128, n0 + (wn >> 1) * 160, wm, wn,
                                                                    lane, nullptr, nullptr, mxo);
             } else if constexpr (!OUT_F32) {
-                epilogue_pair_et<PREC, GELU, 2, true, FOLD, false, STREAM>(acc, upper, Cv, bias, nullptr, 1, N, m0 + wm * 128, n0 + (wn >> 1) * 160, wm, wn,
-                                                                           lane, rowstat, cvec);
+                epilogue_pair_et<PREC, GELU, 2, true, FOLD, false, STREAM, VT>(acc, upper, Cv, bias, nullptr, 1, N, m0 + wm * 128, n0 + (wn >> 1) * 160,
+                                                                               wm, wn, lane, rowstat, cvec, MxOut(), vt);
             } else {
                 epilogue_coalesced<PREC, true, GELU != 0, 8, 1, NI, false, true>(acc, upper + wave * (XSB / 8), Cv, bias, nullptr, 1, N,
                                                                            m0 + wm * 128, n0 + wn * (16 * NI), accumulate, lane);
@@ -776,6 +808,22 @@
         else gemm_et_x64p_kernel<PREC, false, false><<<grid, block, 0, s>>>(X64P_ARGS);
 #undef X64P_ARGS
     }
+    return hipGetLastError();
+}
+
+template <int PREC>
+hipError_t launch_gemm_x64p_vt(const void* A, const void* B, void* C, const float* bias, int M, int N, int K, int ld, void* vt, int tokens,
+                               hipStream_t s) {
+    const int ntiles = (M / QBM) * (N / WBN);
+    const int n_cu = cu_count();
+    dim3 grid(ntiles < n_cu ? ntiles : n_cu), block(QTHREADS);
+    VtOut v;
+    v.vt = reinterpret_cast<uint16_t*>(vt);
+    v.tokens = tokens;
+    v.from = 2 * (N / 3);
+    gemm_et_x64p_kernel<PREC, false, false, false, false, false, false, true><<<grid, block, 0, s>>>(
+        reinterpret_cast<const uint16_t*>(A), reinterpret_cast<const uint16_t*>(B), C, bias, M, N, K, 0, nullptr, nullptr, nullptr, nullptr, 0,
+        MxOut(), ld, v);
     return hipGetLastError();
 }
 
@@ -1469,6 +1517,20 @@
     });
 }
 
+bool gemm_qkv_vt_ok(int prec, int M, int N, int K, int ld, int tokens) {
+    return (prec == PREC_F16 || prec == PREC_BF16) && gemm_vt_ok(M, N, K, ld, tokens, prec == PREC_F16, gemm_env());
+}
+int gemm_debug_vt_ok(int prec, int M, int N, int K, int ld, int tokens, int variant) {
+    GemmEnv e = gemm_env();
+    e.variant = variant;
+    return ((prec == PREC_F16 || prec == PREC_BF16) && gemm_vt_ok(M, N, K, ld, tokens, prec == PREC_F16, e)) ? 1 : 0;
+}
+hipError_t launch_gemm_et_qkv_vt(int prec, const void* A, const void* B, void* C, const float* bias, int M, int N, int K, int ld, void* vt,
+                                 int tokens, hipStream_t s) {
+    if (!A || !B || !C || !vt || !gemm_qkv_vt_ok(prec, M, N, K, ld, tokens)) return hipErrorInvalidValue;
+    return with_prec(prec, [&](auto P) { return launch_gemm_x64p_vt<P.value>(A, B, C, bias, M, N, K, ld, vt, tokens, s); });
+}
+
 bool gemm_has_experiments() {
 #ifdef SAMRS_EXPERIMENTS
     return true;
diff --git a/samrs_amd/csrc/gemm_select.h b/samrs_amd/csrc/gemm_select.h
--- a/samrs_amd/csrc/gemm_select.h
+++ b/samrs_amd/csrc/gemm_select.h
@@ -174,5 +174,10 @@
     e.variant = 8;
     return N <= 1280 && K >= 2 * XBK && gemm_is_x64_wide(gemm_plan_choice(M, N, K, true, false, true, e));
 }
+inline bool gemm_vt_ok(int M, int N, int K, int ld, int tokens, bool f16, const GemmEnv& e) {
+    if (M <= 0 || N <= 0 || N % 3 || tokens <= 0 || tokens % QBM || M % tokens || (2 * (N / 3)) % WBN) return false;
+    const GemmChoice ch = gemm_select(GemmCall{M, N, K, false, false, false, false, ld, f16}, e);
+    return !ch.reject && ch.kernel == GemmKernel::X64P;
+}
 
 }
diff --git a/samrs_amd/csrc/kernels.h b/samrs_amd/csrc/kernels.h
--- a/samrs_amd/csrc/kernels.h
+++ b/samrs_amd/csrc/kernels.h
@@ -11,6 +11,10 @@
                           bool gelu, bool accumulate, hipStream_t s, GemmOpts opts = {});
 void gemm_debug_choice(int prec, int M, int N, int K, bool out_f32, bool gelu, bool accumulate, bool has_add2d, int ld, int variant,
                        int32_t* out8);
+bool gemm_qkv_vt_ok(int prec, int M, int N, int K, int ld, int tokens);
+int gemm_debug_vt_ok(int prec, int M, int N, int K, int ld, int tokens, int variant);
+hipError_t launch_gemm_et_qkv_vt(int prec, const void* A, const void* B, void* C, const float* bias, int M, int N, int K, int ld, void* vt,
+                                 int tokens, hipStream_t s);
 hipError_t launch_gemm_et_gln(int prec, const void* A, const void* B, void* C, const float* bias, const float* gamma_beta,
                               int M, int N, int K, hipStream_t s, const void* A_lo = nullptr, const void* B_lo = nullptr);
 hipError_t launch_gemm_et_stats(int prec, const void* A, const void* B, float* C, const float* bias, void* Xh, float* stats,
@@ -73,7 +77,9 @@
                              int cols = 0, int ld = 0 );
 hipError_t launch_global_attention(int prec, const void* qkv, const float* rel_h, const float* rel_w, void* out,
                                    int n_images, int grid, int heads, int head_dim, void* vt_ws, hipStream_t s, void* out_lo = nullptr,
-                                   void* mx_q_hi = nullptr, void* mx_q_lo = nullptr, void* mx_s_hi = nullptr, void* mx_s_lo = nullptr);
+                                   void* mx_q_hi = nullptr, void* mx_q_lo = nullptr, void* mx_s_hi = nullptr, void* mx_s_lo = nullptr,
+                                   bool vt_ready = false);
+hipError_t launch_vt_pack(const void* qkv, void* vt_ws, int n_images, int grid, int heads, int head_dim, hipStream_t s);
 hipError_t launch_neck_im2col(const void* in, void* A, int n_images, int grid, int C, hipStream_t s);
 hipError_t launch_transpose_f32(const float* in, float* out, int rows, int cols, hipStream_t s);
 
diff --git a/samrs_amd/engine.py b/samrs_amd/engine.py
--- a/samrs_amd/engine.py
+++ b/samrs_amd/engine.py
@@ -221,6 +221,13 @@
         lib.samrs_k_gelu_split.argtypes = [ip, vp, vp, vp, i64, vp]
         for name in ("samrs_k_gemm_f32_batch", "samrs_k_patch_im2col", "samrs_k_transpose_f32", "samrs_k_gelu_split"):
             getattr(lib, name).restype = ip
+    if hasattr(lib, "samrs_k_gemm_qkv_vt"):
+        lib.samrs_debug_gemm_vt_ok.argtypes = [ip] * 7
+        lib.samrs_k_gemm_qkv_vt.argtypes = [ip, vp, vp, vp, vp, ip, ip, ip, ip, vp, ip, vp]
+        lib.samrs_k_vt_pack.argtypes = [vp, vp, ip, ip, ip, ip, vp]
+        lib.samrs_debug_block_route.argtypes = [vp, ip, ip, C.POINTER(C.c_int32)]
+        for name in ("samrs_debug_gemm_vt_ok", "samrs_k_gemm_qkv_vt", "samrs_k_vt_pack", "samrs_debug_block_route"):
+            getattr(lib, name).restype = ip
     for name in ("samrs_load_weight", "samrs_finalize_weights", "samrs_set_images", "samrs_set_images_ragged", "samrs_get_embedding",
                  "samrs_set_embedding", "samrs_reset_image", "samrs_predict", "samrs_predict_multi", "samrs_paint", "samrs_k_gemm",
                  "samrs_k_gemm_f32", "samrs_k_convert", "samrs_k_layernorm", "samrs_k_window_attention",
@@ -420,6 +427,12 @@
             self._check(self.lib.samrs_debug_encoder_prefix(self.handle, images_u8.data_ptr(), n, h, w, n_blocks,
                                                             out.data_ptr(), _stream()))
         return out
+
+    def debug_block_route(self, n_images: int, block: int) -> Dict[str, int]:
+        out = (C.c_int32 * 4)()
+        with torch.cuda.device(self.device):
+            self._check(self.lib.samrs_debug_block_route(self.handle, n_images, block, out))
+        return {"global": out[0], "qkv": out[1], "qkv_ld": out[2], "vt_from_qkv": out[3]}
 
     def outlier_columns(self, block: int, gemm: int):
         buf = (C.c_int32 * 32)()
@@ -574,8 +587,11 @@
         c = 3 if multimask_output else 1
         masks = [None] * n_img
         if want_masks:
-            masks = [torch.empty(counts[i], c, orig_hw[2 * i], orig_hw[2 * i + 1],
-                                 dtype=torch.float32 if return_logits else torch.uint8, device=dev) for i in range(n_img)]
+            mdt = torch.float32 if return_logits else torch.uint8
+            if len({(orig_hw[2 * i], orig_hw[2 * i + 1]) for i in range(n_img)}) == 1:
+                masks = list(torch.split(torch.empty(n, c, orig_hw[0], orig_hw[1], dtype=mdt, device=dev), counts))
+            else:
+                masks = [torch.empty(counts[i], c, orig_hw[2 * i], orig_hw[2 * i + 1], dtype=mdt, device=dev) for i in range(n_img)]
         iou = torch.empty(n, c, **f32)
         low = torch.empty(n, c, 256, 256, **f32)
         if n > 0:
```

Result: no change. 148.8, median of 5 (+0.1%).
